# lnkloveating/MediQuery-RAG

Hardware: AMD Instinct MI355X
Metric: queries/s (embed+top-k, k=5, b=256) over 1M×768 corpus; p50 single-query ms (higher is better)
Workload: dtype f32 (exact 3-way bf16 split, fp32 accumulate; exact fp32 top-k)

## Files before the change

### include/mq.h

```cpp
#ifndef MQ_H
#define MQ_H

#include <stdint.h>

#ifdef __cplusplus
extern "C" {
#endif

#define MQ_OK 0
#define MQ_EINVAL -1
#define MQ_ENOMEM -2
#define MQ_EHIP -3
#define MQ_EIO -4
#define MQ_ESTATE -5

#define MQ_DTYPE_F32 0
#define MQ_DTYPE_BF16 1
#define MQ_DTYPE_F32X6 2
#define MQ_DTYPE_F32_SCREEN 3

#define MQ_GELU_ERF 0
#define MQ_GELU_TANH 1
#define MQ_POOL_CLS 0
#define MQ_POOL_MEAN 1

#define MQ_MAX_K 64

typedef struct mq_index mq_index;
typedef struct mq_encoder mq_encoder;

const char* mq_last_error(void);
const char* mq_version(void);
const char* mq_build_source_hash(void);
int mq_device_count(void);

int mq_index_create(int device, int dim, int64_t capacity, int dtype, mq_index** out);
int mq_index_destroy(mq_index* ix);
int mq_index_size(const mq_index* ix, int64_t* n_rows);
int mq_index_dim(const mq_index* ix, int* dim);
int mq_index_add(mq_index* ix, const float* rows, int64_t n, int rows_on_device, void* stream);
int mq_index_reset(mq_index* ix);
int mq_index_search(mq_index* ix, const float* queries, int64_t nq, int k,
                    float* out_scores, int64_t* out_ids, int io_on_device, void* stream);
int mq_index_select(mq_index* src, const int64_t* rows, int64_t n, mq_index* dst);
int mq_index_get(mq_index* ix, int64_t row0, int64_t n, float* out, int out_on_device, void* stream);
int mq_index_set_precision(mq_index* ix, int dtype);
int mq_index_set_stream_threshold(mq_index* ix, int max_queries);
int mq_index_set_threshold_scan(mq_index* ix, int enabled);
int mq_index_set_int8_screen(mq_index* ix, int enabled);
int mq_index_set_async_screen(mq_index* ix, int enabled);
int mq_index_rescans(const mq_index* ix, int64_t* rescans, int64_t* remerges);
int mq_index_screen_fallbacks(const mq_index* ix, int64_t* to_direct, int64_t* to_split);
int mq_index_screen_skips(const mq_index* ix, int64_t* bf16_skips, int64_t* int8_skips);
int mq_index_data(mq_index* ix, void** device_rows);
int mq_index_set_timing(mq_index* ix, int enabled);
int mq_index_read_timing(mq_index* ix, float* ms, int n);
#define MQ_MASK_SET 0
#define MQ_MASK_AND 1
#define MQ_MASK_OR 2
#define MQ_MASK_CLEAR 3
int mq_mask_eval(const int32_t* codes, int64_t n, const uint8_t* lut, int n_lut, uint32_t* bits, int mode,
                 void* stream);
int mq_mask_eval_bits(const int32_t* codes, int64_t n, const uint64_t* lut_words, int n_lut, uint32_t* bits,
                      int mode, void* stream);
int mq_mask_combine(uint32_t* dst, const uint32_t* src, int64_t n_words, int mode, void* stream);
int mq_index_search_masked(mq_index* ix, const float* query, int k, const uint32_t* bits, float* out_scores,
                           int64_t* out_ids, int io_on_device, void* stream);
int mq_index_search_masked_batch(mq_index* ix, const float* queries, int64_t nq, int k, const uint32_t* bits,
                                 float* out_scores, int64_t* out_ids, int io_on_device, void* stream);
int mq_index_masked_gathers(const mq_index* ix, int64_t* count);
#define MQ_CONTAINS_MAX_BYTES 256
#define MQ_CONTAINS_SPAN_BYTES 16384
int mq_mask_contains(const uint8_t* text, int64_t text_bytes, const int64_t* offsets, int64_t n,
                     const uint8_t* pattern, int pattern_len, int negate, uint32_t* bits, int mode,
                     uint32_t* scratch, void* stream);

#define MQ_MMR_SCORE(fmul, fsub, lambda, s, red) \
  fsub(fmul((lambda), (s)), fmul(fsub(1.0f, (lambda)), (red)))
int mq_index_mmr_select(mq_index* ix, const float* cand_scores, const int64_t* cand_ids, int64_t nq,
                        int fetch_k, int k, float lambda, float* out_scores, int64_t* out_ids,
                        int io_on_device, void* stream);
int mq_index_search_mmr(mq_index* ix, const float* queries, int64_t nq, int k, int fetch_k,
                        float lambda, const uint32_t* bits, float* out_scores, int64_t* out_ids,
                        int io_on_device, void* stream);

int mq_index_save(mq_index* ix, const char* path);
int mq_index_load(mq_index* ix, const char* path);
int mq_index_save_rows(mq_index* ix, const char* path, int64_t row0, int64_t n);
int mq_index_load_append(mq_index* ix, const char* path);

int mq_topk_merge_host(const float* scores, const int64_t* ids, int n_lists, int64_t nq,
                       int k_in, int k_out, float* out_scores, int64_t* out_ids);
int mq_topk_merge_device(const float* scores, const int64_t* ids, int n_lists, int64_t nq,
                         int k_in, int k_out, float* out_scores, int64_t* out_ids, void* stream);

typedef struct mq_bert_config {
  int vocab_size;
  int hidden;
  int layers;
  int heads;
  int ffn;
  int max_positions;
  int type_vocab;
  float ln_eps;
  int gelu;
  int pooling;
} mq_bert_config;

int mq_encoder_create(int device, const mq_bert_config* cfg, mq_encoder** out);
int mq_encoder_destroy(mq_encoder* enc);
int64_t mq_encoder_weight_count(const mq_bert_config* cfg);
int mq_encoder_load_weights(mq_encoder* enc, const float* blob, int64_t n_floats);
int mq_encoder_set_precision(mq_encoder* enc, int dtype);
#define MQ_ENC_STAGES 8
int mq_encoder_set_graphs(mq_encoder* enc, int enabled);
#define MQ_ENC_OPT_ROWS_MAX 0
#define MQ_ENC_OPT_ROWS_SPLITS 1
#define MQ_ENC_OPT_SPLITK_MAX 2
#define MQ_ENC_OPT_LN_ROWS_PER_WAVE 3
#define MQ_ENC_OPT_FUSE_ATTN_OPROJ 4
#define MQ_ENC_OPT_FUSED_LN 5
#define MQ_ENC_OPT_SPLITK_TILES 6
#define MQ_ENC_OPT_LN_ON_LOAD 7
#define MQ_ENC_OPT_RESIDENT_LAYERS 8
#define MQ_ENC_OPT_X6_PRESPLIT 9
#define MQ_ENC_OPT_ROWS_PLANES 10
#define MQ_ENC_OPT_LN_FOLD 11
#define MQ_ENC_OPT_CLS_KFREE 12
int mq_encoder_set_option(mq_encoder* enc, int option, int value);
int mq_encoder_get_option(const mq_encoder* enc, int option, int* value);
int mq_encoder_set_timing(mq_encoder* enc, int enabled);
int mq_encoder_read_timing(mq_encoder* enc, float* ms, int n);
int mq_encoder_embed(mq_encoder* enc, const int32_t* ids, const int32_t* mask, int B, int L,
                     float* out, int io_on_device, void* stream);

#define MQ_HEAD_MAX_LABELS 8
int mq_encoder_load_head(mq_encoder* enc, const float* pooler_w, const float* pooler_b, const float* cls_w,
                         const float* cls_b, int n_labels);
int mq_encoder_score(mq_encoder* enc, const int32_t* ids, const int32_t* types, const int32_t* mask, int B,
                     int L, float* logits, int io_on_device, void* stream);

typedef struct mq_tokenizer mq_tokenizer;
int mq_tokenizer_create_wordpiece(const char* vocab_path, int lower_case, int max_length,
                                  mq_tokenizer** out);
int mq_tokenizer_create_wordpiece_tokens(const char* const* tokens, int n_tokens, int lower_case,
                                         int max_length, mq_tokenizer** out);
int mq_tokenizer_create_char(int vocab_size, int max_length, mq_tokenizer** out);
int mq_tokenizer_destroy(mq_tokenizer* tok);
int mq_tokenizer_encode_batch(mq_tokenizer* tok, const char* const* texts, int n, int pad_to,
                              int32_t* ids, int32_t* mask, int* out_len);

int mq_tokenizer_encode_pairs(mq_tokenizer* tok, const char* const* first, const char* const* second, int n,
                              int pad_to, int32_t* ids, int32_t* types, int32_t* mask, int* out_len);

int mq_debug_gemm_f32(const float* A, const float* W, const float* bias, const float* resid,
                      float* out, int M, int N, int K, int epi, int tile, void* stream);
int64_t mq_debug_w3_bytes(int N, int K);
int mq_debug_split_w3(const float* W, int N, int K, void* w3, void* stream);
int mq_debug_gemm_x6p(const float* A, const void* W3, const float* bias, const float* resid,
                      float* out, int M, int N, int K, int epi, int tile, void* stream);
int mq_debug_gemm_x6p_ln(const float* A, const void* W3, const float* bias, const float* resid,
                         float* out, int M, int N, int K, int epi, int tile, const float* stats_in,
                         float* stats_out, const float* g, const float* b, const float* s_fold,
                         float eps, void* stream);
int mq_debug_ln_fold_weight(const float* W, const float* bias, const float* g, const float* b, int N,
                            int K, float* Wg, float* s_out, float* c_out, void* stream);
int mq_debug_attention(const float* qkv, const int* mask, int B, int L, int H, int heads, float scale,
                       int variant, float* ctx, void* stream);
int mq_debug_cls_attention(const float* q, const float* x, const float* stats, const float* ln_g,
                           const float* ln_b, float eps, const int* mask, int B, int L, int H, int heads,
                           float scale, const float* Wk, const float* Wv, const float* bv, float* ctx,
                           void* stream);
int mq_debug_attn_oproj(const float* qkv, const int* mask, int B, int L, int H, int heads, float scale,
                        const float* Wo, const float* bo, const float* resid, int cls_only, int hg, int qf,
                        int acc, float* out, void* stream);

int mq_debug_cls_head(const float* cls, int B, int H, const float* pooler_w, const float* pooler_b,
                      const float* cls_w, const float* cls_b, int n_labels, float* logits, void* stream);

int mq_debug_int8_screen(mq_index* ix, const float* query, int kc, float* out_scores, int64_t* out_ids,
                         float* stats);

#ifdef __cplusplus
}
#endif
#endif
```

### mediquery-rag_amd/csrc/encoder.hip

```cpp
#include <algorithm>
#include <cmath>
#include <cstdlib>
#include <cstring>
#include <memory>
#include <vector>

#include "cls_head.hpp"
#include "common.hpp"
#include "gemm_epi.hpp"
#include "gemm_f32.hpp"
#include "gemm_x6p.hpp"

namespace mq {


struct LnArgs {
  float* stats_out;
  const float* stats_in;
  const float* g;
  const float* b;
  float* xout;
  int ldx;
  int nt;
  float eps;
// ... 1572 lines not shown
      float mu, rho;
      ln_merge(sr, eps, mu, rho);
#pragma unroll
      for (int j = 0; j < 4; ++j) xr[j] = (xr[j] - mu) * rho;
    }
#pragma unroll
    for (int j = 0; j < 4; ++j) *reinterpret_cast<floatx4*>(xs + lrow * H + (lc4 + TPR * j) * 4) = xr[j];
    const int live_key = mk;
    __syncthreads();
    if (k0 + CH < L) fetch(k0 + CH);
    float d[CH];
#pragma unroll
    for (int k = 0; k < CH; ++k) {
      float a = 0.f;
#pragma unroll
      for (int i = 0; i < VPL; ++i) {
        const floatx4 v = *reinterpret_cast<const floatx4*>(xs + k * H + (i * 64 + lane) * 4);
        a = fmaf(v.x, ur[i].x, fmaf(v.y, ur[i].y, fmaf(v.z, ur[i].z, fmaf(v.w, ur[i].w, a))));
      }
      d[k] = a;
    }
#pragma unroll
    for (int k = 0; k < CH; ++k) d[k] = wave_sum_fast(d[k]);
    float sc = -INFINITY;
#pragma unroll
    for (int k = 0; k < CH; ++k) sc = lane == k ? d[k] : sc;
    sc = live_key != 0 ? sc * scale : -INFINITY;
    float tmax = sc;
#pragma unroll
    for (int off = 8; off > 0; off >>= 1) tmax = fmaxf(tmax, __shfl_xor(tmax, off));
    tmax = __shfl(tmax, 0);
    const float m_new = fmaxf(m_run, tmax);
    const float alpha = m_new == -INFINITY ? 1.f : expf(m_run - m_new);
    const float p = sc == -INFINITY ? 0.f : expf(sc - m_new);
    float psum = p;
#pragma unroll
    for (int off = 8; off > 0; off >>= 1) psum += __shfl_xor(psum, off);
    psum = __shfl(psum, 0);
    l_run = l_run * alpha + psum;
    m_run = m_new;
    if (lane < CH) ps[lane * HEADS + h] = p;
    if (lane == 0) alpha_s[h] = alpha;
    __syncthreads();
#pragma unroll
    for (int q4 = 0; q4 < HEADS / 4; ++q4) {
      const floatx4 a = *reinterpret_cast<const floatx4*>(alpha_s + 4 * q4);
#pragma unroll
      for (int e = 0; e < 4; ++e) zacc[4 * q4 + e] *= a[e];
    }
#pragma unroll
    for (int k = 0; k < CH; ++k) {
      const float xv = xs[k * H + t];
#pragma unroll
      for (int q4 = 0; q4 < HEADS / 4; ++q4) {
        const floatx4 pp = *reinterpret_cast<const floatx4*>(ps + k * HEADS + 4 * q4);
#pragma unroll
        for (int e = 0; e < 4; ++e) zacc[4 * q4 + e] = fmaf(pp[e], xv, zacc[4 * q4 + e]);
      }
    }
    __syncthreads();
  }
  if (lane == 0) l_s[h] = l_run;
  __syncthreads();
#pragma unroll
  for (int hh = 0; hh < HEADS; ++hh) {
    const float l = l_s[hh];
    float v = l > 0.f ? zacc[hh] * (1.0f / l) : 0.f;
    if constexpr (FOLD) v = l > 0.f ? fmaf(v, g[t], be[t]) : 0.f;
    z[((int64_t)b * HEADS + hh) * H + t] = v;
  }
  if (t == 0) live[b] = l_s[0] > 0.f ? 1.f : 0.f;
}

}

using namespace mq;

namespace {

struct Buf {
  float* p = nullptr;
  size_t n = 0;
  int ensure(size_t need) {
    if (need <= n) return MQ_OK;
    if (p) (void)hipFree(p);
    p = nullptr;
    n = 0;
    if (hipMalloc((void**)&p, need * sizeof(float)) != hipSuccess)
      MQ_FAIL(MQ_ENOMEM, "hipMalloc(%zu floats) failed", need);
    n = need;
    return MQ_OK;
  }
  void release() {
    if (p) (void)hipFree(p);
    p = nullptr;
    n = 0;
  }
};

struct LayerW {
  const float *wqkv, *bqkv, *wo, *bo, *ln1g, *ln1b, *w1, *b1, *w2, *b2, *ln2g, *ln2b;
  const unsigned char *wqkv3 = nullptr, *wo3 = nullptr, *w13 = nullptr, *w23 = nullptr;
  const float *wqkvf = nullptr, *wof = nullptr, *w1f = nullptr, *w2f = nullptr;
  const unsigned char *w1g3 = nullptr, *wqkvg3 = nullptr;
  const float *w1gf = nullptr, *wqkvgf = nullptr;
  const float *w1s = nullptr, *w1c = nullptr, *wqkvs = nullptr, *wqkvc = nullptr;
};

int64_t weight_count(const mq_bert_config& c) {
  const int64_t H = c.hidden, F = c.ffn;
  const int64_t per_layer = 3 * H * H + 3 * H + H * H + H + 2 * H + F * H + F + H * F + H + 2 * H;
  return ((int64_t)c.vocab_size + c.max_positions + c.type_vocab) * H + 2 * H + c.layers * per_layer;
}

}


namespace {

struct GemmArgs {
  float* slab;
  size_t slab_floats;
  const float* A;
  int lda;
  const float* W;
  const float* bias;
  const float* resid;
  int ldr;
  float* out;
  int ldo;
  int M, N, K;
  int nt = 0;
  const void* W3 = nullptr;
  LnFold lf{};
};

template <class T, int EPI, bool LN_IN = false>
void launch_gemm_t(const GemmArgs& g, int num_cus, hipStream_t s, const LnArgs& ln = LnArgs{}) {
  const int tiles = ((g.M + T::BM - 1) / T::BM) * ((g.N + T::BN - 1) / T::BN);
  const int grid = (std::min(tiles, T::WG_PER_CU * num_cus) + 7) / 8 * 8;
  const int tiles_m = (g.M + T::BM - 1) / T::BM, tiles_n = (g.N + T::BN - 1) / T::BN;
  const int rx = region_pick_rx(tiles_m, tiles_n, (double)T::BM * g.K * 4, (double)T::BN * g.K * 4, grid);
  hipLaunchKernelGGL((gemm_nt_kernel<T, EPI, LN_IN>), dim3(grid), dim3(T::THREADS), 0, s, g.A, g.lda, g.W,
                     g.bias, g.resid, g.ldr, g.out, g.ldo, g.M, g.N, g.K, ln, rx, g.lf);
}

using GemmBig = F32Tile<2, 2, 2, 2>;
using GemmT96 = F32Tile<4, 1, 1, 3>;
using GemmMid = F32Tile<2, 2, 2, 1>;
using GemmSmall = F32Tile<1, 4, 1, 1>;

using X6Big = F32Tile<2, 2, 2, 2, true, 2, false, 0, false, true>;
using X6T96 = F32Tile<4, 1, 1, 3, true, 2, false, 0, false, true>;
using X6Mid = F32Tile<2, 2, 2, 1, true, 2, false, 0, false, true>;
using X6W192 = F32Tile<4, 2, 1, 3, true, 2, false, 0, false, true>;

template <int EPI>
void launch_gemm_tile(const GemmArgs& g, int tile, int num_cus, hipStream_t s) {
  switch (tile) {
    case 0: launch_gemm_t<GemmBig, EPI>(g, num_cus, s); return;
    case 1: launch_gemm_t<GemmT96, EPI>(g, num_cus, s); return;
    case 2: launch_gemm_t<GemmMid, EPI>(g, num_cus, s); return;
    case 5: launch_gemm_t<X6Big, EPI>(g, num_cus, s); return;
    case 6: launch_gemm_t<X6T96, EPI>(g, num_cus, s); return;
    case 7: launch_gemm_t<X6Mid, EPI>(g, num_cus, s); return;
    case 8: launch_gemm_t<F32Tile<4, 2, 1, 3>, EPI>(g, num_cus, s); return;
    case 9: launch_gemm_t<X6W192, EPI>(g, num_cus, s); return;
    default: launch_gemm_t<GemmSmall, EPI>(g, num_cus, s); return;
  }
}

int splitk_factor(const GemmArgs& g, int num_cus, int cap = 16, int tiles_max = 0) {
  if (!g.slab || g.N % 4 != 0) return 0;
  const int64_t tiles = (int64_t)((g.M + 31) / 32) * ((g.N + 127) / 128);
  const int64_t slots = 2 * (int64_t)num_cus;
  if (tiles > (tiles_max > 0 ? tiles_max : num_cus) || g.M > 256) return 0;
  const int slices = g.K / kBK;
  int best = 1;
  for (int s = 1; s <= slices && s <= cap; ++s)
    if (slices % s == 0 && tiles * s <= slots && (size_t)s * g.M * g.N <= g.slab_floats) best = s;
  return best >= 2 ? best : 0;
}

void launch_splitk_gemm(const GemmArgs& g, int S, hipStream_t s) {
  auto go = [&](auto tile) {
    using T = decltype(tile);
    const int tiles = ((g.M + T::BM - 1) / T::BM) * ((g.N + T::BN - 1) / T::BN);
    hipLaunchKernelGGL((gemm_splitk_kernel<T>), dim3(tiles * S), dim3(256), 0, s, g.A, g.lda, g.W, g.M, g.N, g.K,
                       S, g.slab);
  };
  if (g.nt)
    go(F32Tile<1, 4, 1, 1, false, 2, false, 0, true>{});
  else
    go(F32Tile<1, 4, 1, 1>{});
}

template <int EPI>
void launch_splitk(const GemmArgs& g, int S, hipStream_t s) {
  launch_splitk_gemm(g, S, s);
  const int64_t n4 = (int64_t)g.M * g.N / 4;
  hipLaunchKernelGGL((splitk_reduce_kernel<EPI>), dim3((unsigned)((n4 + 255) / 256)), dim3(256), 0,
                     s, g.slab, S, g.M, g.N, g.bias, g.resid, g.ldr, g.out, g.ldo);
}

int x6_tile_pick(const GemmArgs& g, int num_cus) {
  const int bns[3] = {128, 96, 64};
  const double effs[3] = {1.0, 0.96, 0.9};
  const int64_t slots = 2 * (int64_t)num_cus;
  int best = 0;
  double best_cost = 1e300;
  for (int i = 0; i < 3; ++i) {
    const int64_t tiles = (int64_t)((g.M + 127) / 128) * ((g.N + bns[i] - 1) / bns[i]);
    const double cost = (double)((tiles + slots - 1) / slots) * 128 * bns[i] / effs[i];
    if (cost < best_cost) {
      best_cost = cost;
      best = i;
    }
  }
  return best;
}

template <int EPI>
void launch_gemm_fold(const GemmArgs& g, int num_cus, hipStream_t s) {
  if (g.W3) {
    X6pArgs a{g.A, g.lda, g.W3, g.bias, g.resid, g.ldr, g.out, g.ldo, g.M, g.N, g.K};
    a.lf = g.lf;
    launch_gemm_x6p(a, EPI, -1, num_cus, s);
    return;
  }
  if constexpr (EPI == EPI_RESID_LN_STATS) {
    launch_gemm_t<X6T96, EPI>(g, num_cus, s);
  } else {
    switch (x6_tile_pick(g, num_cus)) {
      case 0: launch_gemm_t<X6Big, EPI>(g, num_cus, s); return;
      case 1: launch_gemm_t<X6T96, EPI>(g, num_cus, s); return;
      default: launch_gemm_t<X6Mid, EPI>(g, num_cus, s); return;
    }
  }
}

template <int EPI>
void launch_gemm(const GemmArgs& g, int num_cus, hipStream_t s, bool x6 = false, int splitk_cap = 16,
                 int splitk_tiles = 0) {
  const int S = splitk_factor(g, num_cus, splitk_cap, splitk_tiles);
  if (S) {
    launch_splitk<EPI>(g, S, s);
    return;
  }
  if (x6 && (int64_t)((g.M + 127) / 128) * ((g.N + 191) / 192) < num_cus) x6 = false;
  if (x6 && g.W3) {
    launch_gemm_x6p(X6pArgs{g.A, g.lda, g.W3, g.bias, g.resid, g.ldr, g.out, g.ldo, g.M, g.N, g.K}, EPI, -1, num_cus,
                    s);
    return;
  }
  if (x6) {
    launch_gemm_tile<EPI>(g, 5 + x6_tile_pick(g, num_cus), num_cus, s);
    return;
  }
  struct Cand {
    int bm, bn;
    double eff;
  };
  const Cand cands[4] = {{128, 128, 1.0}, {128, 96, 0.96}, {128, 64, 0.9}, {32, 128, 0.55}};
  const int64_t slots = 2 * (int64_t)num_cus;
  int best = 0;
  double best_cost = 1e300;
  for (int i = 0; i < 4; ++i) {
    const int64_t tiles = (int64_t)((g.M + cands[i].bm - 1) / cands[i].bm) * ((g.N + cands[i].bn - 1) / cands[i].bn);
    const int64_t rounds = (tiles + slots - 1) / slots;
    const double cost = (double)rounds * cands[i].bm * cands[i].bn / cands[i].eff;
    if (cost < best_cost) {
      best_cost = cost;
      best = i;
    }
  }
  launch_gemm_tile<EPI>(g, best, num_cus, s);
}

void launch_gemm_stats(const GemmArgs& g, const LnArgs& ln, int num_cus, hipStream_t s) {
  launch_gemm_t<GemmT96, EPI_RESID_STATS>(g, num_cus, s, ln);
}

template <int EPI>
void launch_gemm_ln_in(const GemmArgs& g, const LnArgs& ln, int num_cus, hipStream_t s) {
  const int64_t slots = 2 * (int64_t)num_cus;
  auto cost = [&](int bn, double eff) {
    const int64_t tiles = (int64_t)((g.M + 127) / 128) * ((g.N + bn - 1) / bn);
    return (double)((tiles + slots - 1) / slots) * 128 * bn / eff;
  };
  if (cost(128, 1.0) <= cost(96, 0.96))
    launch_gemm_t<GemmBig, EPI, true>(g, num_cus, s, ln);
  else
    launch_gemm_t<GemmT96, EPI, true>(g, num_cus, s, ln);
}

#ifndef MQ_LN_FOLD_DEFAULT
#define MQ_LN_FOLD_DEFAULT 1
#endif
constexpr bool kLnFoldDefault = MQ_LN_FOLD_DEFAULT != 0;
#ifndef MQ_CLS_KFREE_DEFAULT
#define MQ_CLS_KFREE_DEFAULT 1
#endif
constexpr bool kClsKfreeDefault = MQ_CLS_KFREE_DEFAULT != 0;

enum Stage { ST_EMBED = 0, ST_QKV, ST_ATTN, ST_OPROJ, ST_LN, ST_FFN_UP, ST_FFN_DOWN, ST_POOL, ST_N };


}

struct mq_encoder {
  int device = 0;
  PinBuf pin;
  mq_bert_config cfg{};
  int precision = MQ_DTYPE_F32;
  bool loaded = false;
  Buf weights;
  const float *word = nullptr, *pos = nullptr, *typ = nullptr, *eg = nullptr, *eb = nullptr;
  std::vector<LayerW> layers;
  Buf x, y, qkv, ctx, ffn, io_out, slab;
  Buf w3;
  Buf wfrag;
  int* io_ids = nullptr;
  int* io_mask = nullptr;
  size_t io_tokens = 0;
  Timeline tl;
  int num_cus = 256;
  struct Graph {
    int B = 0, L = 0, precision = 0;
    std::vector<const void*> bufs;
    hipGraphExec_t exec = nullptr;
    uint64_t last_use = 0;
  };
  std::vector<Graph> graphs;
  bool fuse_attn_oproj = true;
  int rows_max = kRowsDefault;
  int rows_splits = 0;
  int splitk_max = 16;
  int splitk_tiles = 0;
  int ln_rows_per_wave = 4;
  bool fused_ln = false;
  int resident_layers = 8;
  bool ln_on_load = false;
  Buf lnst;
  bool x6_presplit = true;
  bool ln_fold = kLnFoldDefault;
  Buf wfold3, wfoldf, sfold;
  bool rows_planes = false;
  bool cls_kfree = kClsKfreeDefault;
  Buf wkt;
  Buf cls;
  Buf head;
  int n_labels = 0;
  Buf cls_state;
  int* io_types = nullptr;
  size_t io_type_tokens = 0;
  bool use_graphs = false;
  uint64_t graph_clock = 0;
  hipStream_t cap_stream = nullptr;
  std::mutex mu;
};

namespace {

int build_w3(mq_encoder* e) {
  if (e->precision != MQ_DTYPE_F32X6 || !e->loaded || e->layers.empty() || e->layers[0].wqkv3) return MQ_OK;
  const mq_bert_config& c = e->cfg;
  const int H = c.hidden, F = c.ffn;
  const size_t per = w3_bytes(3 * H, H) + w3_bytes(H, H) + w3_bytes(F, H) + w3_bytes(H, F);
  DeviceGuard dg(e->device);
  int rc = e->w3.ensure((per * e->layers.size() + 3) / 4);
  if (rc) return rc;
  unsigned char* p = reinterpret_cast<unsigned char*>(e->w3.p);
  for (LayerW& w : e->layers) {
    auto one = [&](const float* W, int n, int k, const unsigned char*& dst) {
      launch_split_w3(W, n, k, p, nullptr);
      dst = p;
      p += w3_bytes(n, k);
    };
    one(w.wqkv, 3 * H, H, w.wqkv3);
    one(w.wo, H, H, w.wo3);
    one(w.w1, F, H, w.w13);
    one(w.w2, H, F, w.w23);
  }
  MQ_HIP(hipGetLastError());
  MQ_HIP(hipStreamSynchronize(nullptr));
  return MQ_OK;
}

int build_fold(mq_encoder* e) {
  const mq_bert_config& c = e->cfg;
  const int H = c.hidden, F = c.ffn;
  if (!e->ln_fold || e->precision != MQ_DTYPE_F32X6 || !e->loaded || e->layers.empty() ||
      H != kLnPartW * kLnMaxParts || F % 32 != 0)
    return MQ_OK;
  const bool img = e->x6_presplit;
  if (img ? e->layers[0].w1g3 != nullptr : e->layers[0].w1gf != nullptr) return MQ_OK;
  const size_t nl = e->layers.size();
  DeviceGuard dg(e->device);
  int rc = e->sfold.ensure(nl * 2 * ((size_t)F + 3 * H));
  if (rc) return rc;
  Buf tmp;
  if (img) {
    rc = e->wfold3.ensure((nl * w3_bytes(F, H) + (nl - 1) * w3_bytes(3 * H, H) + 3) / 4);
    if (!rc) rc = tmp.ensure((size_t)std::max(F, 3 * H) * H);
  } else {
    rc = e->wfoldf.ensure((nl * (size_t)F + (nl - 1) * (size_t)3 * H) * H);
  }
  if (rc) return rc;
  unsigned char* p3 = reinterpret_cast<unsigned char*>(e->wfold3.p);
  float* pf = e->wfoldf.p;
  float* ps = e->sfold.p;
  const LayerW* prev = nullptr;
  for (LayerW& w : e->layers) {
    auto one = [&](const float* W, const float* bias, const float* g, const float* b, int n, const unsigned char*& d3,
                   const float*& df, const float*& ds, const float*& dc) {
      float* wg = img ? tmp.p : pf;
      launch_ln_fold_weight(W, bias, g, b, n, H, wg, ps, ps + n, nullptr);
      ds = ps;
      dc = ps + n;
      ps += 2 * n;
      if (img) {
        launch_split_w3(wg, n, H, p3, nullptr);
        d3 = p3;
        p3 += w3_bytes(n, H);
      } else {
        df = pf;
        pf += (size_t)n * H;
      }
    };
    one(w.w1, w.b1, w.ln1g, w.ln1b, F, w.w1g3, w.w1gf, w.w1s, w.w1c);
    if (prev) one(w.wqkv, w.bqkv, prev->ln2g, prev->ln2b, 3 * H, w.wqkvg3, w.wqkvgf, w.wqkvs, w.wqkvc);
    prev = &w;
  }
  const hipError_t e1 = hipGetLastError(), e2 = hipStreamSynchronize(nullptr);
  tmp.release();
  MQ_HIP(e1);
  MQ_HIP(e2);
  return MQ_OK;
}

int build_frag16(mq_encoder* e) {
  const mq_bert_config& c = e->cfg;
  const int64_t H = c.hidden, F = c.ffn;
  const int64_t per = 3 * H * H + H * H + F * H + H * F;
  DeviceGuard dg(e->device);
  int rc = e->wfrag.ensure((size_t)(per * (int64_t)e->layers.size()));
  if (rc) return rc;
  float* p = e->wfrag.p;
  for (LayerW& w : e->layers) {
    auto one = [&](const float* W, int64_t r, int64_t k, const float*& dst) {
      const int64_t n4 = r * k / 4;
      hipLaunchKernelGGL(frag16_image_kernel, dim3((unsigned)((n4 + 255) / 256)), dim3(256), 0, nullptr, W, (int)r,
                         (int)k, reinterpret_cast<floatx4*>(p));
      dst = p;
      p += r * k;
    };
    one(w.wqkv, 3 * H, H, w.wqkvf);
    one(w.wo, H, H, w.wof);
    one(w.w1, F, H, w.w1f);
    one(w.w2, H, F, w.w2f);
  }
  MQ_HIP(hipGetLastError());
  MQ_HIP(hipStreamSynchronize(nullptr));
  return MQ_OK;
}

int build_wkt(mq_encoder* e) {
  const int H = e->cfg.hidden;
  if (e->cfg.pooling != MQ_POOL_CLS || e->layers.empty()) return MQ_OK;
  DeviceGuard dg(e->device);
  int rc = e->wkt.ensure((size_t)H * H);
  if (rc) return rc;
  hipLaunchKernelGGL(transpose_kernel, dim3(H / 32, H / 32), dim3(256), 0, nullptr,
                     e->layers.back().wqkv + (int64_t)H * H, H, H, e->wkt.p);
  MQ_HIP(hipGetLastError());
  MQ_HIP(hipStreamSynchronize(nullptr));
  return MQ_OK;
}

template <int EPI>
void gemm(mq_encoder* e, const GemmArgs& g, int stage, hipStream_t s) {
  e->tl.mark(s, stage);
  GemmArgs a = g;
  if (!e->x6_presplit) a.W3 = nullptr;
  launch_gemm<EPI>(a, e->num_cus, s, e->precision == MQ_DTYPE_F32X6, e->splitk_max, e->splitk_tiles);
}

template <int VPL>
void gemm_resid_ln(mq_encoder* e, const GemmArgs& g, const float* lng, const float* lnb, float* x,
                   int stage, hipStream_t s) {
  const int H = VPL * 256;
  const unsigned rb = (unsigned)((g.M + 3) / 4);
  const int S = splitk_factor(g, e->num_cus, e->splitk_max, e->splitk_tiles);
  if constexpr (VPL <= 3) {
    if (!S && e->fused_ln && e->precision == MQ_DTYPE_F32 && g.ldr == H && g.N == H && g.resid == x) {
      using T = F32Tile<1, 8, 1, VPL, false, 2, false, 16>;
      e->tl.mark(s, stage);
      const int tiles = (g.M + 31) / 32;
      hipLaunchKernelGGL((gemm_resid_ln_kernel<T>), dim3(std::min(tiles, e->num_cus)), dim3(T::THREADS), 0, s,
                         g.A, g.lda, g.W, g.bias, g.resid, lng, lnb, e->cfg.ln_eps, x, g.M, g.K);
      return;
    }
  }
  if (S && g.ldr == H && g.N == H) {
    e->tl.mark(s, stage);
    launch_splitk_gemm(g, S, s);
    e->tl.mark(s, ST_LN);
    hipLaunchKernelGGL((splitk_reduce_ln_kernel<VPL>), dim3((unsigned)g.M), dim3(256), 0, s, g.slab, S,
                       g.M, g.bias, g.resid, g.ldr, lng, lnb, e->cfg.ln_eps, x, 0);
    return;
  }
  gemm<EPI_RESID>(e, g, stage, s);
  e->tl.mark(s, ST_LN);
  const int rpw = e->ln_rows_per_wave;
  if (rpw == 4)
    hipLaunchKernelGGL((ln_kernel<VPL, 4>), dim3((unsigned)((g.M + 15) / 16)), dim3(256), 0, s, g.out, g.M, lng,
                       lnb, e->cfg.ln_eps, x);
  else if (rpw == 1)
    hipLaunchKernelGGL((ln_kernel<VPL, 1>), dim3(rb), dim3(256), 0, s, g.out, g.M, lng, lnb, e->cfg.ln_eps, x);
  else
    hipLaunchKernelGGL((ln_kernel<VPL, 2>), dim3((unsigned)((g.M + 7) / 8)), dim3(256), 0, s, g.out, g.M, lng,
                       lnb, e->cfg.ln_eps, x);
}

struct ClsBufs {
  float *xc, *q, *u, *z, *part, *live;
  static size_t floats(int B, int H, int heads) {
    return (size_t)B * ((2 + kClsCtxSplits) * H + 2 * (size_t)heads * H + 1);
  }
  ClsBufs(float* p, int B, int H, int heads)
      : xc(p), q(xc + (size_t)B * H), u(q + (size_t)B * H), z(u + (size_t)B * heads * H),
        part(z + (size_t)B * heads * H), live(part + (size_t)kClsCtxSplits * B * H) {}
};

void launch_cls_u(int B, int H, int heads, const float* q, const float* wkt, float* u, hipStream_t s) {
  using T = F32Tile<1, 4, 1, 1>;
  const int tiles = ((B + T::BM - 1) / T::BM) * ((H + T::BN - 1) / T::BN);
  hipLaunchKernelGGL((gemm_heads_kernel<T>), dim3(tiles * heads), dim3(256), 0, s, q, H, kDh, wkt, H, kDh, nullptr,
                     nullptr, B, H, kDh, u, heads * H, H, 1, (int64_t)0);
}

void launch_cls_ctx(int B, int L, int H, int heads, float scale, const float* x, const float* stats,
                    const float* g, const float* be, float eps, const float* u, const int* mask, const float* wv,
                    const float* bv, float* z, float* part, float* live, float* ctx, hipStream_t s) {
  auto pass = [&](auto vpl) {
    constexpr int VPL = decltype(vpl)::value;
    if (stats)
      hipLaunchKernelGGL((cls_pass_kernel<VPL, true>), dim3(B), dim3(256 * VPL), 0, s, x, stats, g, be, eps, u, mask, L,
                         scale, z, live);
    else
      hipLaunchKernelGGL((cls_pass_kernel<VPL, false>), dim3(B), dim3(256 * VPL), 0, s, x, stats, g, be, eps, u, mask, L,
                         scale, z, live);
  };
  if (H == 256)
    pass(IC<1>{});
  else if (H == 512)
    pass(IC<2>{});
  else
    pass(IC<3>{});
  using T = F32Tile<2, 2, 1, 1>;
  const int tiles = (B + T::BM - 1) / T::BM;
  hipLaunchKernelGGL((gemm_heads_kernel<T>), dim3(tiles * heads * kClsCtxSplits), dim3(256), 0, s, z, heads * H, H, wv, H,
                     kDh * H, nullptr, nullptr, B, kDh, H, part, H, kDh, kClsCtxSplits, (int64_t)B * H);
  hipLaunchKernelGGL(cls_ctx_reduce_kernel, dim3((unsigned)(((int64_t)B * H / 4 + 255) / 256)), dim3(256), 0, s, part, B,
                     H, bv, live, ctx);
}

template <int VPL>
void gemm_resid_ln_pool(mq_encoder* e, const GemmArgs& g, const float* lng, const float* lnb, const int* mask,
                        float* out, int raw, int stage, hipStream_t s) {
  const int H = VPL * 256;
  const int S = splitk_factor(g, e->num_cus, e->splitk_max, e->splitk_tiles);
  if (S && g.ldr == H && g.N == H) {
    e->tl.mark(s, stage);
    launch_splitk_gemm(g, S, s);
    e->tl.mark(s, ST_POOL);
    hipLaunchKernelGGL((splitk_reduce_ln_kernel<VPL, true>), dim3((unsigned)g.M), dim3(256), 0, s, g.slab, S, g.M,
                       g.bias, g.resid, g.ldr, lng, lnb, e->cfg.ln_eps, out, raw);
    return;
  }
  gemm<EPI_RESID>(e, g, stage, s);
  e->tl.mark(s, ST_POOL);
  hipLaunchKernelGGL((ln_pool_kernel<VPL>), dim3((unsigned)((g.M + 3) / 4)), dim3(256), 0, s, g.out, 1, (int64_t)0, mask,
                     g.M, 1, 1, MQ_POOL_CLS, lng, lnb, e->cfg.ln_eps, out, raw);
}

template <int VPL>
int forward_vpl(mq_encoder* e, const int* ids, const int* types, const int* mask, int B, int L, float* out,
                int raw_cls, hipStream_t s) {
  const mq_bert_config& c = e->cfg;
  const int M = B * L, H = c.hidden, F = c.ffn;
  const unsigned row_blocks = (unsigned)((M + 3) / 4);
  const float scale = 1.0f / sqrtf((float)(H / c.heads));
  const int q_tiles = (L + 31) / 32;
  e->tl.mark(s, ST_EMBED);
  hipLaunchKernelGGL((embed_ln_kernel<VPL>), dim3(row_blocks), dim3(256), 0, s, ids, M, L,
                     c.vocab_size, e->word, e->pos, e->typ, types, c.type_vocab, e->eg, e->eb, c.ln_eps, e->x.p);
  const int nt = H / kLnPartW;
  const bool lnl = e->ln_on_load && !e->fused_ln && e->precision == MQ_DTYPE_F32 && M > 256 &&
                   H == kLnPartW * kLnMaxParts && e->lnst.n >= (size_t)4 * M * nt;
  float* st1 = e->lnst.p;
  float* st2 = lnl ? e->lnst.p + (size_t)2 * M * nt : nullptr;
  bool y_pending = false;
  const LayerW* prev = nullptr;
  const LayerW w0 = e->layers.empty() ? LayerW{} : e->layers[0];
  const bool fold = e->ln_fold && e->precision == MQ_DTYPE_F32X6 && M > 256 && H == kLnPartW * kLnMaxParts &&
                    F % 32 == 0 && (int64_t)((M + 127) / 128) * ((H + 191) / 192) >= e->num_cus &&
                    e->lnst.n >= (size_t)4 * M * nt && (e->x6_presplit ? w0.w1g3 != nullptr : w0.w1gf != nullptr);
  float* fst1 = e->lnst.p;
  float* fst2 = e->lnst.p + (size_t)2 * M * nt;
  bool raw = false;
  bool pooled = false;
  auto fold_gemm = [&](auto epi, GemmArgs g, int stage) {
    e->tl.mark(s, stage);
    if (!e->x6_presplit) g.W3 = nullptr;
    g.lf.eps = c.ln_eps;
    launch_gemm_fold<decltype(epi)::value>(g, e->num_cus, s);
  };
  auto ln_args = [&](const float* stats, const float* g, const float* b) {
    LnArgs a{};
    a.stats_in = stats;
    a.g = g;
    a.b = b;
    a.xout = e->x.p;
    a.ldx = H;
    a.nt = nt;
    a.eps = c.ln_eps;
    return a;
  };
  auto stats_out = [&](float* stats) {
    LnArgs a{};
    a.stats_out = stats;
    a.nt = nt;
    return a;
  };
  for (size_t li = 0; li < e->layers.size(); ++li) {
    const LayerW& w = e->layers[li];
    const bool cls_only = c.pooling == MQ_POOL_CLS && li + 1 == e->layers.size();
    const int rows = cls_only ? B : M;
    int stride = cls_only ? L * H : H;
    const float* resid = e->x.p;
    int ldr = stride;
    const bool kfree = cls_only && L > 1 && e->cls_kfree && VPL <= 3 && e->wkt.p != nullptr &&
                       e->cls.n >= ClsBufs::floats(B, H, c.heads);
    const float* qkv_in = y_pending ? e->y.p : e->x.p;
    const int lnt = M <= 256 && (int)li >= e->resident_layers ? 1 : 0;
    const bool fold_layer = fold && !(cls_only && L > 1);
    auto qkv_fold = [&](GemmArgs g, int row0) {
      g.W = w.wqkvgf ? w.wqkvgf + (int64_t)row0 * H : nullptr;
      g.W3 = w.wqkvg3 ? w.wqkvg3 + w3_row_offset(row0, H) : nullptr;
      g.bias = w.wqkvc + row0;
      g.lf.s = w.wqkvs + row0;
      g.lf.stats_in = fst2;
      fold_gemm(IC<EPI_BIAS_LNFOLD>{}, g, ST_QKV);
    };
    auto qkv_gemm = [&](GemmArgs g) {
      g.nt = lnt;
      if (raw) {
        qkv_fold(g, (int)(g.W - w.wqkv) / H);
      } else if (y_pending) {
        e->tl.mark(s, ST_QKV);
        launch_gemm_ln_in<EPI_BIAS>(g, ln_args(st2, prev->ln2g, prev->ln2b), e->num_cus, s);
      } else {
        gemm<EPI_BIAS>(e, g, ST_QKV, s);
      }
    };
    if (kfree) {
      const ClsBufs cb(e->cls.p, B, H, c.heads);
      const float* xin = raw ? e->x.p : y_pending ? e->y.p : e->x.p;
      const float* xst = raw ? fst2 : y_pending ? st2 : nullptr;
      if (xst) {
        e->tl.mark(s, ST_LN);
        hipLaunchKernelGGL((ln_rows_kernel<VPL>), dim3((unsigned)((B + 3) / 4)), dim3(256), 0, s, xin, B, (int64_t)L * H,
                           prev->ln2g, prev->ln2b, c.ln_eps, cb.xc);
        resid = cb.xc;
        ldr = H;
      }
      GemmArgs q{e->slab.p, e->slab.n, resid, ldr, w.wqkv, w.bqkv, nullptr, 0, cb.q, H, B, H, H, lnt};
      q.W3 = w.wqkv3;
      gemm<EPI_BIAS>(e, q, ST_QKV, s);
      launch_cls_u(B, H, c.heads, cb.q, e->wkt.p, cb.u, s);
      e->tl.mark(s, ST_ATTN);
      launch_cls_ctx(B, L, H, c.heads, scale, xin, xst, xst ? prev->ln2g : nullptr, xst ? prev->ln2b : nullptr,
                     c.ln_eps, cb.u, mask, w.wqkv + (int64_t)2 * H * H, w.bqkv + 2 * H, cb.z, cb.part, cb.live, e->ctx.p, s);
      stride = H;
    } else if (cls_only && L > 1) {
      GemmArgs kv{e->slab.p, e->slab.n, qkv_in, H, w.wqkv + (int64_t)H * H, w.bqkv + H, nullptr, 0, e->qkv.p + H,
                  3 * H, M, 2 * H, H};
      if (w.wqkv3) kv.W3 = w.wqkv3 + w3_row_offset(H, H);
      qkv_gemm(kv);
      if (raw) {
        e->tl.mark(s, ST_LN);
        hipLaunchKernelGGL((ln_rows_inplace_kernel<VPL>), dim3((unsigned)((B + 3) / 4)), dim3(256), 0, s, e->x.p, B,
                           (int64_t)L * H, prev->ln2g, prev->ln2b, c.ln_eps);
      }
      GemmArgs q{e->slab.p, e->slab.n, e->x.p, L * H, w.wqkv, w.bqkv, nullptr, 0, e->qkv.p, L * 3 * H, B, H, H, lnt};
      q.W3 = w.wqkv3;
      gemm<EPI_BIAS>(e, q, ST_QKV, s);
    } else {
      GemmArgs qkv{e->slab.p, e->slab.n, qkv_in, H, w.wqkv, w.bqkv, nullptr, 0, e->qkv.p, 3 * H, M, 3 * H, H};
      qkv.W3 = w.wqkv3;
      qkv_gemm(qkv);
    }
    y_pending = false;
    const bool resid_raw = raw && fold_layer;
    raw = false;
    if (!kfree) {
      e->tl.mark(s, ST_ATTN);
      const int qt = cls_only ? 1 : q_tiles;
      launch_attention(B, L, c.heads, qt, H, scale, e->qkv.p, mask, e->ctx.p, s);
    }
    const bool lnl_layer = lnl && !cls_only;
    GemmArgs oproj{e->slab.p, e->slab.n, e->ctx.p, stride, w.wo, w.bo, resid, ldr, e->y.p, H, rows, H, H, lnt};
    oproj.W3 = w.wo3;
    if (fold_layer) {
      oproj.lf.stats_out = fst1;
      if (resid_raw) {
        oproj.lf.stats_in = fst2;
        oproj.lf.g = prev->ln2g;
        oproj.lf.b = prev->ln2b;
      }
      fold_gemm(IC<EPI_RESID_LN_STATS>{}, oproj, ST_OPROJ);
    } else if (lnl_layer) {
      e->tl.mark(s, ST_OPROJ);
      launch_gemm_stats(oproj, stats_out(st1), e->num_cus, s);
    } else {
      gemm_resid_ln<VPL>(e, oproj, w.ln1g, w.ln1b, e->x.p, ST_OPROJ, s);
    }
    GemmArgs up{e->slab.p, e->slab.n, lnl_layer ? e->y.p : e->x.p, H, w.w1, w.b1, nullptr, 0, e->ffn.p, F,
                rows, F, H, lnt};
    up.W3 = w.w13;
    if (fold_layer) {
      up.A = e->y.p;
      up.W = w.w1gf;
      up.W3 = w.w1g3;
      up.bias = w.w1c;
      up.lf.s = w.w1s;
      up.lf.stats_in = fst1;
      if (c.gelu == MQ_GELU_TANH)
        fold_gemm(IC<EPI_GELU_TANH_LNFOLD>{}, up, ST_FFN_UP);
      else
        fold_gemm(IC<EPI_GELU_ERF_LNFOLD>{}, up, ST_FFN_UP);
    } else if (lnl_layer) {
      e->tl.mark(s, ST_FFN_UP);
      if (c.gelu == MQ_GELU_TANH)
        launch_gemm_ln_in<EPI_GELU_TANH>(up, ln_args(st1, w.ln1g, w.ln1b), e->num_cus, s);
      else
        launch_gemm_ln_in<EPI_GELU_ERF>(up, ln_args(st1, w.ln1g, w.ln1b), e->num_cus, s);
    } else if (c.gelu == MQ_GELU_TANH) {
      gemm<EPI_GELU_TANH>(e, up, ST_FFN_UP, s);
    } else {
      gemm<EPI_GELU_ERF>(e, up, ST_FFN_UP, s);
    }
    GemmArgs down{e->slab.p, e->slab.n, e->ffn.p, F, w.w2, w.b2, e->x.p, H, e->y.p, H, rows, H, F, lnt};
    down.W3 = w.w23;
    if (fold_layer) {
      const bool last = li + 1 == e->layers.size();
      down.resid = e->y.p;
      down.lf.stats_in = fst1;
      down.lf.g = w.ln1g;
      down.lf.b = w.ln1b;
      down.lf.stats_out = fst2;
      down.out = last ? e->ctx.p : e->x.p;
      fold_gemm(IC<EPI_RESID_LN_STATS>{}, down, ST_FFN_DOWN);
      if (last) {
        e->tl.mark(s, ST_LN);
        hipLaunchKernelGGL((ln_kernel<VPL, 4>), dim3((unsigned)((M + 15) / 16)), dim3(256), 0, s, e->ctx.p, M, w.ln2g,
                           w.ln2b, c.ln_eps, e->x.p);
      } else {
        raw = true;
      }
    } else if (lnl_layer && li + 1 < e->layers.size()) {
      e->tl.mark(s, ST_FFN_DOWN);
      launch_gemm_stats(down, stats_out(st2), e->num_cus, s);
      y_pending = true;
    } else if (kfree) {
      gemm_resid_ln_pool<VPL>(e, down, w.ln2g, w.ln2b, mask, out, raw_cls, ST_FFN_DOWN, s);
      pooled = true;
    } else {
      gemm_resid_ln<VPL>(e, down, w.ln2g, w.ln2b, e->x.p, ST_FFN_DOWN, s);
    }
    prev = &w;
  }
  if (!pooled) {
    e->tl.mark(s, ST_POOL);
    const bool pruned = c.pooling == MQ_POOL_CLS;
    hipLaunchKernelGGL((pool_kernel<VPL>), dim3((B + 3) / 4), dim3(256), 0, s, e->x.p, mask, B,
                       pruned ? 1 : L, c.pooling, out, raw_cls);
  }
  e->tl.close(s);
  MQ_HIP(hipGetLastError());
  return MQ_OK;
}

struct RowsArgs {
  const float* A;
  int lda;
  int64_t a_plane;
  const float* W;
  int ldw;
  const float* bias;
  const float* resid;
  int ldr;
  float* out;
  int ldo;
  int64_t o_plane;
  int M, N, K;
  int splits;
  const int* ids = nullptr;
  int L = 1, vocab = 0;
  const float* pos = nullptr;
  const float* typ = nullptr;
  const int* types = nullptr;
  int type_vocab = 1;
  int nt_w = 0;
  float* zbuf = nullptr;
  int64_t zn = 0;
};

template <int EPI, bool LN_IN, int VPL, int NB, int S_IN, int RT, int FL>
void launch_rows_rt(const RowsArgs& g, const float* lng, const float* lnb, float eps, float* ln_out,
                    hipStream_t s) {
  hipLaunchKernelGGL((rows_gemm_kernel<EPI, LN_IN, VPL, NB, S_IN, RT, FL>),
                     dim3(g.N / kRT, (g.M + kRT * RT - 1) / (kRT * RT), g.splits), dim3(64 * kRWaves), 0, s,
                     g.A, g.lda, g.a_plane, g.M, lng, lnb, eps, ln_out, g.W, g.ldw, g.bias, g.resid, g.ldr,
                     g.out, g.ldo, g.o_plane, g.ids, g.L, g.vocab, g.pos, g.typ, g.types, g.type_vocab, g.nt_w, g.zbuf,
                     g.zn);
}

template <int EPI, bool LN_IN, int VPL, int NB, int S_IN, int FL = 0>
void launch_rows_nb(const RowsArgs& g, const float* lng, const float* lnb, float eps, float* ln_out,
                    hipStream_t s) {
  constexpr bool two_fit = LN_IN && (size_t)(2 * kRT * (NB * 256 + 4) + kRWaves * 2 * kRT * kRT) * 4 <= 160 * 1024;
  if constexpr (two_fit) {
    if (g.M > kRT) {
      launch_rows_rt<EPI, LN_IN, VPL, NB, S_IN, 2, FL>(g, lng, lnb, eps, ln_out, s);
      return;
    }
  }
  launch_rows_rt<EPI, LN_IN, VPL, NB, S_IN, 1, FL>(g, lng, lnb, eps, ln_out, s);
}

bool rows_nb_ok(int nb) { return nb >= 1 && (nb <= 4 || nb == 6 || nb == 8 || nb == 12 || nb == 16); }

int rows_splits(int K, int forced = 0) {
  const int nb = K / 256;
  if (forced >= 1 && forced <= 4 && nb % forced == 0 && rows_nb_ok(nb / forced)) return forced;
  for (int sp = 1; sp <= 4; ++sp)
    if (nb % sp == 0 && nb / sp <= 6 && rows_nb_ok(nb / sp)) return sp;
  return 1;
}

template <int EPI, int NB, int FL>
void launch_rows_plain(const RowsArgs& g, hipStream_t s) {
  launch_rows_nb<EPI, false, 1, NB, 1, FL>(g, nullptr, nullptr, 0.f, nullptr, s);
}

template <int EPI, int FL = 0>
void launch_rows(const RowsArgs& g, hipStream_t s) {
  switch (g.K / g.splits / 256) {
    case 1: launch_rows_plain<EPI, 1, FL>(g, s); return;
    case 2: launch_rows_plain<EPI, 2, FL>(g, s); return;
    case 3: launch_rows_plain<EPI, 3, FL>(g, s); return;
    case 4: launch_rows_plain<EPI, 4, FL>(g, s); return;
    case 6: launch_rows_plain<EPI, 6, FL>(g, s); return;
    case 8: launch_rows_plain<EPI, 8, FL>(g, s); return;
    case 12: launch_rows_plain<EPI, 12, FL>(g, s); return;
    default: launch_rows_plain<EPI, 16, FL>(g, s); return;
  }
}

template <int EPI, int VPL, int FL = 0>
void launch_rows_ln(const RowsArgs& g, int s_in, const float* lng, const float* lnb, float eps,
                    float* ln_out, hipStream_t s) {
  switch (s_in) {
    case 0: launch_rows_nb<EPI, true, VPL, VPL, 0, FL>(g, lng, lnb, eps, ln_out, s); return;
    case 1: launch_rows_nb<EPI, true, VPL, VPL, 1, FL>(g, lng, lnb, eps, ln_out, s); return;
    case 2: launch_rows_nb<EPI, true, VPL, VPL, 2, FL>(g, lng, lnb, eps, ln_out, s); return;
    case 3: launch_rows_nb<EPI, true, VPL, VPL, 3, FL>(g, lng, lnb, eps, ln_out, s); return;
    default: launch_rows_nb<EPI, true, VPL, VPL, 4, FL>(g, lng, lnb, eps, ln_out, s); return;
  }
}

template <int HG, bool QF, bool ACC>
void launch_attn_oproj_hg(int nkb, dim3 grid, hipStream_t s, const float* qkv, const int* mask, int L, int H,
                          int rps, int qtiles, float scale, const float* wo, const float* bo, const float* resid,
                          int ldr, float* out, int64_t o_plane, int nt_w) {
  auto go = [&](auto kern) {
    hipLaunchKernelGGL(kern, grid, dim3(512), 0, s, qkv, mask, L, H, rps, qtiles, scale, wo, bo, resid, ldr, out,
                       o_plane, nt_w);
  };
  switch (nkb) {
    case 1: go(attn_oproj_rows_kernel<HG, 1, QF, ACC>); break;
    case 2: go(attn_oproj_rows_kernel<HG, 2, QF, ACC>); break;
    case 3: go(attn_oproj_rows_kernel<HG, 3, QF, ACC>); break;
    default: go(attn_oproj_rows_kernel<HG, 4, QF, ACC>); break;
  }
}

void launch_attn_oproj(int hg, bool qf, bool acc, int nkb, dim3 grid, hipStream_t s, const float* qkv,
                       const int* mask, int L, int H, int rps, int qtiles, float scale, const float* wo,
                       const float* bo, const float* resid, int ldr, float* out, int64_t o_plane, int nt_w) {
  auto go = [&](auto hgc, auto qfc, auto accc) {
    launch_attn_oproj_hg<decltype(hgc)::value, decltype(qfc)::value, decltype(accc)::value>(
        nkb, grid, s, qkv, mask, L, H, rps, qtiles, scale, wo, bo, resid, ldr, out, o_plane, nt_w);
  };
  if (hg == 6) {
    if (qf && acc) go(IC<6>{}, std::true_type{}, std::true_type{});
    else if (qf) go(IC<6>{}, std::true_type{}, std::false_type{});
    else if (acc) go(IC<6>{}, std::false_type{}, std::true_type{});
    else go(IC<6>{}, std::false_type{}, std::false_type{});
  } else {
    if (qf && acc) go(IC<4>{}, std::true_type{}, std::true_type{});
    else if (qf) go(IC<4>{}, std::true_type{}, std::false_type{});
    else if (acc) go(IC<4>{}, std::false_type{}, std::true_type{});
    else go(IC<4>{}, std::false_type{}, std::false_type{});
  }
}

int oproj_heads_per_plane(const mq_encoder* e, int L) {
  const mq_bert_config& c = e->cfg;
  if (!e->fuse_attn_oproj || L > 64 || c.hidden != c.heads * kDh || c.hidden % kOpCols) return 0;
  return c.heads % 6 == 0 ? 6 : c.heads % 4 == 0 ? 4 : 0;
}

template <int VPL>
int forward_rows(mq_encoder* e, const int* ids, const int* types, const int* mask, int B, int L, float* out,
                 int raw, hipStream_t s) {
  const mq_bert_config& c = e->cfg;
  const int M = B * L, H = c.hidden, F = c.ffn;
  const float eps = c.ln_eps;
  const float scale = 1.0f / sqrtf((float)(H / c.heads));
  const int q_tiles = (L + 31) / 32;
  const int dsplit = rows_splits(F, e->rows_splits);
  const int hg = oproj_heads_per_plane(e, L);
  const bool qf = hg != 0 && L % 16 == 0 && (3 * H) % 48 == 0;
  const bool dacc = dsplit == 2 && !e->rows_planes;
  const bool yacc = hg != 0 && c.heads / hg == 2 && !e->rows_planes;
  int prev_rows = M;
  for (size_t li = 0; li < e->layers.size(); ++li) {
    const LayerW& w = e->layers[li];
    const bool cls_only = c.pooling == MQ_POOL_CLS && li + 1 == e->layers.size();
    const int rows = cls_only ? B : M;
    const int stride = cls_only ? L * H : H;
    const int nt = (int)li >= e->resident_layers ? 1 : 0;
    e->tl.mark(s, ST_QKV);
    RowsArgs qkv{e->slab.p, H, (int64_t)prev_rows * H, w.wqkvf, H, w.bqkv, nullptr, 0, e->qkv.p, 3 * H, 0, M, 3 * H, H, 1};
    qkv.nt_w = nt;
    if (li == 0) {
      qkv.A = e->word;
      qkv.a_plane = 0;
      qkv.ids = ids;
      qkv.L = L;
      qkv.vocab = c.vocab_size;
      qkv.pos = e->pos;
      qkv.typ = e->typ;
      qkv.types = types;
      qkv.type_vocab = c.type_vocab;
    }
    const LayerW* pl = li ? &e->layers[li - 1] : nullptr;
    const float* lg = pl ? pl->ln2g : e->eg;
    const float* lb = pl ? pl->ln2b : e->eb;
    const int s_in = pl ? (dacc ? 1 : dsplit) : 0;
    if (yacc) {
      qkv.zbuf = e->y.p;
      qkv.zn = (int64_t)rows * H;
    }
    if (qf)
      ROWS_REP launch_rows_ln<EPI_BIAS, VPL, FL_O | FL_OT>(qkv, s_in, lg, lb, eps, e->x.p, s);
    else
      ROWS_REP launch_rows_ln<EPI_BIAS, VPL>(qkv, s_in, lg, lb, eps, e->x.p, s);
    const int qt = cls_only ? 1 : q_tiles;
    int y_planes = 1;
    if (hg) {
      e->tl.mark(s, ST_OPROJ);
      const int rps = cls_only ? 1 : L, qtiles = (rps + 15) / 16;
      y_planes = c.heads / hg;
      const dim3 grid(H / kOpCols, B * qtiles, y_planes);
      if (yacc) y_planes = 1;
      ROWS_REP launch_attn_oproj(hg, qf, yacc, (L + 15) / 16, grid, s, e->qkv.p, mask, L, H, rps, qtiles, scale, w.wof, w.bo, e->x.p,
                                 stride, e->y.p, (int64_t)rows * H, nt);
    } else {
      e->tl.mark(s, ST_ATTN);
      if (L <= 64)
        hipLaunchKernelGGL(attention_rows_kernel, dim3(B * c.heads * qt), dim3(512), 0, s, e->qkv.p, mask, L,
                           H, c.heads, qt, scale, e->ctx.p);
      else
        launch_attention(B, L, c.heads, qt, H, scale, e->qkv.p, mask, e->ctx.p, s);
      e->tl.mark(s, ST_OPROJ);
      RowsArgs oproj{e->ctx.p, stride, 0, w.wof, H, w.bo, e->x.p, stride, e->y.p, H, 0, rows, H, H, 1};
      oproj.nt_w = nt;
      launch_rows<EPI_RESID>(oproj, s);
    }
    e->tl.mark(s, ST_FFN_UP);
    RowsArgs up{e->y.p, H, (int64_t)rows * H, w.w1f, H, w.b1, nullptr, 0, e->ffn.p, F, 0, rows, F, H, 1};
    up.nt_w = nt;
    if (dacc) {
      up.zbuf = e->slab.p;
      up.zn = (int64_t)rows * H;
    }
    if (c.gelu == MQ_GELU_TANH)
      ROWS_REP launch_rows_ln<EPI_GELU_TANH, VPL, FL_O>(up, y_planes, w.ln1g, w.ln1b, eps, e->x.p, s);
    else
      ROWS_REP launch_rows_ln<EPI_GELU_ERF, VPL, FL_O>(up, y_planes, w.ln1g, w.ln1b, eps, e->x.p, s);
    e->tl.mark(s, ST_FFN_DOWN);
    RowsArgs down{e->ffn.p, F, 0, w.w2f, F, w.b2, e->x.p, H, e->slab.p, H, (int64_t)rows * H, rows, H, F, dsplit};
    down.nt_w = nt;
    if (dacc)
      ROWS_REP launch_rows<EPI_RESID, FL_A | FL_ACC>(down, s);
    else
      ROWS_REP launch_rows<EPI_RESID, FL_A>(down, s);
    prev_rows = rows;
  }
// ... 122 lines not shown
               "bad config");
  MQ_CHECK_ARG(c.gelu == MQ_GELU_ERF || c.gelu == MQ_GELU_TANH, "bad gelu variant");
  MQ_CHECK_ARG(c.pooling == MQ_POOL_CLS || c.pooling == MQ_POOL_MEAN, "bad pooling");
  DeviceGuard dg(device);
  if (!dg.ok) MQ_FAIL(MQ_EHIP, "hipSetDevice(%d) failed", device);
  auto e = std::make_unique<mq_encoder>();
  e->device = device;
  e->cfg = c;
  int cus = 0;
  if (hipDeviceGetAttribute(&cus, hipDeviceAttributeMultiprocessorCount, device) == hipSuccess &&
      cus > 0)
    e->num_cus = cus;
  *out = e.release();
  return MQ_OK;
}

int mq_encoder_destroy(mq_encoder* e) {
  clear_error();
  if (!e) return MQ_OK;
  {
    DeviceGuard dg(e->device);
    for (Buf* b : {&e->weights, &e->x, &e->y, &e->qkv, &e->ctx, &e->ffn, &e->io_out, &e->slab, &e->w3, &e->wfrag,
                   &e->lnst, &e->wkt, &e->cls, &e->head, &e->cls_state})
      b->release();
    if (e->io_types) (void)hipFree(e->io_types);
    if (e->io_ids) (void)hipFree(e->io_ids);
    if (e->io_mask) (void)hipFree(e->io_mask);
    e->pin.release();
    for (auto& g : e->graphs) (void)hipGraphExecDestroy(g.exec);
    if (e->cap_stream) (void)hipStreamDestroy(e->cap_stream);
  }
  delete e;
  return MQ_OK;
}

int mq_encoder_load_weights(mq_encoder* e, const float* blob, int64_t n_floats) {
  clear_error();
  MQ_CHECK_ARG(e && blob, "NULL argument");
  const mq_bert_config& c = e->cfg;
  const int64_t need = weight_count(c);
  MQ_CHECK_ARG(n_floats == need, "weight blob has %lld floats, config needs %lld",
               (long long)n_floats, (long long)need);
  std::lock_guard<std::mutex> lk(e->mu);
  DeviceGuard dg(e->device);
  int rc = e->weights.ensure((size_t)need);
  if (rc) return rc;
  MQ_HIP(hipMemcpy(e->weights.p, blob, (size_t)need * 4, hipMemcpyHostToDevice));
  const int64_t H = c.hidden, F = c.ffn;
  const float* p = e->weights.p;
  auto take = [&](int64_t n) {
    const float* r = p;
    p += n;
    return r;
  };
  e->word = take((int64_t)c.vocab_size * H);
  e->pos = take((int64_t)c.max_positions * H);
  e->typ = take((int64_t)c.type_vocab * H);
  e->eg = take(H);
  e->eb = take(H);
  e->layers.clear();
  for (int l = 0; l < c.layers; ++l) {
    LayerW w;
    w.wqkv = take(3 * H * H);
    w.bqkv = take(3 * H);
    w.wo = take(H * H);
    w.bo = take(H);
    w.ln1g = take(H);
    w.ln1b = take(H);
    w.w1 = take(F * H);
    w.b1 = take(F);
    w.w2 = take(H * F);
    w.b2 = take(H);
    w.ln2g = take(H);
    w.ln2b = take(H);
    e->layers.push_back(w);
  }
  e->loaded = true;
  if (H % 16 == 0 && F % 16 == 0) {
    rc = build_frag16(e);
    if (rc) return rc;
  }
  rc = build_wkt(e);
  if (rc) return rc;
  return build_w3(e);
}

int mq_encoder_set_precision(mq_encoder* e, int dtype) {
  clear_error();
  MQ_CHECK_ARG(e, "NULL encoder");
  MQ_CHECK_ARG(dtype == MQ_DTYPE_F32 || dtype == MQ_DTYPE_F32X6,
               "encoder precision must be MQ_DTYPE_F32 or MQ_DTYPE_F32X6 (got %d)", dtype);
  std::lock_guard<std::mutex> lk(e->mu);
  e->precision = dtype;
  return build_w3(e);
}

int mq_debug_gemm_f32(const float* A, const float* W, const float* bias, const float* resid,
                      float* out, int M, int N, int K, int epi, int tile, void* stream) {
  clear_error();
  MQ_CHECK_ARG(A && W && bias && out && (epi != EPI_RESID || resid), "NULL buffer");
  MQ_CHECK_ARG(M > 0 && N > 0 && K > 0 && K % kBK == 0, "bad shape M=%d N=%d K=%d", M, N, K);
  MQ_CHECK_ARG(epi >= 0 && epi <= 3 && tile >= 0 && tile <= 9, "bad epi/tile");
  int dev = 0, cus = 256;
  (void)hipGetDevice(&dev);
  (void)hipDeviceGetAttribute(&cus, hipDeviceAttributeMultiprocessorCount, dev);
  GemmArgs g{nullptr, 0, A, K, W, bias, resid, N, out, N, M, N, K};
  hipStream_t s = (hipStream_t)stream;
  if (tile == 4) {
    MQ_CHECK_ARG(N % 4 == 0, "split-K needs N %% 4 == 0");
    const int slices = K / kBK;
    int S = 1;
    for (int c = 2; c <= slices && c <= 64; ++c)
      if (slices % c == 0) S = c;
    float* slab = nullptr;
    if (hipMalloc((void**)&slab, (size_t)S * M * N * 4) != hipSuccess)
      MQ_FAIL(MQ_ENOMEM, "slab allocation failed");
    g.slab = slab;
    g.slab_floats = (size_t)S * M * N;
    switch (epi) {
      case EPI_BIAS: launch_splitk<EPI_BIAS>(g, S, s); break;
      case EPI_GELU_ERF: launch_splitk<EPI_GELU_ERF>(g, S, s); break;
      case EPI_GELU_TANH: launch_splitk<EPI_GELU_TANH>(g, S, s); break;
      default: launch_splitk<EPI_RESID>(g, S, s); break;
    }
    const hipError_t err = hipStreamSynchronize(s);
    (void)hipFree(slab);
    if (err != hipSuccess) MQ_FAIL(MQ_EHIP, "split-K GEMM failed: %s", hipGetErrorString(err));
    return MQ_OK;
  }
  switch (epi) {
    case EPI_BIAS: launch_gemm_tile<EPI_BIAS>(g, tile, cus, s); break;
    case EPI_GELU_ERF: launch_gemm_tile<EPI_GELU_ERF>(g, tile, cus, s); break;
    case EPI_GELU_TANH: launch_gemm_tile<EPI_GELU_TANH>(g, tile, cus, s); break;
    default: launch_gemm_tile<EPI_RESID>(g, tile, cus, s); break;
  }
  MQ_HIP(hipGetLastError());
  return MQ_OK;
}

int mq_debug_attention(const float* qkv, const int* mask, int B, int L, int H, int heads, float scale,
                       int variant, float* ctx, void* stream) {
  clear_error();
  MQ_CHECK_ARG(qkv && mask && ctx, "NULL buffer");
  MQ_CHECK_ARG(B > 0 && L > 0 && heads > 0 && H == heads * kDh, "bad shape B=%d L=%d H=%d heads=%d", B, L, H, heads);
  hipStream_t s = (hipStream_t)stream;
  const int qt = (L + 31) / 32;
  const dim3 grid(B * heads * qt);
  switch (variant) {
    case -1: launch_attention(B, L, heads, qt, H, scale, qkv, mask, ctx, s); break;
    case 1: hipLaunchKernelGGL(attention_kernel<1>, grid, dim3(64), 0, s, qkv, mask, L, H, heads, qt, scale, ctx); break;
    case 2: hipLaunchKernelGGL(attention_kernel<2>, grid, dim3(128), 0, s, qkv, mask, L, H, heads, qt, scale, ctx); break;
    case 4: hipLaunchKernelGGL(attention_kernel<4>, grid, dim3(256), 0, s, qkv, mask, L, H, heads, qt, scale, ctx); break;
    case 8: hipLaunchKernelGGL(attention_kernel<8>, grid, dim3(512), 0, s, qkv, mask, L, H, heads, qt, scale, ctx); break;
    case 12:
      MQ_CHECK_ARG(heads == 12 && L <= 32, "variant 12 needs heads == 12 and L <= 32 (heads %d, L %d)", heads, L);
      hipLaunchKernelGGL((attention_kernel<1, 12>), dim3(B * qt), dim3(768), 0, s, qkv, mask, L, H, heads, qt, scale,
                         ctx);
      break;
    case 16:
      MQ_CHECK_ARG(L <= 64, "variant 16 (attention_rows_kernel) needs L <= 64 (got %d)", L);
      hipLaunchKernelGGL(attention_rows_kernel, grid, dim3(512), 0, s, qkv, mask, L, H, heads, qt, scale, ctx);
      break;
    default: MQ_FAIL(MQ_EINVAL, "bad attention variant %d", variant);
  }
  MQ_HIP(hipGetLastError());
  return MQ_OK;
}

int mq_debug_attn_oproj(const float* qkv, const int* mask, int B, int L, int H, int heads, float scale,
                        const float* Wo, const float* bo, const float* resid, int cls_only, int hg, int qf,
                        int acc, float* out, void* stream) {
  clear_error();
  MQ_CHECK_ARG(qkv && mask && Wo && bo && resid && out, "NULL buffer");
  MQ_CHECK_ARG(B > 0 && L > 0 && heads > 0 && H == heads * kDh, "bad shape B=%d L=%d H=%d heads=%d", B, L, H, heads);
  MQ_CHECK_ARG((hg == 4 || hg == 6) && heads % hg == 0, "hg must be 4 or 6 and divide heads (hg %d, heads %d)", hg,
               heads);
  MQ_CHECK_ARG(L <= 64, "the fused kernel holds L <= 64 keys (got %d)", L);
  MQ_CHECK_ARG(!qf || L % 16 == 0, "qf needs L %% 16 == 0 (got %d)", L);
  const int planes = heads / hg;
  MQ_CHECK_ARG(!acc || planes == 2, "acc needs two head groups (got %d)", planes);
  hipStream_t s = (hipStream_t)stream;
  const int M = B * L, rows = cls_only ? B : M;
  float* scratch = nullptr;
  const size_t wo_floats = (size_t)H * H, qkv_floats = qf ? (size_t)M * 3 * H : 0;
  if (hipMalloc((void**)&scratch, (wo_floats + qkv_floats) * 4) != hipSuccess)
    MQ_FAIL(MQ_ENOMEM, "operand image allocation failed");
  hipLaunchKernelGGL(frag16_image_kernel, dim3((unsigned)((wo_floats / 4 + 255) / 256)), dim3(256), 0, s, Wo, H, H,
                     reinterpret_cast<floatx4*>(scratch));
  const float* qkv_in = qkv;
  if (qf) {
    float* img = scratch + wo_floats;
    hipLaunchKernelGGL(frag16_qkv_image_kernel, dim3((unsigned)((qkv_floats + 255) / 256)), dim3(256), 0, s, qkv, M,
                       H, img);
    qkv_in = img;
  }
  hipError_t err = hipSuccess;
  if (acc) err = hipMemsetAsync(out, 0, (size_t)rows * H * 4, s);
  if (err == hipSuccess) {
    const int rps = cls_only ? 1 : L, qtiles = (rps + 15) / 16;
    const dim3 grid(H / kOpCols, B * qtiles, planes);
    launch_attn_oproj(hg, qf != 0, acc != 0, (L + 15) / 16, grid, s, qkv_in, mask, L, H, rps, qtiles, scale, scratch,
                      bo, resid, cls_only ? L * H : H, out, (int64_t)rows * H, 0);
    err = hipGetLastError();
  }
  const hipError_t serr = hipStreamSynchronize(s);
  (void)hipFree(scratch);
  if (err == hipSuccess) err = serr;
  if (err != hipSuccess) MQ_FAIL(MQ_EHIP, "fused attention + output projection failed: %s", hipGetErrorString(err));
  return MQ_OK;
}

int mq_debug_cls_attention(const float* q, const float* x, const float* stats, const float* ln_g,
                           const float* ln_b, float eps, const int* mask, int B, int L, int H, int heads,
                           float scale, const float* Wk, const float* Wv, const float* bv, float* ctx,
                           void* stream) {
  clear_error();
  MQ_CHECK_ARG(q && x && mask && Wk && Wv && bv && ctx, "NULL buffer");
  MQ_CHECK_ARG(B > 0 && L > 0 && heads > 0 && H == heads * kDh, "bad shape B=%d L=%d H=%d heads=%d", B, L, H, heads);
  MQ_CHECK_ARG(H == 256 || H == 512 || H == 768, "hidden must be 256 / 512 / 768 (got %d)", H);
  MQ_CHECK_ARG(!stats || (ln_g && ln_b && H == kLnPartW * kLnMaxParts), "stats need ln_g, ln_b and H = %d",
               kLnPartW * kLnMaxParts);
  hipStream_t s = (hipStream_t)stream;
  float* scratch = nullptr;
  const size_t wkt_floats = (size_t)H * H;
  if (hipMalloc((void**)&scratch, (wkt_floats + ClsBufs::floats(B, H, heads)) * 4) != hipSuccess)
    MQ_FAIL(MQ_ENOMEM, "scratch allocation failed");
  const ClsBufs cb(scratch + wkt_floats, B, H, heads);
  hipLaunchKernelGGL(transpose_kernel, dim3(H / 32, H / 32), dim3(256), 0, s, Wk, H, H, scratch);
  launch_cls_u(B, H, heads, q, scratch, cb.u, s);
  launch_cls_ctx(B, L, H, heads, scale, x, stats, ln_g, ln_b, eps, cb.u, mask, Wv, bv, cb.z, cb.part, cb.live, ctx, s);
  hipError_t err = hipGetLastError();
  const hipError_t serr = hipStreamSynchronize(s);
  (void)hipFree(scratch);
  if (err == hipSuccess) err = serr;
  if (err != hipSuccess) MQ_FAIL(MQ_EHIP, "CLS attention failed: %s", hipGetErrorString(err));
  return MQ_OK;
}

int mq_encoder_set_graphs(mq_encoder* e, int enabled) {
  clear_error();
  MQ_CHECK_ARG(e, "NULL encoder");
  std::lock_guard<std::mutex> lk(e->mu);
  e->use_graphs = enabled != 0;
  return MQ_OK;
}

int mq_encoder_set_option(mq_encoder* e, int option, int value) {
  clear_error();
  MQ_CHECK_ARG(e, "NULL encoder");
  std::lock_guard<std::mutex> lk(e->mu);
  switch (option) {
    case MQ_ENC_OPT_ROWS_MAX:
      MQ_CHECK_ARG(value >= 0 && value <= kRowsMax, "rows_max must be in [0, %d] (got %d)", kRowsMax, value);
      e->rows_max = value;
      break;
    case MQ_ENC_OPT_ROWS_SPLITS:
      MQ_CHECK_ARG(value >= 0 && value <= 4, "rows_splits must be in [0, 4] (got %d)", value);
      e->rows_splits = value;
      break;
    case MQ_ENC_OPT_SPLITK_MAX:
      MQ_CHECK_ARG(value >= 2 && value <= 64, "splitk_max must be in [2, 64] (got %d)", value);
      e->splitk_max = value;
      break;
    case MQ_ENC_OPT_LN_ROWS_PER_WAVE:
      MQ_CHECK_ARG(value == 1 || value == 2 || value == 4, "ln_rows_per_wave must be 1, 2 or 4 (got %d)", value);
      e->ln_rows_per_wave = value;
      break;
    case MQ_ENC_OPT_FUSE_ATTN_OPROJ:
      MQ_CHECK_ARG(value == 0 || value == 1, "fuse_attn_oproj must be 0 or 1 (got %d)", value);
      e->fuse_attn_oproj = value != 0;
      break;
    case MQ_ENC_OPT_FUSED_LN:
      MQ_CHECK_ARG(value == 0 || value == 1, "fused_ln must be 0 or 1 (got %d)", value);
      e->fused_ln = value != 0;
      break;
    case MQ_ENC_OPT_RESIDENT_LAYERS:
      MQ_CHECK_ARG(value >= 0 && value <= 1024, "resident_layers must be in [0, 1024] (got %d)", value);
      e->resident_layers = value;
      break;
    case MQ_ENC_OPT_LN_ON_LOAD:
      MQ_CHECK_ARG(value == 0 || value == 1, "ln_on_load must be 0 or 1 (got %d)", value);
      e->ln_on_load = value != 0;
      break;
    case MQ_ENC_OPT_SPLITK_TILES:
      MQ_CHECK_ARG(value >= 0 && value <= 4096, "splitk_tiles must be in [0, 4096] (got %d)", value);
      e->splitk_tiles = value;
      break;
    case MQ_ENC_OPT_X6_PRESPLIT:
      MQ_CHECK_ARG(value == 0 || value == 1, "x6_presplit must be 0 or 1 (got %d)", value);
      e->x6_presplit = value != 0;
      break;
    case MQ_ENC_OPT_ROWS_PLANES:
      MQ_CHECK_ARG(value == 0 || value == 1, "rows_planes must be 0 or 1 (got %d)", value);
      e->rows_planes = value != 0;
      break;
    case MQ_ENC_OPT_LN_FOLD:
      MQ_CHECK_ARG(value == 0 || value == 1, "ln_fold must be 0 or 1 (got %d)", value);
      e->ln_fold = value != 0;
      break;
    case MQ_ENC_OPT_CLS_KFREE:
      MQ_CHECK_ARG(value == 0 || value == 1, "cls_kfree must be 0 or 1 (got %d)", value);
      e->cls_kfree = value != 0;
      break;
    default:
      MQ_FAIL(MQ_EINVAL, "unknown encoder option %d", option);
  }
  for (auto& g : e->graphs) (void)hipGraphExecDestroy(g.exec);
  e->graphs.clear();
  return MQ_OK;
}

int mq_encoder_get_option(const mq_encoder* e, int option, int* value) {
  clear_error();
  MQ_CHECK_ARG(e && value, "NULL argument");
  switch (option) {
    case MQ_ENC_OPT_ROWS_MAX: *value = e->rows_max; break;
    case MQ_ENC_OPT_ROWS_SPLITS: *value = e->rows_splits; break;
    case MQ_ENC_OPT_SPLITK_MAX: *value = e->splitk_max; break;
    case MQ_ENC_OPT_LN_ROWS_PER_WAVE: *value = e->ln_rows_per_wave; break;
    case MQ_ENC_OPT_FUSE_ATTN_OPROJ: *value = e->fuse_attn_oproj ? 1 : 0; break;
    case MQ_ENC_OPT_FUSED_LN: *value = e->fused_ln ? 1 : 0; break;
    case MQ_ENC_OPT_LN_ON_LOAD: *value = e->ln_on_load ? 1 : 0; break;
    case MQ_ENC_OPT_RESIDENT_LAYERS: *value = e->resident_layers; break;
    case MQ_ENC_OPT_SPLITK_TILES: *value = e->splitk_tiles; break;
    case MQ_ENC_OPT_X6_PRESPLIT: *value = e->x6_presplit ? 1 : 0; break;
    case MQ_ENC_OPT_ROWS_PLANES: *value = e->rows_planes ? 1 : 0; break;
    case MQ_ENC_OPT_LN_FOLD: *value = e->ln_fold ? 1 : 0; break;
    case MQ_ENC_OPT_CLS_KFREE: *value = e->cls_kfree ? 1 : 0; break;
    default: MQ_FAIL(MQ_EINVAL, "unknown encoder option %d", option);
  }
  return MQ_OK;
}

int mq_encoder_set_timing(mq_encoder* e, int enabled) {
  clear_error();
  MQ_CHECK_ARG(e, "NULL encoder");
  std::lock_guard<std::mutex> lk(e->mu);
  DeviceGuard dg(e->device);
  e->tl.drain();
  e->tl.on = enabled != 0;
  return MQ_OK;
}

int mq_encoder_read_timing(mq_encoder* e, float* ms, int n) {
  clear_error();
  MQ_CHECK_ARG(e && ms && n >= 0, "bad argument");
  std::lock_guard<std::mutex> lk(e->mu);
  DeviceGuard dg(e->device);
  e->tl.read(ms, n);
  return MQ_OK;
}

}

namespace {

int ensure_forward_bufs(mq_encoder* e, int B, int L) {
  const mq_bert_config& c = e->cfg;
  const size_t M = (size_t)B * L;
  if (e->tl.used > 4096) e->tl.drain();
  int rc = MQ_OK;
  rc = e->slab.ensure((size_t)2 * e->num_cus * 32 * 128);
  if (rc) return rc;
  rc = build_fold(e);
  if (rc) return rc;
  const size_t ln_parts = (e->ln_on_load || e->ln_fold) && M > 256 ? (size_t)4 * M * std::max(1, c.hidden / kLnPartW) : 0;
  const size_t cls_floats = e->cls_kfree && c.pooling == MQ_POOL_CLS && L > 1 ? ClsBufs::floats(B, c.hidden, c.heads) : 0;
  for (auto bn : {std::make_pair(&e->x, M * c.hidden), std::make_pair(&e->y, (M <= (size_t)kRowsMax ? 4 : 1) * M * c.hidden),
                  std::make_pair(&e->ctx, M * c.hidden), std::make_pair(&e->qkv, M * 3 * c.hidden),
                  std::make_pair(&e->ffn, (M + 15) / 16 * 16 * c.ffn), std::make_pair(&e->lnst, ln_parts),
                  std::make_pair(&e->cls, cls_floats)}) {
    rc = bn.first->ensure(bn.second);
    if (rc) return rc;
  }
  return MQ_OK;
}

int ensure_io(mq_encoder* e, size_t M, int B) {
  if (e->io_tokens < M) {
    if (e->io_ids) (void)hipFree(e->io_ids);
    if (e->io_mask) (void)hipFree(e->io_mask);
    e->io_ids = e->io_mask = nullptr;
    e->io_tokens = 0;
    if (hipMalloc((void**)&e->io_ids, M * 4) != hipSuccess ||
        hipMalloc((void**)&e->io_mask, M * 4) != hipSuccess)
      MQ_FAIL(MQ_ENOMEM, "hipMalloc(io) failed");
    e->io_tokens = M;
  }
  return e->io_out.ensure((size_t)B * e->cfg.hidden);
}

}

extern "C" {

int mq_encoder_embed(mq_encoder* e, const int32_t* ids, const int32_t* mask, int B, int L,
                     float* out, int io_on_device, void* stream) {
  clear_error();
  MQ_CHECK_ARG(e, "NULL encoder");
  MQ_CHECK_ARG(B >= 0 && L >= 1, "bad shape B=%d L=%d", B, L);
  MQ_CHECK_ARG(L <= e->cfg.max_positions, "L=%d exceeds max_positions %d", L, e->cfg.max_positions);
  if (B == 0) return MQ_OK;
  MQ_CHECK_ARG(ids && mask && out, "NULL buffer");
  MQ_CHECK_ARG((int64_t)B * L < (1ll << 31) / 4096, "batch too large");
  if (!e->loaded) MQ_FAIL(MQ_ESTATE, "encoder weights not loaded");
  std::lock_guard<std::mutex> lk(e->mu);
  DeviceGuard dg(e->device);
  hipStream_t s = (hipStream_t)stream;
  const mq_bert_config& c = e->cfg;
  const size_t M = (size_t)B * L;
  int rc = ensure_forward_bufs(e, B, L);
  if (rc) return rc;
  const bool graph = e->use_graphs && !e->tl.on;
  const int* dids = ids;
  const int* dmask = mask;
  float* dout = out;
  if (!io_on_device || graph) {
    rc = ensure_io(e, M, B);
    if (rc) return rc;
    const hipMemcpyKind kind = io_on_device ? hipMemcpyDeviceToDevice : hipMemcpyHostToDevice;
    if (!io_on_device && M * 8 + (size_t)B * c.hidden * 4 <= (1u << 20)) {
      rc = e->pin.ensure(M * 8 + (size_t)B * c.hidden * 4);
      if (rc) return rc;
      memcpy(e->pin.as<unsigned char>(), ids, M * 4);
      memcpy(e->pin.as<unsigned char>() + M * 4, mask, M * 4);
      MQ_HIP(hipMemcpyAsync(e->io_ids, e->pin.p, M * 4, kind, s));
      MQ_HIP(hipMemcpyAsync(e->io_mask, e->pin.as<unsigned char>() + M * 4, M * 4, kind, s));
    } else {
      MQ_HIP(hipMemcpyAsync(e->io_ids, ids, M * 4, kind, s));
      MQ_HIP(hipMemcpyAsync(e->io_mask, mask, M * 4, kind, s));
    }
    dids = e->io_ids;
    dmask = e->io_mask;
    dout = e->io_out.p;
  }
  if (graph) {
    rc = launch_graph(e, B, L, s);
  } else {
    rc = forward(e, dids, nullptr, dmask, B, L, dout, 0, s);
  }
  if (rc) return rc;
  if (io_on_device && dout != out)
    MQ_HIP(hipMemcpyAsync(out, dout, (size_t)B * c.hidden * 4, hipMemcpyDeviceToDevice, s));
  if (!io_on_device) {
    const size_t ob = (size_t)B * c.hidden * 4;
    if (M * 8 + ob <= (1u << 20)) {
      unsigned char* hp = e->pin.as<unsigned char>() + M * 8;
      MQ_HIP(hipMemcpyAsync(hp, dout, ob, hipMemcpyDeviceToHost, s));
      MQ_HIP(hipStreamSynchronize(s));
      memcpy(out, hp, ob);
    } else {
      MQ_HIP(hipMemcpyAsync(out, dout, ob, hipMemcpyDeviceToHost, s));
      MQ_HIP(hipStreamSynchronize(s));
    }
  }
  return MQ_OK;
}

int mq_encoder_load_head(mq_encoder* e, const float* pooler_w, const float* pooler_b, const float* cls_w,
                         const float* cls_b, int n_labels) {
  clear_error();
  MQ_CHECK_ARG(n_labels >= 1 && n_labels <= MQ_HEAD_MAX_LABELS, "n_labels must be in [1, %d] (got %d)",
               MQ_HEAD_MAX_LABELS, n_labels);
  MQ_CHECK_ARG(e, "NULL encoder");
  MQ_CHECK_ARG(pooler_w && pooler_b && cls_w && cls_b, "NULL argument");
  if (!e->loaded) MQ_FAIL(MQ_ESTATE, "encoder weights not loaded");
  std::lock_guard<std::mutex> lk(e->mu);
  DeviceGuard dg(e->device);
  const size_t H = (size_t)e->cfg.hidden;
  e->n_labels = 0;
  const int rc = e->head.ensure(H * H + H + (size_t)MQ_HEAD_MAX_LABELS * (H + 1));
  if (rc) return rc;
  float* p = e->head.p;
  MQ_HIP(hipMemcpy(p, pooler_w, H * H * 4, hipMemcpyHostToDevice));
  MQ_HIP(hipMemcpy(p + H * H, pooler_b, H * 4, hipMemcpyHostToDevice));
  MQ_HIP(hipMemcpy(p + H * H + H, cls_w, (size_t)n_labels * H * 4, hipMemcpyHostToDevice));
  MQ_HIP(hipMemcpy(p + H * H + H + (size_t)MQ_HEAD_MAX_LABELS * H, cls_b, (size_t)n_labels * 4, hipMemcpyHostToDevice));
  e->n_labels = n_labels;
  return MQ_OK;
}

int mq_encoder_score(mq_encoder* e, const int32_t* ids, const int32_t* types, const int32_t* mask, int B, int L,
                     float* logits, int io_on_device, void* stream) {
  clear_error();
  MQ_CHECK_ARG(e, "NULL encoder");
  MQ_CHECK_ARG(B >= 0 && L >= 1, "bad shape B=%d L=%d", B, L);
  MQ_CHECK_ARG(L <= e->cfg.max_positions, "L=%d exceeds max_positions %d", L, e->cfg.max_positions);
  if (!e->loaded) MQ_FAIL(MQ_ESTATE, "encoder weights not loaded");
  if (e->cfg.pooling != MQ_POOL_CLS) MQ_FAIL(MQ_ESTATE, "scoring needs CLS pooling (the head reads the CLS state)");
  if (B == 0) return MQ_OK;
  MQ_CHECK_ARG(ids && types && mask && logits, "NULL buffer");
  MQ_CHECK_ARG((int64_t)B * L < (1ll << 31) / 4096, "batch too large");
  std::lock_guard<std::mutex> lk(e->mu);
  if (e->n_labels < 1) MQ_FAIL(MQ_ESTATE, "no cross-encoder head loaded (mq_encoder_load_head)");
  DeviceGuard dg(e->device);
  hipStream_t s = (hipStream_t)stream;
  const mq_bert_config& c = e->cfg;
  const size_t M = (size_t)B * L, H = (size_t)c.hidden, nl = (size_t)e->n_labels;
  int rc = ensure_forward_bufs(e, B, L);
  if (!rc) rc = e->cls_state.ensure((size_t)B * H);
  if (rc) return rc;
  const int* dids = ids;
  const int* dtypes = types;
  const int* dmask = mask;
  float* dlogits = logits;
  const size_t ob = (size_t)B * nl * 4;
  if (!io_on_device) {
    rc = ensure_io(e, M, B);
    if (rc) return rc;
    if (e->io_type_tokens < M) {
      if (e->io_types) (void)hipFree(e->io_types);
      e->io_types = nullptr;
      e->io_type_tokens = 0;
      if (hipMalloc((void**)&e->io_types, M * 4) != hipSuccess) MQ_FAIL(MQ_ENOMEM, "hipMalloc(io) failed");
      e->io_type_tokens = M;
    }
    rc = e->pin.ensure(M * 12 + ob);
    if (rc) return rc;
    unsigned char* hp = e->pin.as<unsigned char>();
    memcpy(hp, ids, M * 4);
    memcpy(hp + M * 4, types, M * 4);
    memcpy(hp + M * 8, mask, M * 4);
    MQ_HIP(hipMemcpyAsync(e->io_ids, hp, M * 4, hipMemcpyHostToDevice, s));
    MQ_HIP(hipMemcpyAsync(e->io_types, hp + M * 4, M * 4, hipMemcpyHostToDevice, s));
    MQ_HIP(hipMemcpyAsync(e->io_mask, hp + M * 8, M * 4, hipMemcpyHostToDevice, s));
    dids = e->io_ids;
    dtypes = e->io_types;
    dmask = e->io_mask;
    dlogits = e->io_out.p;
  }
  rc = forward(e, dids, dtypes, dmask, B, L, e->cls_state.p, 1, s);
  if (rc) return rc;
  const float* hp = e->head.p;
  e->tl.mark(s, ST_POOL);
  launch_cls_head(e->cls_state.p, B, c.hidden, hp, hp + H * H, hp + H * H + H,
                  hp + H * H + H + (size_t)MQ_HEAD_MAX_LABELS * H, e->n_labels, dlogits, s);
  e->tl.close(s);
  MQ_HIP(hipGetLastError());
  if (!io_on_device) {
    unsigned char* out_pin = e->pin.as<unsigned char>() + M * 12;
    MQ_HIP(hipMemcpyAsync(out_pin, dlogits, ob, hipMemcpyDeviceToHost, s));
    MQ_HIP(hipStreamSynchronize(s));
    memcpy(logits, out_pin, ob);
  }
  return MQ_OK;
}

#ifdef MQ_KTRACE
int mq_debug_ktrace_read(long long* out, int n) {
  const int total = kTraceRegions * kTraceWgs * kTraceSlots;
  if (!out || n < total) return MQ_EINVAL;
  if (hipMemcpyFromSymbol(out, HIP_SYMBOL(mq_ktrace), total * sizeof(long long)) != hipSuccess) return MQ_EHIP;
  std::vector<long long> zero(total, 0);
  if (hipMemcpyToSymbol(HIP_SYMBOL(mq_ktrace), zero.data(), total * sizeof(long long)) != hipSuccess) return MQ_EHIP;
  return MQ_OK;
}
#endif

}
```

### mediquery-rag_amd/csrc/gemm_epi.hpp

```cpp
#pragma once

#include "gemm_f32.hpp"
#include "gemm_x6p.hpp"

namespace mq {

enum Epi {
  EPI_BIAS = 0,
  EPI_GELU_ERF = 1,
  EPI_GELU_TANH = 2,
  EPI_RESID = 3,
  EPI_RESID_STATS = 4,
  EPI_RESID_LN_STATS = 5,
  EPI_BIAS_LNFOLD = 6,
  EPI_GELU_ERF_LNFOLD = 7,
  EPI_GELU_TANH_LNFOLD = 8
};
constexpr bool epi_is_lnfold(int epi) { return epi >= EPI_BIAS_LNFOLD && epi <= EPI_GELU_TANH_LNFOLD; }

__device__ __forceinline__ float gelu_erf(float x) {
  const float z = fabsf(x) * 0.70710678118654752f;
  const float t = __builtin_amdgcn_rcpf(fmaf(0.5f, z, 1.0f));
  float p = 0.17087277f;
  p = fmaf(p, t, -0.82215223f);
  p = fmaf(p, t, 1.48851587f);
  p = fmaf(p, t, -1.13520398f);
  p = fmaf(p, t, 0.27886807f);
  p = fmaf(p, t, -0.18628806f);
  p = fmaf(p, t, 0.09678418f);
  p = fmaf(p, t, 0.37409196f);
  p = fmaf(p, t, 1.00002368f);
  p = fmaf(p, t, -1.26551223f);
  const float e = t * __builtin_amdgcn_exp2f(fmaf(-z, z, p) * 1.4426950408889634f);
  return x * (x >= 0.f ? fmaf(-0.5f, e, 1.0f) : 0.5f * e);
}
__device__ __forceinline__ float gelu_tanh(float x) {
  const float u = 0.7978845608028654f * fmaf(0.044715f * x, x * x, x);
  return x * __builtin_amdgcn_rcpf(1.0f + __builtin_amdgcn_exp2f(u * -2.8853900817779268f));
}

template <int EPI>
__device__ __forceinline__ float epi_apply(float v) {
  if constexpr (EPI == EPI_GELU_ERF || EPI == EPI_GELU_ERF_LNFOLD) return gelu_erf(v);
  if constexpr (EPI == EPI_GELU_TANH || EPI == EPI_GELU_TANH_LNFOLD) return gelu_tanh(v);
  return v;
}

__device__ __forceinline__ void ln_merge(const floatx4 (&p)[kLnMaxParts / 2], float eps, float& mean, float& rstd) {
  float sum = 0.f;
#pragma unroll
  for (int i = 0; i < kLnMaxParts / 2; ++i) {
    sum += p[i].x;
    sum += p[i].z;
  }
  mean = sum * (1.0f / (float)kLnMaxParts);
  float m2 = 0.f;
#pragma unroll
  for (int i = 0; i < kLnMaxParts / 2; ++i) {
    const float d0 = p[i].x - mean, d1 = p[i].z - mean;
    m2 = __fmaf_rn((float)kLnPartW * d0, d0, m2 + p[i].y);
    m2 = __fmaf_rn((float)kLnPartW * d1, d1, m2 + p[i].w);
  }
  rstd = 1.0f / sqrtf(__fmaf_rn(m2, 1.0f / (float)(kLnPartW * kLnMaxParts), eps));
}
template <int MB>
__device__ __forceinline__ void ln_row_own(const float* __restrict__ stats, int wr0, int M, float eps, int lane,
                                           float& mean, float& rstd) {
  const int c = lane & 15;
  const int row = min(wr0 + 16 * min(c >> 2, MB - 1) + 4 * (lane >> 4) + (c & 3), M - 1);
  const floatx4* src = reinterpret_cast<const floatx4*>(stats + (int64_t)row * (2 * kLnMaxParts));
  floatx4 p[kLnMaxParts / 2];
#pragma unroll
  for (int i = 0; i < kLnMaxParts / 2; ++i) p[i] = src[i];
  ln_merge(p, eps, mean, rstd);
}
__device__ __forceinline__ float ln_row_bcast(float v, int lane, int m, int e) {
  return __shfl(v, (lane & 48) + 4 * m + e);
}
__device__ __forceinline__ float row16_sum(float v) {
  v += __int_as_float(__builtin_amdgcn_update_dpp(0, __float_as_int(v), 0xB1, 0xF, 0xF, false));
  v += __int_as_float(__builtin_amdgcn_update_dpp(0, __float_as_int(v), 0x4E, 0xF, 0xF, false));
  v += __int_as_float(__builtin_amdgcn_update_dpp(0, __float_as_int(v), 0x141, 0xF, 0xF, false));
  v += __int_as_float(__builtin_amdgcn_update_dpp(0, __float_as_int(v), 0x140, 0xF, 0xF, false));
  return v;
}

template <int EPI, int TM, int TN>
__device__ __forceinline__ void store_wave_tile(floatx16 (&acc)[TM][TN], int wr0, int wc0, int M, int N,
                                                const float* __restrict__ bias, const float* __restrict__ resid,
                                                int ldr, float* __restrict__ out, int ldo, int lane) {
  if (wr0 + TM * 32 <= M && wc0 + TN * 32 <= N) {
    float bv[TN];
#pragma unroll
    for (int tn = 0; tn < TN; ++tn) bv[tn] = bias[wc0 + tn * 32 + (lane & 31)];
    float rv[TM][TN][16];
    if constexpr (EPI == EPI_RESID) {
      const __amdgpu_buffer_rsrc_t rr = __builtin_amdgcn_make_buffer_rsrc(
          (void*)(resid + (int64_t)wr0 * ldr + wc0), (short)0, 0x7fffffff, 0x00020000);
      const int rl = (4 * (lane >> 5) * ldr + (lane & 31)) * 4;
#pragma unroll
      for (int tm = 0; tm < TM; ++tm)
#pragma unroll
        for (int tn = 0; tn < TN; ++tn)
#pragma unroll
          for (int e = 0; e < 16; ++e)
            rv[tm][tn][e] = __uint_as_float(
                __builtin_amdgcn_raw_buffer_load_b32(rr, rl, (acc_row(tm, e, 0) * ldr + tn * 32) * 4, 0));
    }
    const __amdgpu_buffer_rsrc_t ro = __builtin_amdgcn_make_buffer_rsrc(
        (void*)(out + (int64_t)wr0 * ldo + wc0), (short)0, 0x7fffffff, 0x00020000);
    const int ol = (4 * (lane >> 5) * ldo + (lane & 31)) * 4;
#pragma unroll
    for (int tm = 0; tm < TM; ++tm)
#pragma unroll
      for (int tn = 0; tn < TN; ++tn)
#pragma unroll
        for (int e = 0; e < 16; ++e) {
          float v = epi_apply<EPI>(acc[tm][tn][e] + bv[tn]);
          if constexpr (EPI == EPI_RESID) v += rv[tm][tn][e];
          __builtin_amdgcn_raw_buffer_store_b32(__float_as_uint(v), ro, ol, (acc_row(tm, e, 0) * ldo + tn * 32) * 4, 0);
        }
    return;
  }
#pragma unroll
  for (int tn = 0; tn < TN; ++tn) {
    const int col = wc0 + tn * 32 + (lane & 31);
    if (col >= N) continue;
    const float b = bias[col];
#pragma unroll
    for (int tm = 0; tm < TM; ++tm)
#pragma unroll
      for (int e = 0; e < 16; ++e) {
        const int row = wr0 + acc_row(tm, e, lane);
        if (row >= M) continue;
        float v = epi_apply<EPI>(acc[tm][tn][e] + b);
        if constexpr (EPI == EPI_RESID) v += resid[(int64_t)row * ldr + col];
        out[(int64_t)row * ldo + col] = v;
      }
  }
}

typedef unsigned uint2v_t __attribute__((ext_vector_type(2)));
__device__ __forceinline__ unsigned ln_t_slot(int lane) { return 16u * (unsigned)(lane ^ (lane >> 4)); }
template <int ER, int MB, int NB, bool HAND = false>
__device__ __forceinline__ void store_wave_tile16_ln_stats(floatx4 (&acc)[MB][NB], int wr0, int wc0, int M,
                                                           const float* __restrict__ bias,
                                                           const float* __restrict__ resid, int ldr,
                                                           float* __restrict__ out, int ldo, int lane,
                                                           const LnFold& lf, const unsigned char* tl = nullptr) {
  static_assert(NB * 16 == kLnPartW && MB <= 4, "partials are per kLnPartW-column wave tile");
  static_assert(!HAND || ER == 1, "the hand-off form finishes a row at a time");
  const int c = lane & 15, g = lane >> 4;
  const bool ln_r = lf.stats_in != nullptr;
  float own_mu = 0.f, own_rho = 1.0f;
  if constexpr (!HAND) {
    if (ln_r) ln_row_own<MB>(lf.stats_in, wr0, M, lf.eps, lane, own_mu, own_rho);
  }
  float gv[NB];
#pragma unroll
  for (int n = 0; n < NB; ++n) {
    const int col = wc0 + n * 16 + c;
    const float bb = bias[col] + (ln_r ? lf.b[col] : 0.f);
    gv[n] = ln_r ? lf.g[col] : 1.0f;
#pragma unroll
    for (int m = 0; m < MB; ++m)
#pragma unroll
      for (int e = 0; e < 4; ++e) acc[m][n][e] += bb;
  }
  const __amdgpu_buffer_rsrc_t rr =
      __builtin_amdgcn_make_buffer_rsrc((void*)(resid + wc0), (short)0, 0x7fffffff, 0x00020000);
  const __amdgpu_buffer_rsrc_t ro =
      __builtin_amdgcn_make_buffer_rsrc((void*)(out + wc0), (short)0, 0x7fffffff, 0x00020000);
  const __amdgpu_buffer_rsrc_t rs = __builtin_amdgcn_make_buffer_rsrc(
      (void*)(lf.stats_out + 2 * (wc0 / kLnPartW)), (short)0, 0x7fffffff, 0x00020000);
#pragma unroll
  for (int m = 0; m < MB; ++m) {
    floatx4 tv[NB];
    if constexpr (HAND) {
#pragma unroll
      for (int n = 0; n < NB; ++n)
        tv[n] = *reinterpret_cast<const floatx4*>(tl + (m * NB + n) * 1024 + ln_t_slot(lane));
    }
#pragma unroll
    for (int eh = 0; eh < 4; eh += ER) {
      float v[ER][NB];
      if constexpr (!HAND) {
#pragma unroll
        for (int e2 = 0; e2 < ER; ++e2) {
          const int lo = (min(wr0 + m * 16 + 4 * g + eh + e2, M - 1) * ldr + c) * 4;
#pragma unroll
          for (int n = 0; n < NB; ++n)
            v[e2][n] = __uint_as_float(__builtin_amdgcn_raw_buffer_load_b32(rr, lo, n * 64, 0));
        }
      }
#pragma unroll
      for (int e2 = 0; e2 < ER; ++e2) {
        const int e = eh + e2, row = wr0 + m * 16 + 4 * g + e;
        float mu = 0.f, rho = 1.0f;
        if constexpr (!HAND) {
          mu = ln_row_bcast(own_mu, lane, m, e);
          rho = ln_row_bcast(own_rho, lane, m, e);
        }
        const int so = (row * ldo + c) * 4;
        float sum = 0.f;
#pragma unroll
        for (int n = 0; n < NB; ++n) {
          if constexpr (HAND)
            v[e2][n] = __fmaf_rn(tv[n][e], gv[n], acc[m][n][e]);
          else
            v[e2][n] = __fmaf_rn((v[e2][n] - mu) * rho, gv[n], acc[m][n][e]);
          sum += v[e2][n];
          if (row < M) __builtin_amdgcn_raw_buffer_store_b32(__float_as_uint(v[e2][n]), ro, so, n * 64, 0);
        }
        const float mean = row16_sum(sum) * (1.0f / (float)kLnPartW);
        float m2 = 0.f;
#pragma unroll
        for (int n = 0; n < NB; ++n) {
          const float d = v[e2][n] - mean;
          m2 = __fmaf_rn(d, d, m2);
        }
        m2 = row16_sum(m2);
        if (c == 0 && row < M) {
          uint2v_t pr;
          pr.x = __float_as_uint(mean);
          pr.y = __float_as_uint(m2);
          __builtin_amdgcn_raw_buffer_store_b64(pr, rs, row * (kLnMaxParts * 8), 0, 0);
        }
      }
    }
  }
}

template <int MB, int NB>
struct LnTileRegs {
  floatx4 r[MB][NB];
  floatx4 p[kLnMaxParts / 2];
};
template <int Q>
__device__ __forceinline__ float quad_bcast(float v) {
  return __int_as_float(__builtin_amdgcn_update_dpp(0, __float_as_int(v), Q * 0x55, 0xF, 0xF, false));
}
template <int MB, int NB>
__device__ __forceinline__ void ln_tile_load(LnTileRegs<MB, NB>& q, const float* __restrict__ resid, int ldr,
                                             int wr0, int wc0, int M, const LnFold& lf, int lane) {
  const __amdgpu_buffer_rsrc_t rr =
      __builtin_amdgcn_make_buffer_rsrc((void*)(resid + wc0), (short)0, 0x7fffffff, 0x00020000);
#pragma unroll
  for (int m = 0; m < MB; ++m) {
    const int row = min(wr0 + m * 16 + (lane >> 2), M - 1);
    const int lo = (row * ldr + 4 * (lane & 3)) * 4;
#pragma unroll
    for (int n = 0; n < NB; ++n)
      q.r[m][n] = __builtin_bit_cast(floatx4, __builtin_amdgcn_raw_buffer_load_b128(rr, lo, n * 64, 0));
  }
  if (lf.stats_in != nullptr) {
    const int row = min(wr0 + (lane & 3) * 16 + (lane >> 2), M - 1);
    const floatx4* src = reinterpret_cast<const floatx4*>(lf.stats_in + (int64_t)row * (2 * kLnMaxParts));
#pragma unroll
    for (int i = 0; i < kLnMaxParts / 2; ++i) q.p[i] = src[i];
  }
}
template <int MB, int NB>
__device__ __forceinline__ void ln_tile_write(const LnTileRegs<MB, NB>& q, unsigned char* tl, const LnFold& lf,
                                              int lane) {
  static_assert(MB == 4, "a quad's lanes share out the block rows");
  const int g = lane >> 4, e = (lane >> 2) & 3;
  unsigned off[4];
#pragma unroll
  for (int i = 0; i < 4; ++i) off[i] = (unsigned)(256 * g + 16 * ((4 * (lane & 3) + i) ^ g) + 4 * e);
  float own_mu = 0.f, own_rho = 1.0f;
  if (lf.stats_in != nullptr) ln_merge(q.p, lf.eps, own_mu, own_rho);
  const float mus[4] = {quad_bcast<0>(own_mu), quad_bcast<1>(own_mu), quad_bcast<2>(own_mu), quad_bcast<3>(own_mu)};
  const float rhos[4] = {quad_bcast<0>(own_rho), quad_bcast<1>(own_rho), quad_bcast<2>(own_rho),
                         quad_bcast<3>(own_rho)};
#pragma unroll
  for (int m = 0; m < MB; ++m) {
    const float mu = mus[m], rho = rhos[m];
#pragma unroll
    for (int n = 0; n < NB; ++n)
#pragma unroll
      for (int i = 0; i < 4; ++i)
        *reinterpret_cast<float*>(tl + (m * NB + n) * 1024 + off[i]) = (q.r[m][n][i] - mu) * rho;
  }
}

template <int EPI, int MB, int NB>
__device__ __forceinline__ void store_wave_tile16(floatx4 (&acc)[MB][NB], int wr0, int wc0, int M, int N,
                                                  const float* __restrict__ bias, const float* __restrict__ resid,
                                                  int ldr, float* __restrict__ out, int ldo, int lane,
                                                  const LnFold& lf = LnFold{}) {
  const int c = lane & 15, g = lane >> 4;
  if constexpr (EPI == EPI_RESID_LN_STATS) {
    store_wave_tile16_ln_stats<1>(acc, wr0, wc0, M, bias, resid, ldr, out, ldo, lane, lf);
    return;
  }
  constexpr bool FOLD = epi_is_lnfold(EPI);
  static_assert(!FOLD || MB <= 4, "one lane of a 16-lane row group per row of the wave tile");
  float own_mu = 0.f, own_rho = 0.f;
  if constexpr (FOLD) ln_row_own<MB>(lf.stats_in, wr0, M, lf.eps, lane, own_mu, own_rho);
  if (wr0 + MB * 16 <= M && wc0 + NB * 16 <= N) {
    float bv[NB], sv[NB];
#pragma unroll
    for (int n = 0; n < NB; ++n) bv[n] = bias[wc0 + n * 16 + c];
    if constexpr (FOLD) {
#pragma unroll
      for (int n = 0; n < NB; ++n) sv[n] = lf.s[wc0 + n * 16 + c];
    }
    const __amdgpu_buffer_rsrc_t rr = __builtin_amdgcn_make_buffer_rsrc(
        (void*)(resid + (EPI == EPI_RESID ? (int64_t)wr0 * ldr + wc0 : 0)), (short)0, 0x7fffffff, 0x00020000);
    const int rl = (4 * g * ldr + c) * 4;
    const __amdgpu_buffer_rsrc_t ro = __builtin_amdgcn_make_buffer_rsrc(
        (void*)(out + (int64_t)wr0 * ldo + wc0), (short)0, 0x7fffffff, 0x00020000);
    const int ol = (4 * g * ldo + c) * 4;
#pragma unroll
    for (int m = 0; m < MB; ++m) {
      float rv[NB][4];
      if constexpr (EPI == EPI_RESID) {
#pragma unroll
        for (int n = 0; n < NB; ++n)
#pragma unroll
          for (int e = 0; e < 4; ++e)
            rv[n][e] = __uint_as_float(
                __builtin_amdgcn_raw_buffer_load_b32(rr, rl, ((m * 16 + e) * ldr + n * 16) * 4, 0));
      }
      if constexpr (FOLD) {
#pragma unroll
        for (int e = 0; e < 4; ++e) {
          const float mu = ln_row_bcast(own_mu, lane, m, e), rho = ln_row_bcast(own_rho, lane, m, e);
#pragma unroll
          for (int n = 0; n < NB; ++n) {
            const float v = epi_apply<EPI>(__fmaf_rn(rho, __fmaf_rn(-mu, sv[n], acc[m][n][e]), bv[n]));
            __builtin_amdgcn_raw_buffer_store_b32(__float_as_uint(v), ro, ol, ((m * 16 + e) * ldo + n * 16) * 4, 0);
          }
        }
      } else {
#pragma unroll
        for (int n = 0; n < NB; ++n)
#pragma unroll
          for (int e = 0; e < 4; ++e) {
            float v = epi_apply<EPI>(acc[m][n][e] + bv[n]);
            if constexpr (EPI == EPI_RESID) v += rv[n][e];
            __builtin_amdgcn_raw_buffer_store_b32(__float_as_uint(v), ro, ol, ((m * 16 + e) * ldo + n * 16) * 4, 0);
          }
      }
    }
    return;
  }
  if constexpr (FOLD) {
#pragma unroll
    for (int m = 0; m < MB; ++m) {
      float mu[4], rho[4];
#pragma unroll
      for (int e = 0; e < 4; ++e) {
        mu[e] = ln_row_bcast(own_mu, lane, m, e);
        rho[e] = ln_row_bcast(own_rho, lane, m, e);
      }
#pragma unroll
      for (int n = 0; n < NB; ++n) {
        const int col = wc0 + n * 16 + c;
        if (col < N) {
          const float b = bias[col], sn = lf.s[col];
#pragma unroll
          for (int e = 0; e < 4; ++e) {
            const int row = wr0 + m * 16 + 4 * g + e;
            if (row < M)
              out[(int64_t)row * ldo + col] = epi_apply<EPI>(__fmaf_rn(rho[e], __fmaf_rn(-mu[e], sn, acc[m][n][e]), b));
          }
        }
      }
    }
    return;
  }
#pragma unroll
  for (int n = 0; n < NB; ++n) {
    const int col = wc0 + n * 16 + c;
    if (col >= N) continue;
    const float b = bias[col];
#pragma unroll
    for (int m = 0; m < MB; ++m)
#pragma unroll
      for (int e = 0; e < 4; ++e) {
        const int row = wr0 + m * 16 + 4 * g + e;
        if (row >= M) continue;
        float v = epi_apply<EPI>(acc[m][n][e] + b);
        if constexpr (EPI == EPI_RESID) v += resid[(int64_t)row * ldr + col];
        out[(int64_t)row * ldo + col] = v;
      }
  }
}

}
```

### mediquery-rag_amd/csrc/gemm_x6p.hip

```cpp
#include <algorithm>

#include "gemm_epi.hpp"
#include "gemm_x6p.hpp"

namespace mq {
namespace {

typedef __attribute__((address_space(3))) void x6p_lds_t;

__device__ __forceinline__ void x6p_glds(const void* base, unsigned voff, unsigned lds_dst) {
  const uint64_t b64 = (uint64_t)(uintptr_t)base;
  base = (const void*)(uintptr_t)(((uint64_t)__builtin_amdgcn_readfirstlane((unsigned)(b64 >> 32)) << 32) |
                                  (unsigned)__builtin_amdgcn_readfirstlane((unsigned)b64));
  unsigned keep;
  asm volatile("s_mov_b32 %0, m0\n\ts_mov_b32 m0, %3\n\ts_nop 0\n\tglobal_load_lds_dwordx4 %1, %2\n\ts_mov_b32 m0, %0"
               : "=&s"(keep)
               : "v"(voff), "s"(base), "s"(__builtin_amdgcn_readfirstlane(lds_dst))
               : "memory");
}

__device__ __forceinline__ int a_swz(int q) { return q ^ (q >> 1); }

typedef __bf16 bf16x2_t __attribute__((ext_vector_type(2)));
typedef float float2_t __attribute__((ext_vector_type(2)));
__device__ __forceinline__ unsigned cvt_pk_bf16(float lo, float hi) {
  float2_t v;
  v.x = lo;
  v.y = hi;
  return __builtin_bit_cast(unsigned, __builtin_convertvector(v, bf16x2_t));
}
__device__ __forceinline__ void split3v(floatx4 x, uint2 (&pl)[3]) {
#pragma unroll
  for (int p = 0; p < 3; ++p) {
    const unsigned a = cvt_pk_bf16(x.x, x.y), b = cvt_pk_bf16(x.z, x.w);
    pl[p] = make_uint2(a, b);
    if (p < 2) {
      x.x -= bf16_lo(a);
      x.y -= bf16_hi(a);
      x.z -= bf16_lo(b);
      x.w -= bf16_hi(b);
    }
  }
}

#if defined(MQ_X6P_DBG) && !defined(MQ_MEASUREMENT_BUILD)
#error "MQ_X6P_DBG computes wrong results: only a measurement build (-DMQ_MEASUREMENT_BUILD) may set it"
#endif

template <int WAVES_M_, int WAVES_N_, int TM_, int TN_, int NBUF_, int KS_ = 1, int DMAW_ = 8, bool SCHED_ = false,
          int DBG_ = 0, int DSTEP_ = 1, int BR0_ = 0, int PS_ = 4, bool LDR_ = false, bool M16_ = false,
          bool DEEP_ = false>
struct X6pTile {
  static constexpr int WAVES_M = WAVES_M_, WAVES_N = WAVES_N_, TM = TM_, TN = TN_, NBUF = NBUF_;
  static constexpr int KS = KS_;
  static constexpr int DMAW = DMAW_;
  static constexpr bool SCHED = SCHED_;
  static constexpr int DSTEP = DSTEP_, BR0 = BR0_, PS = PS_;
  static constexpr int DBG = DBG_;
  static constexpr bool LDR = LDR_;
  static constexpr bool M16 = M16_, DEEP = DEEP_;
  static constexpr int NW = WAVES_M * WAVES_N, THREADS = (LDR ? 2 * NW : NW) * 64;
  static constexpr int WM = TM * 32, WN = TN * 32, BM = WAVES_M * WM, BN = WAVES_N * WN;
  static constexpr int A_SUB = BM * 64;
  static constexpr int B_SUB = BN * 96;
  static constexpr int STAGE = KS * (A_SUB + B_SUB);
  static constexpr int NA = BM / 16, NB = BN / 32 * 3;
  static constexpr int NI = KS * (NA + NB);
  static constexpr int CNT_LO = NI / DMAW, REM = NI % DMAW, CNT_HI = CNT_LO + (REM ? 1 : 0);
  static_assert(DMAW == 8 || DMAW == 4, "DMA waves");
  static_assert(!LDR || DMAW == 4, "loader mode: the 4 loader waves issue every DMA");
  static constexpr int AHEAD = KS == 1 || (M16 && DEEP) ? NBUF : NBUF - 1;
  static_assert(!M16 || (KS == 2 && SCHED), "16x16x32 body: slot-scheduled 32-deep stages");
  static_assert(!DEEP || M16, "DEEP is a 16x16x32 option");
#ifndef MQ_X6P_GM
#define MQ_X6P_GM 4
#endif
  static constexpr int GM = MQ_X6P_GM;
  static_assert(LDR ? NW == 4 : NW == 8, "8-wave workgroups");
  static_assert(!SCHED || (CNT_HI - 1) * DSTEP < TM * TN * 6 * (M16 ? 4 : 1), "DMAs per k-step slots");
  static_assert(AHEAD >= 2 && NBUF * STAGE <= 160 * 1024, "LDS ring");
};

template <class T, int EPI, bool FORMER = false>
__global__ __launch_bounds__(T::THREADS, 1) void gemm_x6p_kernel(const float* __restrict__ A, int lda,
                                                             const unsigned char* __restrict__ W3,
                                                             const float* __restrict__ bias,
                                                             const float* __restrict__ resid, int ldr,
                                                             float* __restrict__ out, int ldo, int M, int N,
                                                             int K, int rx, LnFold lf) {
  __shared__ __attribute__((aligned(1024))) unsigned char lds[T::NBUF * T::STAGE];
  const unsigned lds0 = (unsigned)(uintptr_t)(x6p_lds_t*)lds;
  constexpr bool HAND = EPI == EPI_RESID_LN_STATS && T::LDR && T::M16 && !T::DEEP && T::NBUF == 3 && !FORMER;
  static_assert(!HAND || (T::NW == 4 && 2 * T::WM * T::WN * 4 <= T::STAGE && T::WN == kLnPartW && T::STAGE % 1024 == 0),
                "hand-off: two wave tiles of t per ring slot");
  const int lane = threadIdx.x & 63;
  const int wave = __builtin_amdgcn_readfirstlane(threadIdx.x >> 6);
  const int cw = T::LDR ? wave % T::NW : wave;
  const int wm = cw / T::WAVES_N, wn = cw % T::WAVES_N;
  const int tiles_m = (M + T::BM - 1) / T::BM, tiles_n = (N + T::BN - 1) / T::BN;
  const int total = tiles_m * tiles_n;
  const int G = gridDim.x, per_xcd = G >> 3;
  const int xslot = (blockIdx.x & 7) * per_xcd + (blockIdx.x >> 3);
  int m_lo = 0, rm = tiles_m, n_lo = 0, rn = tiles_n, loc = xslot, wstep = G, rtiles = total;
  if (rx > 0) {
    const Region rg = region_of(rx, blockIdx.x & 7, tiles_m, tiles_n);
    m_lo = rg.m_lo;
    rm = rg.rm;
    n_lo = rg.n_lo;
    rn = rg.rn;
    loc = blockIdx.x >> 3;
    wstep = per_xcd;
    rtiles = rm * rn;
  }
  const int n_tiles = loc < rtiles ? (rtiles - loc + wstep - 1) / wstep : 0;
  if (n_tiles == 0) return;
  const int nk = K >> 4;
  const int nst = nk / T::KS;
  const int S = n_tiles * nst;
  const int nbw = (N + 31) >> 5;
  const int band_tiles = T::GM * rn;
  auto coords = [&](int i, int& m0, int& n0) {
    const int t = i * wstep + loc;
    const int band = t / band_tiles;
    const int gm = min(T::GM, rm - band * T::GM);
    const int w = t - band * band_tiles;
    const int tc = w / gm;
    m0 = (m_lo + band * T::GM + (w - tc * gm)) * T::BM;
    n0 = (n_lo + tc) * T::BN;
  };

  int is_j = 0, is_i = 0, is_kt = 0, is_m0, is_n0;
  coords(0, is_m0, is_n0);
  const unsigned a_chunk = (unsigned)(((lane & 3) ^ a_swz((lane >> 4) & 3)) * 16);
  auto issue_one = [&](int buf, int t) __attribute__((always_inline)) {
    if constexpr (T::DBG & 1) return;
    if constexpr (T::DBG & 64) {
      if (is_j >= T::AHEAD) return;
    }
    const int dw = T::LDR ? wave - T::NW : wave;
    if (dw < 0 || dw >= T::DMAW || (T::REM && t == T::CNT_HI - 1 && dw >= T::REM)) return;
    const unsigned dst = lds0 + (unsigned)(buf * T::STAGE);
    const int ins = dw + t * T::DMAW;
    const int ks = ins / (T::NA + T::NB), in = ins - ks * (T::NA + T::NB);
    const int kt = is_kt + ks;
    if (in < T::NA) {
      if constexpr (T::DBG & 16) return;
      const float* abase = A + (int64_t)is_m0 * lda + kt * 16;
      const unsigned voff = (unsigned)min(16 * in + (lane >> 2), M - 1 - is_m0) * (unsigned)lda * 4u + a_chunk;
      x6p_glds(abase, voff, dst + ks * T::A_SUB + in * 1024);
    } else {
      if constexpr (T::DBG & 32) return;
      const int b = in - T::NA, nbl = b / 3, p = b - nbl * 3;
      const int nbg = min((is_n0 >> 5) + nbl, nbw - 1);
      const unsigned char* wbase = W3 + ((size_t)(nbg * nk + kt) * 3 + p) * 1024;
      x6p_glds(wbase, (unsigned)lane * 16u, dst + T::KS * T::A_SUB + ks * T::B_SUB + b * 1024);
    }
  };
  auto advance = [&]() __attribute__((always_inline)) {
    if (is_j + 1 < S) {
      ++is_j;
      is_kt += T::KS;
      if (is_kt == nk) {
        is_kt = 0;
        ++is_i;
        coords(is_i, is_m0, is_n0);
      }
    }
  };
  auto issue = [&](int buf) __attribute__((always_inline)) {
#pragma unroll
    for (int t = 0; t < T::CNT_HI; ++t) issue_one(buf, t);
    advance();
  };

  const int r = lane & 31, h = lane >> 5, sw = a_swz((r >> 2) & 3);
  const unsigned a_lo = (unsigned)((((2 * h) ^ sw) * 16)), a_hi = (unsigned)((((2 * h + 1) ^ sw) * 16));
  struct Frags {
    floatx4 raw[T::TM][2];
    bf16x8 a[T::TM][3], b[T::TN][3];
  };
  auto read_frags = [&](int buf, int ks, Frags& f) __attribute__((always_inline)) {
    if constexpr (T::DBG & 8) return;
    const unsigned char* st = lds + buf * T::STAGE;
#pragma unroll
    for (int tm = 0; tm < T::TM; ++tm) {
      const unsigned char* ar = st + ks * T::A_SUB + (wm * T::WM + tm * 32 + r) * 64;
      f.raw[tm][0] = *reinterpret_cast<const floatx4*>(ar + a_lo);
      f.raw[tm][1] = *reinterpret_cast<const floatx4*>(ar + a_hi);
    }
    const unsigned char* bs = st + T::KS * T::A_SUB + ks * T::B_SUB + lane * 16;
#pragma unroll
    for (int tn = 0; tn < T::TN; ++tn)
#pragma unroll
      for (int p = 0; p < 3; ++p)
        f.b[tn][p] = __builtin_bit_cast(bf16x8, *reinterpret_cast<const uintx4*>(bs + ((wn * T::TN + tn) * 3 + p) * 1024));
  };
  auto split_frags = [&](Frags& f) __attribute__((always_inline)) {
#pragma unroll
    for (int tm = 0; tm < T::TM; ++tm) {
      if constexpr (T::DBG & 2) {
        f.a[tm][0] = __builtin_bit_cast(bf16x8, f.raw[tm][0]);
        f.a[tm][1] = __builtin_bit_cast(bf16x8, f.raw[tm][1]);
        f.a[tm][2] = f.a[tm][0];
        continue;
      }
      uint2 pl[3], ph[3];
      split3v(f.raw[tm][0], pl);
      split3v(f.raw[tm][1], ph);
#pragma unroll
      for (int p = 0; p < 3; ++p) {
        uintx4 v;
        v.x = pl[p].x;
        v.y = pl[p].y;
        v.z = ph[p].x;
        v.w = ph[p].y;
        f.a[tm][p] = __builtin_bit_cast(bf16x8, v);
      }
    }
  };
  floatx16 acc[T::TM][T::TN];
  auto mma = [&](const Frags& f, auto&& hook) __attribute__((always_inline)) {
#pragma unroll
    for (int tm = 0; tm < T::TM; ++tm)
#pragma unroll
      for (int tn = 0; tn < T::TN; ++tn) {
        acc[tm][tn] = __builtin_amdgcn_mfma_f32_32x32x16_bf16(f.a[tm][2], f.b[tn][0], acc[tm][tn], 0, 0, 0);
        acc[tm][tn] = __builtin_amdgcn_mfma_f32_32x32x16_bf16(f.a[tm][1], f.b[tn][1], acc[tm][tn], 0, 0, 0);
        acc[tm][tn] = __builtin_amdgcn_mfma_f32_32x32x16_bf16(f.a[tm][0], f.b[tn][2], acc[tm][tn], 0, 0, 0);
        acc[tm][tn] = __builtin_amdgcn_mfma_f32_32x32x16_bf16(f.a[tm][1], f.b[tn][0], acc[tm][tn], 0, 0, 0);
        acc[tm][tn] = __builtin_amdgcn_mfma_f32_32x32x16_bf16(f.a[tm][0], f.b[tn][1], acc[tm][tn], 0, 0, 0);
        acc[tm][tn] = __builtin_amdgcn_mfma_f32_32x32x16_bf16(f.a[tm][0], f.b[tn][0], acc[tm][tn], 0, 0, 0);
        hook(tm * T::TN + tn);
      }
  };
  auto mma_one = [&](const Frags& f, int i) __attribute__((always_inline)) {
    const int g = i / 6, tm = g / T::TN, tn = g % T::TN, term = i % 6;
    const int pa = term == 0 ? 2 : term == 1 || term == 3 ? 1 : 0;
    const int pb = term == 0 || term >= 3 ? (term == 4 ? 1 : 0) : term == 1 ? 1 : 2;
    acc[tm][tn] = __builtin_amdgcn_mfma_f32_32x32x16_bf16(f.a[tm][pa], f.b[tn][pb], acc[tm][tn], 0, 0, 0);
  };
  auto read_a = [&](int buf, int ks, Frags& f) __attribute__((always_inline)) {
    if constexpr ((T::DBG & 8) || (T::DBG & 512)) {
#pragma unroll
      for (int tm = 0; tm < T::TM; ++tm) asm volatile("" : "+v"(f.raw[tm][0]), "+v"(f.raw[tm][1]));
      return;
    }
    const unsigned char* st = lds + buf * T::STAGE;
#pragma unroll
    for (int tm = 0; tm < T::TM; ++tm) {
      const unsigned char* ar = st + ks * T::A_SUB + (wm * T::WM + tm * 32 + r) * 64;
      f.raw[tm][0] = *reinterpret_cast<const floatx4*>(ar + a_lo);
      f.raw[tm][1] = *reinterpret_cast<const floatx4*>(ar + a_hi);
    }
  };
  auto read_b = [&](int buf, int ks, Frags& f, int q) __attribute__((always_inline)) {
    if constexpr ((T::DBG & 8) || (T::DBG & 256)) {
      asm volatile("" : "+v"(f.b[q / 3][q % 3]));
      return;
    }
    const unsigned char* bs = lds + buf * T::STAGE + T::KS * T::A_SUB + ks * T::B_SUB + lane * 16;
    f.b[q / 3][q % 3] = __builtin_bit_cast(bf16x8, *reinterpret_cast<const uintx4*>(bs + ((wn * T::TN) * 3 + q) * 1024));
  };
  unsigned pk[T::TM][2][3][2];
  auto piece = [&](Frags& f, int q) __attribute__((always_inline)) {
    const int tm = q / 12, half = (q / 6) % 2, p = (q % 6) / 2, part = q % 2;
    floatx4& x = f.raw[tm][half];
    unsigned u;
    if (part == 0) {
      u = cvt_pk_bf16(x.x, x.y);
      if (p < 2) {
        x.x -= bf16_lo(u);
        x.y -= bf16_hi(u);
      }
    } else {
      u = cvt_pk_bf16(x.z, x.w);
      if (p < 2) {
        x.z -= bf16_lo(u);
        x.w -= bf16_hi(u);
      }
    }
    asm volatile("" : "+v"(u), "+v"(x));
    pk[tm][half][p][part] = u;
  };
  auto assemble = [&](Frags& f) __attribute__((always_inline)) {
#pragma unroll
    for (int tm = 0; tm < T::TM; ++tm)
#pragma unroll
      for (int p = 0; p < 3; ++p) {
        uintx4 v;
        v.x = pk[tm][0][p][0];
        v.y = pk[tm][0][p][1];
        v.z = pk[tm][1][p][0];
        v.w = pk[tm][1][p][1];
        f.a[tm][p] = __builtin_bit_cast(bf16x8, v);
        asm volatile("" : "+v"(f.a[tm][p]));
      }
  };
  int c_i = 0, c_st = 0;
  auto tile_end = [&]() __attribute__((always_inline)) {
    if (++c_st == nst) {
      c_st = 0;
      int m0, n0;
      coords(c_i, m0, n0);
      if constexpr (!(T::DBG & 4))
        store_wave_tile<EPI, T::TM, T::TN>(acc, m0 + wm * T::WM, n0 + wn * T::WN, M, N, bias, resid, ldr, out, ldo,
                                           lane);
      zero_acc<T>(acc);
      ++c_i;
    }
  };
  auto wait_stages = [&](auto stages) __attribute__((always_inline)) {
    constexpr int n = decltype(stages)::value;
    const int dwi = T::LDR ? wave - T::NW : wave;
    if constexpr (T::DBG & 128) {
      if (T::REM && dwi >= 0 && dwi < T::REM)
        asm volatile("s_waitcnt vmcnt(%0)\n\ts_waitcnt lgkmcnt(0)" ::"n"(T::CNT_HI * n) : "memory");
      else
        asm volatile("s_waitcnt vmcnt(%0)\n\ts_waitcnt lgkmcnt(0)" ::"n"(T::CNT_LO * n) : "memory");
      return;
    }
    if (T::REM && dwi >= 0 && dwi < T::REM)
      asm volatile("s_waitcnt vmcnt(%0)" ::"n"(T::CNT_HI * n) : "memory");
    else
      asm volatile("s_waitcnt vmcnt(%0)" ::"n"(T::CNT_LO * n) : "memory");
    __builtin_amdgcn_s_waitcnt(0xC07F);
    asm volatile("s_barrier" ::: "memory");
  };
  zero_acc<T>(acc);

  if constexpr (T::LDR) {
    if (wave >= T::NW) {
#pragma unroll
      for (int d = 0; d < T::AHEAD; ++d) issue(d);
      wait_stages(IC<T::AHEAD - 1>{});
      if constexpr (HAND) {
        static_assert(T::AHEAD == 2, "hand-off: the ring two stages ahead");
        for (int j = 0; j + 2 < S; ++j) {
          wait_stages(IC<0>{});
          issue((j + 2) % T::NBUF);
        }
        if (S >= 2) wait_stages(IC<0>{});
        int m0, n0;
        coords(n_tiles - 1, m0, n0);
        LnTileRegs<2 * T::TM, 2 * T::TN> q;
        ln_tile_load(q, resid, ldr, m0 + wm * T::WM, n0 + wn * T::WN, M, lf, lane);
        wait_stages(IC<0>{});
        const int ts = (S + (cw >> 1)) % T::NBUF;
        ln_tile_write(q, lds + ts * T::STAGE + (cw & 1) * (T::WM * T::WN * 4), lf, lane);
        __builtin_amdgcn_s_waitcnt(0xC07F);
        asm volatile("s_barrier" ::: "memory");
        return;
      }
      for (int j = 0; j < S; ++j) {
        wait_stages(IC<T::AHEAD - 2>{});
        issue((j + T::AHEAD) % T::NBUF);
      }
      asm volatile("s_waitcnt vmcnt(0)" ::: "memory");
      return;
    }
  } else {
#pragma unroll
    for (int d = 0; d < T::AHEAD; ++d) issue(d);
  }
  if constexpr (T::M16) {
    constexpr int MB = 2 * T::TM, NB16 = 2 * T::TN, RS = NB16 * 6, NM16 = MB * RS, NSUB = 28;
    static_assert(RS >= NSUB + 4, "a region holds one block's split and its raw reads");
    const int c = lane & 15, kq = lane >> 4, hq = kq & 1, sw16 = a_swz((c >> 2) & 3);
    const unsigned a_base = (unsigned)((kq >> 1) * T::A_SUB + (wm * T::WM + c) * 64);
    const unsigned a_lo16 = a_base + (unsigned)(((2 * hq) ^ sw16) * 16);
    const unsigned a_hi16 = a_base + (unsigned)(((2 * hq + 1) ^ sw16) * 16);
    const unsigned b_base =
        (unsigned)(T::KS * T::A_SUB + (kq >> 1) * T::B_SUB + wn * T::TN * 3 * 1024 + hq * 512 + c * 16);
    floatx4 acc4[MB][NB16];
    uintx4 au[MB][3];
    bf16x8 bw[NB16][3];
    floatx4 raw[2];
    auto rd_raw = [&](const unsigned char* st, int m, int half) __attribute__((always_inline)) {
      raw[half] = *reinterpret_cast<const floatx4*>(st + m * 1024 + (half ? a_hi16 : a_lo16));
    };
    auto rd_b = [&](const unsigned char* st, int n, int p) __attribute__((always_inline)) {
      bw[n][p] = __builtin_bit_cast(
          bf16x8, *reinterpret_cast<const uintx4*>(st + b_base + ((n >> 1) * 3 + p) * 1024 + (n & 1) * 256));
    };
    auto sub = [&](int m, int q) __attribute__((always_inline)) {
      const int half = q / 14, rq = q % 14;
      const int p = rq < 12 ? rq / 6 : 2, part = rq < 12 ? (rq % 6) / 3 : rq - 12, op = rq < 12 ? rq % 3 : 0;
      floatx4& x = raw[half];
      if (op == 0) {
        unsigned u = cvt_pk_bf16(x[2 * part], x[2 * part + 1]);
        asm volatile("" : "+v"(u));
        au[m][p][2 * half + part] = u;
      } else {
        const unsigned u = au[m][p][2 * half + part];
        if (op == 1)
          x[2 * part] -= bf16_lo(u);
        else
          x[2 * part + 1] -= bf16_hi(u);
        asm volatile("" : "+v"(x));
      }
    };
    auto zero4 = [&]() __attribute__((always_inline)) {
#pragma unroll
      for (int m = 0; m < MB; ++m)
#pragma unroll
        for (int n = 0; n < NB16; ++n) acc4[m][n] = floatx4{0.f, 0.f, 0.f, 0.f};
    };
    zero4();
    wait_stages(IC<T::AHEAD - 1>{});
#pragma unroll
    for (int m = 0; m < MB; ++m) {
      rd_raw(lds, m, 0);
      rd_raw(lds, m, 1);
      if (m < MB - 1) {
#pragma unroll
        for (int q = 0; q < NSUB; ++q) sub(m, q);
      }
    }
#pragma unroll
    for (int n = 0; n < NB16; ++n)
#pragma unroll
      for (int p = 0; p < 3; ++p) rd_b(lds, n, p);
    int rb = 1 % T::NBUF;
    int ib = T::AHEAD % T::NBUF;
    for (int j = 0; j < S; ++j) {
      if constexpr (!T::LDR) {
        wait_stages(IC<T::AHEAD - 2>{});
      } else {
        if constexpr (T::DEEP) __builtin_amdgcn_s_waitcnt(0xC07F);
        asm volatile("s_barrier" ::: "memory");
      }
      const unsigned char* st = lds + rb * T::STAGE;
      static_for<NM16>([&](auto ic) {
        constexpr int i = decltype(ic)::value;
        constexpr int m = i / RS, w = i % RS, n = w / 6, term = w % 6;
        constexpr int pa = term == 0 ? 2 : term == 1 || term == 3 ? 1 : 0;
        constexpr int pb = term == 0 || term >= 3 ? (term == 4 ? 1 : 0) : term == 1 ? 1 : 2;
        acc4[m][n] = __builtin_amdgcn_mfma_f32_16x16x32_bf16(__builtin_bit_cast(bf16x8, au[m][pa]), bw[n][pb],
                                                             acc4[m][n], 0, 0, 0);
        if constexpr (w >= 2 && w < 2 + NSUB) sub((m + MB - 1) % MB, w - 2);
        if constexpr (w == 2 + NSUB || w == 3 + NSUB) rd_raw(st, m, w - 2 - NSUB);
        if constexpr (m == MB - 1 && term == 2) rd_b(st, n, 2);
        if constexpr (m == MB - 1 && term == 4) rd_b(st, n, 1);
        if constexpr (m == MB - 1 && term == 5) rd_b(st, n, 0);
        if constexpr (!T::LDR && i % T::DSTEP == 0 && i / T::DSTEP < T::CNT_HI) issue_one(ib, i / T::DSTEP);
        __builtin_amdgcn_sched_barrier(0);
      });
      if constexpr (!T::LDR) {
        advance();
        ib = ib + 1 == T::NBUF ? 0 : ib + 1;
      }
      rb = rb + 1 == T::NBUF ? 0 : rb + 1;
      if (++c_st == nst) {
        if constexpr (HAND) {
          if (j == S - 1) break;
        }
        c_st = 0;
        int m0, n0;
        coords(c_i, m0, n0);
        store_wave_tile16<EPI, MB, NB16>(acc4, m0 + wm * T::WM, n0 + wn * T::WN, M, N, bias, resid, ldr, out, ldo,
                                         lane, lf);
        zero4();
        ++c_i;
      }
    }
    if constexpr (HAND) {
      asm volatile("s_barrier" ::: "memory");
      int m0, n0;
      coords(n_tiles - 1, m0, n0);
      const int ts = (S + (cw >> 1)) % T::NBUF;
      store_wave_tile16_ln_stats<1, MB, NB16, true>(acc4, m0 + wm * T::WM, n0 + wn * T::WN, M, bias, resid, ldr, out,
                                                    ldo, lane, lf,
                                                    lds + ts * T::STAGE + (cw & 1) * (T::WM * T::WN * 4));
      return;
    }
    if constexpr (!T::LDR) asm volatile("s_waitcnt vmcnt(0)" ::: "memory");
    return;
  }
  wait_stages(IC<T::AHEAD - 1>{});
  Frags f0 = {}, f1 = {};
  read_frags(0, 0, f0);
  split_frags(f0);
  auto step = [&](int j, Frags& fa, Frags& fb) __attribute__((always_inline)) {
    wait_stages(IC<T::AHEAD - 2>{});
    const int buf = (j + T::AHEAD) % T::NBUF;
    if constexpr (!T::SCHED && !T::LDR) issue(buf);
    static_for<T::KS>([&](auto kc) {
      constexpr int ks = decltype(kc)::value;
      Frags& cur = ks % 2 == 0 ? fa : fb;
      Frags& nxt = ks % 2 == 0 ? fb : fa;
      if constexpr (T::SCHED) {
        constexpr int NM = T::TM * T::TN * 6, NBR = 3 * T::TN, PS = T::PS, NP = 12 * T::TM;
        constexpr int PER = (NP + (NM - PS) - 1) / (NM - PS);
        const int rbuf = ks + 1 < T::KS ? j % T::NBUF : (j + 1) % T::NBUF;
        constexpr int rks = ks + 1 < T::KS ? ks + 1 : 0;
        read_a(rbuf, rks, nxt);
        __builtin_amdgcn_sched_barrier(0);
        static_for<NM>([&](auto ic) {
          constexpr int i = decltype(ic)::value;
          mma_one(cur, i);
          constexpr bool dma_slot = !T::LDR && ks == 0 && i % T::DSTEP == 0 && i / T::DSTEP < T::CNT_HI;
          constexpr int bslot = [] {
            int n = 0;
            for (int k = T::BR0; k < i; ++k)
              if (!(!T::LDR && ks == 0 && k % T::DSTEP == 0 && k / T::DSTEP < T::CNT_HI) || T::DSTEP == 1) ++n;
            return n;
          }();
          if constexpr (i >= T::BR0 && (!dma_slot || T::DSTEP == 1)) {
            if constexpr (2 * bslot < NBR) read_b(rbuf, rks, nxt, 2 * bslot);
            if constexpr (2 * bslot + 1 < NBR) read_b(rbuf, rks, nxt, 2 * bslot + 1);
          }
          if constexpr (dma_slot) issue_one(buf, i / T::DSTEP);
          if constexpr (i >= PS) {
            static_for<PER>([&](auto pc) {
              constexpr int q = (i - PS) * PER + decltype(pc)::value;
              if constexpr (q < NP) piece(nxt, q);
            });
          }
          __builtin_amdgcn_sched_barrier(0);
        });
        assemble(nxt);
      } else {
        if constexpr (ks + 1 < T::KS)
          read_frags(j % T::NBUF, ks + 1, nxt);
        else
          read_frags((j + 1) % T::NBUF, 0, nxt);
        mma(cur, [](int) {});
        split_frags(nxt);
      }
    });
    if constexpr (T::SCHED && !T::LDR) advance();
    tile_end();
  };
  if constexpr (T::KS % 2 == 0) {
    for (int j = 0; j < S; ++j) step(j, f0, f1);
  } else {
    for (int j = 0; j < S; j += 2) {
      step(j, f0, f1);
      if (j + 1 >= S) break;
      step(j + 1, f1, f0);
    }
  }
  asm volatile("s_waitcnt vmcnt(0)" ::: "memory");
}

__global__ __launch_bounds__(256) void split_w3_kernel(const float* __restrict__ W, int N, int K,
                                                       uintx4* __restrict__ w3) {
  const int k8n = K >> 3, np = (N + 31) & ~31;
  const int64_t idx = (int64_t)blockIdx.x * 256 + threadIdx.x;
  if (idx >= (int64_t)np * k8n) return;
  const int n = (int)(idx / k8n), k8 = (int)(idx - (int64_t)n * k8n);
  floatx4 lo = {0.f, 0.f, 0.f, 0.f}, hi = lo;
  if (n < N) {
    lo = *reinterpret_cast<const floatx4*>(W + (int64_t)n * K + 8 * k8);
    hi = *reinterpret_cast<const floatx4*>(W + (int64_t)n * K + 8 * k8 + 4);
  }
  uint2 pl[3], ph[3];
  split3(lo, pl);
  split3(hi, ph);
  const int kb = k8 >> 1, hh = k8 & 1, nb = n >> 5, rr = n & 31;
#pragma unroll
  for (int p = 0; p < 3; ++p) {
    uintx4 v;
    v.x = pl[p].x;
    v.y = pl[p].y;
    v.z = ph[p].x;
    v.w = ph[p].y;
    w3[((int64_t)(nb * (K >> 4) + kb) * 3 + p) * 64 + hh * 32 + rr] = v;
  }
}

using X6p0 = X6pTile<2, 2, 2, 3, 3, 2, 4, true, 0, 1, 0, 6, true, true>;
using X6p1 = X6pTile<4, 1, 2, 3, 3, 2, 4, true, 0, 1, 0, 6, true, true>;
using X6p2 = X6pTile<4, 2, 1, 3, 3, 2, 4, true, 0, 2, 1, 6, false, true>;
using X6p3 = X6pTile<4, 2, 2, 3, 2, 2, 8, true, 0, 6, 1, 8, false, true, true>;
using X6p4 = X6pTile<2, 2, 2, 3, 3, 2, 4, true, 0, 1, 0, 6, true, true, true>;
using X6p5 = X6pTile<2, 2, 1, 3, 3, 2, 4, true, 0, 1, 0, 6, true, true, true>;
using X6p6 = X6pTile<4, 1, 2, 3, 3, 2, 4, true, 0, 1, 0, 6, true, true, true>;
using X6p7 = X6pTile<2, 2, 1, 3, 3, 2, 4, true, 0, 1, 0, 6, true, true>;
using X6p16 = X6pTile<2, 2, 2, 3, 4, 1, 4, true, 0, 1, 0, 6, true>;
using X6p17 = X6pTile<2, 2, 1, 3, 4, 1, 4, true, 0, 1, 0, 6, true>;

template <class T, int EPI, bool FORMER = false>
void launch_t(const X6pArgs& g, int num_cus, hipStream_t s) {
  if constexpr (EPI < EPI_RESID_LN_STATS) {
    if (g.K % (16 * T::KS) != 0) {
      launch_t<X6pTile<4, 2, 1, 3, 4>, EPI>(g, num_cus, s);
      return;
    }
  }
  const int tiles = ((g.M + T::BM - 1) / T::BM) * ((g.N + T::BN - 1) / T::BN);
  const int grid = (std::min(tiles, num_cus) + 7) / 8 * 8;
  const int tiles_m = (g.M + T::BM - 1) / T::BM, tiles_n = (g.N + T::BN - 1) / T::BN;
  int rx = g.rx;
  if (rx < 0) rx = region_pick_rx(tiles_m, tiles_n, (double)T::BM * g.K * 4, (double)T::BN * g.K * 6, grid);
  if (rx > 0 && (8 % rx != 0 || rx > tiles_n || 8 / rx > tiles_m || grid < 8)) rx = 0;
  hipLaunchKernelGGL((gemm_x6p_kernel<T, EPI, FORMER>), dim3(grid), dim3(T::THREADS), 0, s, g.A, g.lda,
                     static_cast<const unsigned char*>(g.W3), g.bias, g.resid, g.ldr, g.out, g.ldo, g.M, g.N, g.K, rx,
                     g.lf);
}

template <int EPI>
void launch_tile(const X6pArgs& g, int tile, int num_cus, hipStream_t s) {
#ifdef MQ_X6P_DBG
  if (tile >= 8) {
    switch (tile) {
      case 8: launch_t<X6pTile<2, 2, 2, 3, 4, 1, 4, true, 64, 1, 0, 6, true>, EPI>(g, num_cus, s); return;
      case 9: launch_t<X6pTile<2, 2, 2, 3, 4, 1, 4, true, 66, 1, 0, 6, true>, EPI>(g, num_cus, s); return;
      case 10: launch_t<X6pTile<2, 2, 2, 3, 4, 1, 4, true, 8, 1, 0, 6, true>, EPI>(g, num_cus, s); return;
      case 11: launch_t<X6pTile<2, 2, 2, 3, 4, 1, 4, true, 74, 1, 0, 6, true>, EPI>(g, num_cus, s); return;
      case 12: launch_t<X6pTile<2, 2, 2, 3, 4, 1, 4, true, 2, 1, 0, 6, true>, EPI>(g, num_cus, s); return;
      case 13: launch_t<X6pTile<2, 2, 2, 3, 4, 1, 4, true, 256, 1, 0, 6, true>, EPI>(g, num_cus, s); return;
      case 14: launch_t<X6pTile<2, 2, 2, 3, 4, 1, 4, true, 512, 1, 0, 6, true>, EPI>(g, num_cus, s); return;
      default: launch_t<X6pTile<2, 2, 2, 3, 4, 1, 4, true, 128, 1, 0, 6, true>, EPI>(g, num_cus, s); return;
    }
  }
#endif
  switch (tile) {
    case 1: launch_t<X6p1, EPI>(g, num_cus, s); return;
    case 2: launch_t<X6p2, EPI>(g, num_cus, s); return;
    case 3: launch_t<X6p3, EPI>(g, num_cus, s); return;
    case 4: launch_t<X6p4, EPI>(g, num_cus, s); return;
    case 5: launch_t<X6p5, EPI>(g, num_cus, s); return;
    case 6: launch_t<X6p6, EPI>(g, num_cus, s); return;
    case 7: launch_t<X6p7, EPI>(g, num_cus, s); return;
    case 16: launch_t<X6p16, EPI>(g, num_cus, s); return;
    case 17: launch_t<X6p17, EPI>(g, num_cus, s); return;
    default: launch_t<X6p0, EPI>(g, num_cus, s); return;
  }
}

template <int EPI>
void launch_tile_fold(const X6pArgs& g, int tile, int num_cus, hipStream_t s) {
  constexpr bool HAS_FORMER = EPI == EPI_RESID_LN_STATS;
  switch (tile) {
    case 1: launch_t<X6p1, EPI>(g, num_cus, s); return;
    case 20: launch_t<X6p0, EPI, HAS_FORMER>(g, num_cus, s); return;
    case 21: launch_t<X6p1, EPI, HAS_FORMER>(g, num_cus, s); return;
    default: launch_t<X6p0, EPI>(g, num_cus, s); return;
  }
}

__global__ __launch_bounds__(256) void ln_fold_weight_kernel(const float* __restrict__ W,
                                                             const float* __restrict__ bias,
                                                             const float* __restrict__ g,
                                                             const float* __restrict__ b, int N, int K,
                                                             float* __restrict__ Wg, float* __restrict__ s_out,
                                                             float* __restrict__ c_out) {
  const int lane = threadIdx.x & 63;
  const int n = blockIdx.x * 4 + (threadIdx.x >> 6);
  if (n >= N) return;
  double sg = 0.0, sb = 0.0;
  for (int k = lane; k < K; k += 64) {
    const float w = W[(int64_t)n * K + k];
    const float wg = g[k] * w;
    Wg[(int64_t)n * K + k] = wg;
    sg += (double)wg;
    sb += (double)b[k] * (double)w;
  }
#pragma unroll
  for (int off = 32; off > 0; off >>= 1) {
    sg += __shfl_xor(sg, off);
    sb += __shfl_xor(sb, off);
  }
  if (lane == 0) {
    s_out[n] = (float)sg;
    c_out[n] = (float)((double)bias[n] + sb);
  }
}

}

void launch_ln_fold_weight(const float* W, const float* bias, const float* g, const float* b, int N, int K, float* Wg,
                           float* s_out, float* c_out, hipStream_t s) {
  hipLaunchKernelGGL(ln_fold_weight_kernel, dim3((unsigned)((N + 3) / 4)), dim3(256), 0, s, W, bias, g, b, N, K, Wg,
                     s_out, c_out);
}

void launch_split_w3(const float* W, int N, int K, void* w3, hipStream_t s) {
  const int64_t n = (int64_t)((N + 31) & ~31) * (K >> 3);
  hipLaunchKernelGGL(split_w3_kernel, dim3((unsigned)((n + 255) / 256)), dim3(256), 0, s, W, N, K,
                     static_cast<uintx4*>(w3));
}

int x6p_pick_tile(int M, int N, int num_cus) {
  auto rounds = [&](int bm, int bn) {
    const int64_t tiles = (int64_t)((M + bm - 1) / bm) * ((N + bn - 1) / bn);
    return (tiles + num_cus - 1) / num_cus;
  };
  return rounds(256, 96) < rounds(128, 192) ? 1 : 0;
}

void launch_gemm_x6p(const X6pArgs& g, int epi, int tile, int num_cus, hipStream_t s) {
  if (tile < 0) {
    tile = x6p_pick_tile(g.M, g.N, num_cus);
  }
  switch (epi) {
    case EPI_GELU_ERF: launch_tile<EPI_GELU_ERF>(g, tile, num_cus, s); return;
    case EPI_GELU_TANH: launch_tile<EPI_GELU_TANH>(g, tile, num_cus, s); return;
    case EPI_RESID: launch_tile<EPI_RESID>(g, tile, num_cus, s); return;
    case EPI_RESID_LN_STATS: launch_tile_fold<EPI_RESID_LN_STATS>(g, tile, num_cus, s); return;
    case EPI_BIAS_LNFOLD: launch_tile_fold<EPI_BIAS_LNFOLD>(g, tile, num_cus, s); return;
    case EPI_GELU_ERF_LNFOLD: launch_tile_fold<EPI_GELU_ERF_LNFOLD>(g, tile, num_cus, s); return;
    case EPI_GELU_TANH_LNFOLD: launch_tile_fold<EPI_GELU_TANH_LNFOLD>(g, tile, num_cus, s); return;
    default: launch_tile<EPI_BIAS>(g, tile, num_cus, s); return;
  }
}

}

extern "C" {

int64_t mq_debug_w3_bytes(int N, int K) { return N > 0 && K > 0 && K % 16 == 0 ? (int64_t)mq::w3_bytes(N, K) : -1; }

int mq_debug_split_w3(const float* W, int N, int K, void* w3, void* stream) {
  using namespace mq;
  clear_error();
  MQ_CHECK_ARG(W && w3, "NULL buffer");
  MQ_CHECK_ARG(N > 0 && K > 0 && K % 16 == 0, "bad shape N=%d K=%d", N, K);
  launch_split_w3(W, N, K, w3, (hipStream_t)stream);
  MQ_HIP(hipGetLastError());
  return MQ_OK;
}

int mq_debug_gemm_x6p(const float* A, const void* W3, const float* bias, const float* resid, float* out, int M,
                      int N, int K, int epi, int tile, void* stream) {
  using namespace mq;
  clear_error();
  MQ_CHECK_ARG(A && W3 && bias && out && (epi != EPI_RESID || resid), "NULL buffer");
  MQ_CHECK_ARG(M > 0 && N > 0 && K > 0 && K % 32 == 0, "bad shape M=%d N=%d K=%d", M, N, K);
  const int rx = tile >= 100 ? tile / 100 - 1 : -1;
  if (tile >= 100) tile %= 100;
  MQ_CHECK_ARG(epi >= 0 && epi <= 3 && tile >= -1 && tile <= 17 && rx <= 8, "bad epi/tile");
  int dev = 0, cus = 256;
  (void)hipGetDevice(&dev);
  (void)hipDeviceGetAttribute(&cus, hipDeviceAttributeMultiprocessorCount, dev);
  X6pArgs g{A, K, W3, bias, resid, N, out, N, M, N, K};
  g.rx = rx;
  launch_gemm_x6p(g, epi, tile, cus, (hipStream_t)stream);
  MQ_HIP(hipGetLastError());
  return MQ_OK;
}

int mq_debug_ln_fold_weight(const float* W, const float* bias, const float* g, const float* b, int N, int K,
                            float* Wg, float* s_out, float* c_out, void* stream) {
  using namespace mq;
  clear_error();
  MQ_CHECK_ARG(W && bias && g && b && Wg && s_out && c_out, "NULL buffer");
  MQ_CHECK_ARG(N > 0 && K > 0, "bad shape N=%d K=%d", N, K);
  launch_ln_fold_weight(W, bias, g, b, N, K, Wg, s_out, c_out, (hipStream_t)stream);
  MQ_HIP(hipGetLastError());
  return MQ_OK;
}

int mq_debug_gemm_x6p_ln(const float* A, const void* W3, const float* bias, const float* resid, float* out, int M,
                         int N, int K, int epi, int tile, const float* stats_in, float* stats_out, const float* g,
                         const float* b, const float* s_fold, float eps, void* stream) {
  using namespace mq;
  clear_error();
  MQ_CHECK_ARG(A && W3 && bias && out, "NULL buffer");
  MQ_CHECK_ARG(M > 0 && N > 0 && K > 0 && K % 32 == 0, "bad shape M=%d N=%d K=%d", M, N, K);
  MQ_CHECK_ARG((tile >= -1 && tile <= 1) || tile == 20 || tile == 21,
               "the LayerNorm-fold epilogues run on tiles 0 and 1 (20 / 21: their former epilogues; got %d)", tile);
  if (epi == EPI_RESID_LN_STATS) {
    MQ_CHECK_ARG(resid && stats_out && (!stats_in || (g && b)), "producer: NULL buffer");
    MQ_CHECK_ARG(N == kLnPartW * kLnMaxParts, "producer: N must be %d (got %d)", kLnPartW * kLnMaxParts, N);
    MQ_CHECK_ARG((int64_t)M * N < (1ll << 29), "producer: M * N must stay below 2^29 (32-bit byte offsets)");
  } else {
    MQ_CHECK_ARG(epi_is_lnfold(epi), "epi must be a LayerNorm-fold kind (got %d)", epi);
    MQ_CHECK_ARG(stats_in && s_fold, "consumer: NULL buffer");
    MQ_CHECK_ARG(K == kLnPartW * kLnMaxParts, "consumer: K must be %d (got %d)", kLnPartW * kLnMaxParts, K);
  }
  int dev = 0, cus = 256;
  (void)hipGetDevice(&dev);
  (void)hipDeviceGetAttribute(&cus, hipDeviceAttributeMultiprocessorCount, dev);
  X6pArgs a{A, K, W3, bias, resid, N, out, N, M, N, K};
  a.lf.stats_in = stats_in;
  a.lf.stats_out = stats_out;
  a.lf.g = g;
  a.lf.b = b;
  a.lf.s = s_fold;
  a.lf.eps = eps;
  launch_gemm_x6p(a, epi, tile, cus, (hipStream_t)stream);
  MQ_HIP(hipGetLastError());
  return MQ_OK;
}

}
```

### mediquery-rag_amd/csrc/gemm_x6p.hpp

```cpp
#pragma once

#include <hip/hip_runtime.h>

#include <cstddef>
#include <cstdint>

namespace mq {

inline size_t w3_bytes(int64_t N, int64_t K) { return (size_t)((N + 31) / 32) * (size_t)(K / 16) * 3 * 1024; }
inline size_t w3_row_offset(int64_t row0, int64_t K) { return (size_t)(row0 / 32) * (size_t)(K / 16) * 3 * 1024; }

inline int region_pick_rx(int64_t tiles_m, int64_t tiles_n, double a_bytes_per_row_tile,
                          double w_bytes_per_col_tile, int64_t grid) {
  if (tiles_m * tiles_n <= grid || grid < 8) return 0;
  const double l2 = 4.0 * 1024 * 1024;
  const int64_t per_xcd = grid / 8;
  int best = 0;
  double best_b = 0;
  for (int rx = 1; rx <= 8; rx *= 2) {
    const int ry = 8 / rx;
    if (rx > tiles_n || ry > tiles_m) continue;
    const int64_t rm = (tiles_m + ry - 1) / ry, rn = (tiles_n + rx - 1) / rx;
    const int64_t rounds = (rm * rn + per_xcd - 1) / per_xcd;
    const double w = (double)rn * w_bytes_per_col_tile;
    const double b = (double)rm * a_bytes_per_row_tile + (w <= l2 ? w : w * (double)rounds);
    if (best == 0 || b < best_b) {
      best = rx;
      best_b = b;
    }
  }
  return best;
}
struct Region {
  int m_lo, rm, n_lo, rn;
};
__host__ __device__ inline Region region_of(int rx, int xc, int tiles_m, int tiles_n) {
  const int ry = 8 / rx, ri = xc / rx, rj = xc - ri * rx;
  Region r;
  r.m_lo = ri * tiles_m / ry;
  r.rm = (ri + 1) * tiles_m / ry - r.m_lo;
  r.n_lo = rj * tiles_n / rx;
  r.rn = (rj + 1) * tiles_n / rx - r.n_lo;
  return r;
}

void launch_split_w3(const float* W, int N, int K, void* w3, hipStream_t s);

constexpr int kLnPartW = 96;
constexpr int kLnMaxParts = 8;
struct LnFold {
  const float* stats_in = nullptr;
  float* stats_out = nullptr;
  const float* g = nullptr;
  const float* b = nullptr;
  const float* s = nullptr;
  float eps = 0.f;
};
void launch_ln_fold_weight(const float* W, const float* bias, const float* g, const float* b, int N, int K, float* Wg,
                           float* s_out, float* c_out, hipStream_t s);

struct X6pArgs {
  const float* A;
  int lda;
  const void* W3;
  const float* bias;
  const float* resid;
  int ldr;
  float* out;
  int ldo;
  int M, N, K;
  int rx = -1;
  LnFold lf{};
};

int x6p_pick_tile(int M, int N, int num_cus);
void launch_gemm_x6p(const X6pArgs& g, int epi, int tile, int num_cus, hipStream_t s);

}
```

### mediquery-rag_amd/mediquery_hip/_lib.py

```python
import ctypes
import hashlib
import os

try:
    import torch
except Exception:
    torch = None

LIB_PATH = os.environ.get("MQ_LIB_PATH") or os.path.join(os.path.dirname(os.path.abspath(__file__)),
                                                          "libmqhip.so")

MQ_OK = 0
MQ_DTYPE_F32, MQ_DTYPE_BF16, MQ_DTYPE_F32X6, MQ_DTYPE_F32_SCREEN = 0, 1, 2, 3
MQ_GELU_ERF, MQ_GELU_TANH = 0, 1
MQ_POOL_CLS, MQ_POOL_MEAN = 0, 1
MQ_MAX_K = 64
MQ_HEAD_MAX_LABELS = 8
MQ_MASK_SET, MQ_MASK_AND, MQ_MASK_OR, MQ_MASK_CLEAR = 0, 1, 2, 3
MQ_CONTAINS_MAX_BYTES = 256
MQ_CONTAINS_SPAN_BYTES = 16384
MQ_ENC_OPT_ROWS_MAX, MQ_ENC_OPT_ROWS_SPLITS, MQ_ENC_OPT_SPLITK_MAX = 0, 1, 2
MQ_ENC_OPT_LN_ROWS_PER_WAVE, MQ_ENC_OPT_FUSE_ATTN_OPROJ, MQ_ENC_OPT_FUSED_LN = 3, 4, 5
MQ_ENC_OPT_SPLITK_TILES, MQ_ENC_OPT_LN_ON_LOAD, MQ_ENC_OPT_RESIDENT_LAYERS = 6, 7, 8
MQ_ENC_OPT_X6_PRESPLIT = 9
MQ_ENC_OPT_ROWS_PLANES = 10
MQ_ENC_OPT_LN_FOLD = 11
MQ_ENC_OPT_CLS_KFREE = 12


class MQError(RuntimeError):

    def __init__(self, fn, code, msg):
        super().__init__("%s failed (status %d): %s" % (fn, code, msg))
        self.code = code


class BertConfigC(ctypes.Structure):
    _fields_ = [("vocab_size", ctypes.c_int), ("hidden", ctypes.c_int), ("layers", ctypes.c_int),
                ("heads", ctypes.c_int), ("ffn", ctypes.c_int), ("max_positions", ctypes.c_int),
                ("type_vocab", ctypes.c_int), ("ln_eps", ctypes.c_float), ("gelu", ctypes.c_int),
                ("pooling", ctypes.c_int)]

    @classmethod
    def from_config(cls, cfg):
        return cls(cfg.vocab_size, cfg.hidden, cfg.layers, cfg.heads, cfg.ffn, cfg.max_positions,
                   cfg.type_vocab, cfg.ln_eps, cfg.gelu, cfg.pooling)


_P = ctypes.c_void_p
_I = ctypes.c_int
_I64 = ctypes.c_int64
_PP = ctypes.POINTER(ctypes.c_void_p)

SIGNATURES = {
    "mq_last_error": (ctypes.c_char_p, []),
    "mq_version": (ctypes.c_char_p, []),
    "mq_build_source_hash": (ctypes.c_char_p, []),
    "mq_device_count": (_I, []),
    "mq_index_create": (_I, [_I, _I, _I64, _I, _PP]),
    "mq_index_destroy": (_I, [_P]),
    "mq_index_size": (_I, [_P, ctypes.POINTER(_I64)]),
    "mq_index_dim": (_I, [_P, ctypes.POINTER(_I)]),
    "mq_index_add": (_I, [_P, _P, _I64, _I, _P]),
    "mq_index_reset": (_I, [_P]),
    "mq_index_search": (_I, [_P, _P, _I64, _I, _P, _P, _I, _P]),
    "mq_index_get": (_I, [_P, _I64, _I64, _P, _I, _P]),
    "mq_index_select": (_I, [_P, _P, _I64, _P]),
    "mq_index_data": (_I, [_P, _PP]),
    "mq_index_set_precision": (_I, [_P, _I]),
    "mq_index_set_stream_threshold": (_I, [_P, _I]),
    "mq_index_set_threshold_scan": (_I, [_P, _I]),
    "mq_index_set_int8_screen": (_I, [_P, _I]),
    "mq_index_set_async_screen": (_I, [_P, _I]),
    "mq_index_rescans": (_I, [_P, _P, _P]),
    "mq_index_screen_fallbacks": (_I, [_P, _P, _P]),
    "mq_index_screen_skips": (_I, [_P, _P, _P]),
    "mq_index_set_timing": (_I, [_P, _I]),
    "mq_index_read_timing": (_I, [_P, _P, _I]),
    "mq_index_save": (_I, [_P, ctypes.c_char_p]),
    "mq_index_load": (_I, [_P, ctypes.c_char_p]),
    "mq_index_save_rows": (_I, [_P, ctypes.c_char_p, ctypes.c_int64, ctypes.c_int64]),
    "mq_index_load_append": (_I, [_P, ctypes.c_char_p]),
    "mq_mask_eval": (_I, [_P, _I64, _P, _I, _P, _I, _P]),
    "mq_mask_eval_bits": (_I, [_P, _I64, _P, _I, _P, _I, _P]),
    "mq_mask_combine": (_I, [_P, _P, _I64, _I, _P]),
    "mq_mask_contains": (_I, [_P, _I64, _P, _I64, _P, _I, _I, _P, _I, _P, _P]),
    "mq_index_search_masked": (_I, [_P, _P, _I, _P, _P, _P, _I, _P]),
    "mq_index_search_masked_batch": (_I, [_P, _P, _I64, _I, _P, _P, _P, _I, _P]),
    "mq_index_masked_gathers": (_I, [_P, ctypes.POINTER(_I64)]),
    "mq_index_mmr_select": (_I, [_P, _P, _P, _I64, _I, _I, ctypes.c_float, _P, _P, _I, _P]),
    "mq_index_search_mmr": (_I, [_P, _P, _I64, _I, _I, ctypes.c_float, _P, _P, _P, _I, _P]),
    "mq_topk_merge_host": (_I, [_P, _P, _I, _I64, _I, _I, _P, _P]),
    "mq_topk_merge_device": (_I, [_P, _P, _I, _I64, _I, _I, _P, _P, _P]),
    "mq_encoder_create": (_I, [_I, ctypes.POINTER(BertConfigC), _PP]),
    "mq_encoder_destroy": (_I, [_P]),
    "mq_encoder_weight_count": (_I64, [ctypes.POINTER(BertConfigC)]),
    "mq_encoder_load_weights": (_I, [_P, _P, _I64]),
    "mq_encoder_set_precision": (_I, [_P, _I]),
    "mq_encoder_set_graphs": (_I, [_P, _I]),
    "mq_encoder_set_option": (_I, [_P, _I, _I]),
    "mq_encoder_get_option": (_I, [_P, _I, ctypes.POINTER(ctypes.c_int)]),
    "mq_encoder_set_timing": (_I, [_P, _I]),
    "mq_encoder_read_timing": (_I, [_P, _P, _I]),
    "mq_encoder_embed": (_I, [_P, _P, _P, _I, _I, _P, _I, _P]),
    "mq_encoder_load_head": (_I, [_P, _P, _P, _P, _P, _I]),
    "mq_encoder_score": (_I, [_P, _P, _P, _P, _I, _I, _P, _I, _P]),
    "mq_tokenizer_create_wordpiece": (_I, [ctypes.c_char_p, _I, _I, _PP]),
    "mq_tokenizer_create_wordpiece_tokens": (_I, [ctypes.POINTER(ctypes.c_char_p), _I, _I, _I, _PP]),
    "mq_tokenizer_create_char": (_I, [_I, _I, _PP]),
    "mq_tokenizer_destroy": (_I, [_P]),
    "mq_tokenizer_encode_batch": (_I, [_P, ctypes.POINTER(ctypes.c_char_p), _I, _I, _P, _P,
                                       ctypes.POINTER(_I)]),
    "mq_tokenizer_encode_pairs": (_I, [_P, ctypes.POINTER(ctypes.c_char_p), ctypes.POINTER(ctypes.c_char_p), _I, _I,
                                       _P, _P, _P, ctypes.POINTER(_I)]),
    "mq_debug_cls_head": (_I, [_P, _I, _I, _P, _P, _P, _P, _I, _P, _P]),
    "mq_debug_gemm_f32": (_I, [_P, _P, _P, _P, _P, _I, _I, _I, _I, _I, _P]),
    "mq_debug_w3_bytes": (_I64, [_I, _I]),
    "mq_debug_split_w3": (_I, [_P, _I, _I, _P, _P]),
    "mq_debug_gemm_x6p": (_I, [_P, _P, _P, _P, _P, _I, _I, _I, _I, _I, _P]),
    "mq_debug_gemm_x6p_ln": (_I, [_P, _P, _P, _P, _P, _I, _I, _I, _I, _I, _P, _P, _P, _P, _P, ctypes.c_float, _P]),
    "mq_debug_ln_fold_weight": (_I, [_P, _P, _P, _P, _I, _I, _P, _P, _P, _P]),
    "mq_debug_attention": (_I, [_P, _P, _I, _I, _I, _I, ctypes.c_float, _I, _P, _P]),
    "mq_debug_cls_attention": (_I, [_P, _P, _P, _P, _P, ctypes.c_float, _P, _I, _I, _I, _I, ctypes.c_float, _P, _P, _P,
                                    _P, _P]),
    "mq_debug_attn_oproj": (_I, [_P, _P, _I, _I, _I, _I, ctypes.c_float, _P, _P, _P, _I, _I, _I, _I, _P, _P]),
    "mq_debug_int8_screen":(_I, [_P, _P, _I, _P, _P, _P]),
}

_lib = None


def lib():
    global _lib
    if _lib is None:
        if not os.path.exists(LIB_PATH):
            raise ImportError("libmqhip.so not found at %s - build it with "
                              "`make -C mediquery-rag_amd/csrc` or __graft_entry__.build()" % LIB_PATH)
        h = ctypes.CDLL(LIB_PATH)
        allow_missing = os.environ.get("MQ_LIB_ALLOW_MISSING") == "1"
        for name, (res, args) in SIGNATURES.items():
            if allow_missing and not hasattr(h, name):
                continue
            fn = getattr(h, name)
            fn.restype = res
            fn.argtypes = args
        _lib = h
    return _lib


def check(fn_name, rc):
    if rc != MQ_OK:
        raise MQError(fn_name, rc, lib().mq_last_error().decode("utf-8", "replace"))
    return rc


def call(fn_name, *args):
    return check(fn_name, getattr(lib(), fn_name)(*args))


CSRC = os.path.join(os.path.dirname(os.path.dirname(os.path.abspath(__file__))), "csrc")
_STAMPED_EXT = (".hip", ".cpp", ".hpp", ".inc")


def tree_source_hash(csrc=CSRC):
    names = sorted(f for f in os.listdir(csrc) if f.endswith(_STAMPED_EXT))
    paths = [os.path.join(csrc, f) for f in names]
    paths += [os.path.join(csrc, "Makefile"), os.path.join(csrc, "..", "..", "include", "mq.h")]
    h = hashlib.sha256()
    for p in paths:
        with open(p, "rb") as f:
            h.update(f.read())
    return h.hexdigest()[:16]


def built_source_hash():
    return lib().mq_build_source_hash().decode()


def check_build_fresh():
    if not os.path.isdir(CSRC):
        return
    built, tree = built_source_hash(), tree_source_hash()
    if built != tree:
        raise ImportError("libmqhip.so at %s was built from sources %s, the tree holds %s: "
                          "rebuild with `make -C mediquery-rag_amd/csrc`" % (LIB_PATH, built, tree))


def device_count():
    return lib().mq_device_count()


def ptr(a):
    if a is None:
        return None
    if isinstance(a, int):
        return ctypes.c_void_p(a)
    if hasattr(a, "data_ptr"):
        return ctypes.c_void_p(a.data_ptr())
    return ctypes.c_void_p(a.ctypes.data)


class device_scope:

    def __init__(self, device):
        self._ctx = None
        if device is not None and torch is not None and torch.cuda.is_available():
            self._ctx = torch.cuda.device(int(device))

    def __enter__(self):
        if self._ctx is not None:
            self._ctx.__enter__()
        return self

    def __exit__(self, *exc):
        if self._ctx is not None:
            return self._ctx.__exit__(*exc)
        return False


def stream_handle(stream=None):
    if stream is None:
        if torch is None or not torch.cuda.is_available():
            return None
        stream = torch.cuda.current_stream()
    if isinstance(stream, int):
        return ctypes.c_void_p(stream)
    return ctypes.c_void_p(stream.cuda_stream)
```

### mediquery-rag_amd/mediquery_hip/native.py

```python
import ctypes

import numpy as np

from . import _lib
from .config import BertConfig
from .weights import head_from_state_dict, state_dict_to_blob, synthetic_state_dict


class FlatIndex:

    def __init__(self, dim=768, capacity=0, device=0, dtype=_lib.MQ_DTYPE_F32):
        h = ctypes.c_void_p()
        _lib.call("mq_index_create", device, dim, capacity, dtype, ctypes.byref(h))
        self._h = h
        self.dim = dim
        self.device = device

    def close(self):
        h, self._h = getattr(self, "_h", None), None
        if h:
            try:
                _lib.lib().mq_index_destroy(h)
            except Exception:
                pass

    __del__ = close

    def __len__(self):
        n = ctypes.c_int64()
        _lib.call("mq_index_size", self._h, ctypes.byref(n))
        return n.value

    def add(self, rows):
        rows = np.ascontiguousarray(rows, dtype=np.float32).reshape(-1, self.dim)
        _lib.call("mq_index_add", self._h, _lib.ptr(rows), rows.shape[0], 0, None)

    def add_device(self, rows, stream=None):
        assert rows.is_cuda and rows.dtype.is_floating_point and rows.is_contiguous()
        _lib.call("mq_index_add", self._h, _lib.ptr(rows), rows.shape[0], 1,
                  _lib.stream_handle(stream))

    def reset(self):
        _lib.call("mq_index_reset", self._h)

    def search(self, queries, k):
        q = np.ascontiguousarray(queries, dtype=np.float32).reshape(-1, self.dim)
        scores = np.empty((q.shape[0], k), dtype=np.float32)
        ids = np.empty((q.shape[0], k), dtype=np.int64)
        _lib.call("mq_index_search", self._h, _lib.ptr(q), q.shape[0], k, _lib.ptr(scores),
                  _lib.ptr(ids), 0, None)
        return scores, ids

    def search_device(self, queries, k, out_scores, out_ids, stream=None):
        _lib.call("mq_index_search", self._h, _lib.ptr(queries), queries.shape[0], k,
                  _lib.ptr(out_scores), _lib.ptr(out_ids), 1, _lib.stream_handle(stream))

    def get(self, row0=0, n=None):
        n = len(self) - row0 if n is None else n
        out = np.empty((n, self.dim), dtype=np.float32)
        _lib.call("mq_index_get", self._h, row0, n, _lib.ptr(out), 0, None)
        return out

    def select(self, rows, out=None):
        rows = np.ascontiguousarray(rows, dtype=np.int64).reshape(-1)
        out = FlatIndex(dim=self.dim, device=self.device) if out is None else out
        _lib.call("mq_index_select", self._h, _lib.ptr(rows), rows.size, out._h)
        return out

    def data_ptr(self):
        p = ctypes.c_void_p()
        _lib.call("mq_index_data", self._h, ctypes.byref(p))
        return p.value

    STAGES = ("flat_search_kernel", "merge_kernel")

    def set_precision(self, dtype):
        _lib.call("mq_index_set_precision", self._h, dtype)

    def set_stream_threshold(self, max_queries):
        _lib.call("mq_index_set_stream_threshold", self._h, int(max_queries))

    def set_threshold_scan(self, enabled=True):
        _lib.call("mq_index_set_threshold_scan", self._h, int(bool(enabled)))

    def set_int8_screen(self, enabled=True):
        _lib.call("mq_index_set_int8_screen", self._h, int(bool(enabled)))

    def set_async_screen(self, enabled=True):
        _lib.call("mq_index_set_async_screen", self._h, int(bool(enabled)))

    @property
    def rescans(self):
        n = ctypes.c_int64()
        _lib.call("mq_index_rescans", self._h, ctypes.byref(n), None)
        return n.value

    @property
    def remerges(self):
        n = ctypes.c_int64()
        _lib.call("mq_index_rescans", self._h, None, ctypes.byref(n))
        return n.value

    @property
    def screen_fallbacks(self):
        n = ctypes.c_int64()
        _lib.call("mq_index_screen_fallbacks", self._h, ctypes.byref(n), None)
        return n.value

    @property
    def screen_passdowns(self):
        n = ctypes.c_int64()
        _lib.call("mq_index_screen_fallbacks", self._h, None, ctypes.byref(n))
        return n.value

    @property
    def screen_skips(self):
        n = ctypes.c_int64()
        _lib.call("mq_index_screen_skips", self._h, ctypes.byref(n), None)
        return n.value

    @property
    def int8_skips(self):
        n = ctypes.c_int64()
        _lib.call("mq_index_screen_skips", self._h, None, ctypes.byref(n))
        return n.value

    def set_timing(self, enabled=True):
        _lib.call("mq_index_set_timing", self._h, int(bool(enabled)))

    def read_timing(self):
        ms = np.zeros(len(self.STAGES), dtype=np.float32)
        _lib.call("mq_index_read_timing", self._h, _lib.ptr(ms), len(ms))
        return dict(zip(self.STAGES, ms.tolist()))

    def save(self, path):
        _lib.call("mq_index_save", self._h, str(path).encode())

    def load(self, path):
        _lib.call("mq_index_load", self._h, str(path).encode())

    def _check_bits(self, bits):
        check_mask_words(bits, len(self), self.device)

    def search_masked(self, queries, k, bits):
        q = np.ascontiguousarray(queries, dtype=np.float32).reshape(-1, self.dim)
        self._check_bits(bits)
        scores = np.empty((q.shape[0], k), dtype=np.float32)
        ids = np.empty((q.shape[0], k), dtype=np.int64)
        with _lib.device_scope(self.device):
            _lib.call("mq_index_search_masked_batch", self._h, _lib.ptr(q), q.shape[0], k, _lib.ptr(bits),
                      _lib.ptr(scores), _lib.ptr(ids), 0, _lib.stream_handle(None))
        return scores, ids

    def mmr_select(self, cand_scores, cand_ids, k, lambda_mult=0.5):
        s = np.ascontiguousarray(cand_scores, dtype=np.float32)
        i = np.ascontiguousarray(cand_ids, dtype=np.int64)
        s = s.reshape(1, -1) if s.ndim == 1 else s
        i = i.reshape(s.shape)
        scores = np.empty((s.shape[0], k), dtype=np.float32)
        ids = np.empty((s.shape[0], k), dtype=np.int64)
        with _lib.device_scope(self.device):
            _lib.call("mq_index_mmr_select", self._h, _lib.ptr(s), _lib.ptr(i), s.shape[0], s.shape[1], k,
                      float(lambda_mult), _lib.ptr(scores), _lib.ptr(ids), 0, _lib.stream_handle(None))
        return scores, ids

    def mmr_select_device(self, cand_scores, cand_ids, k, lambda_mult, out_scores, out_ids, stream=None):
        _lib.call("mq_index_mmr_select", self._h, _lib.ptr(cand_scores), _lib.ptr(cand_ids),
                  cand_scores.shape[0], cand_scores.shape[1], k, float(lambda_mult), _lib.ptr(out_scores),
                  _lib.ptr(out_ids), 1, _lib.stream_handle(stream))

    def search_mmr(self, queries, k, fetch_k, lambda_mult=0.5, bits=None):
        q = np.ascontiguousarray(queries, dtype=np.float32).reshape(-1, self.dim)
        if bits is not None:
            self._check_bits(bits)
        scores = np.empty((q.shape[0], k), dtype=np.float32)
        ids = np.empty((q.shape[0], k), dtype=np.int64)
        with _lib.device_scope(self.device):
            _lib.call("mq_index_search_mmr", self._h, _lib.ptr(q), q.shape[0], k, fetch_k, float(lambda_mult),
                      _lib.ptr(bits), _lib.ptr(scores), _lib.ptr(ids), 0, _lib.stream_handle(None))
        return scores, ids

    @property
    def masked_gathers(self):
        n = ctypes.c_int64()
        _lib.call("mq_index_masked_gathers", self._h, ctypes.byref(n))
        return n.value

    def save_rows(self, path, row0, n):
        _lib.call("mq_index_save_rows", self._h, str(path).encode(), int(row0), int(n))

    def load_append(self, path):
        _lib.call("mq_index_load_append", self._h, str(path).encode())


def merge_topk_host(scores, ids, k_out):
    scores = np.ascontiguousarray(scores, dtype=np.float32)
    ids = np.ascontiguousarray(ids, dtype=np.int64)
    n_lists, nq, k_in = scores.shape
    os_ = np.empty((nq, k_out), dtype=np.float32)
    oi = np.empty((nq, k_out), dtype=np.int64)
    _lib.call("mq_topk_merge_host", _lib.ptr(scores), _lib.ptr(ids), n_lists, nq, k_in, k_out,
              _lib.ptr(os_), _lib.ptr(oi))
    return os_, oi


def merge_topk_device(scores, ids, k_out, out_scores, out_ids, stream=None):
    n_lists, nq, k_in = scores.shape
    _lib.call("mq_topk_merge_device", _lib.ptr(scores), _lib.ptr(ids), n_lists, nq, k_in, k_out,
              _lib.ptr(out_scores), _lib.ptr(out_ids), _lib.stream_handle(stream))


class Encoder:

    def __init__(self, cfg: BertConfig, weights=None, seed=0, device=0):
        self.cfg = cfg
        self.device = device
        self._ccfg = _lib.BertConfigC.from_config(cfg)
        h = ctypes.c_void_p()
        _lib.call("mq_encoder_create", device, ctypes.byref(self._ccfg), ctypes.byref(h))
        self._h = h
        sd = weights if weights is not None else synthetic_state_dict(cfg, seed)
        blob = state_dict_to_blob(cfg, sd)
        n = _lib.lib().mq_encoder_weight_count(ctypes.byref(self._ccfg))
        if n != blob.size:
            raise ValueError("weight blob %d floats, library expects %d" % (blob.size, n))
        _lib.call("mq_encoder_load_weights", self._h, _lib.ptr(blob), blob.size)
        self.n_labels = 0

    def close(self):
        h, self._h = getattr(self, "_h", None), None
        if h:
            try:
                _lib.lib().mq_encoder_destroy(h)
            except Exception:
                pass

    __del__ = close

    STAGES = ("embed_ln", "qkv_gemm", "attention", "out_proj_gemm", "layernorm", "ffn_up_gemm",
              "ffn_down_gemm", "pool")

    def set_timing(self, enabled=True):
        _lib.call("mq_encoder_set_timing", self._h, int(bool(enabled)))

    def read_timing(self):
        ms = np.zeros(len(self.STAGES), dtype=np.float32)
        _lib.call("mq_encoder_read_timing", self._h, _lib.ptr(ms), len(ms))
        return dict(zip(self.STAGES, ms.tolist()))

    def set_precision(self, dtype):
        _lib.call("mq_encoder_set_precision", self._h, dtype)

    def set_graphs(self, enabled=True):
        _lib.call("mq_encoder_set_graphs", self._h, int(bool(enabled)))

    OPTIONS = {"rows_max": _lib.MQ_ENC_OPT_ROWS_MAX, "rows_splits": _lib.MQ_ENC_OPT_ROWS_SPLITS,
               "splitk_max": _lib.MQ_ENC_OPT_SPLITK_MAX, "ln_rows_per_wave": _lib.MQ_ENC_OPT_LN_ROWS_PER_WAVE,
               "fuse_attn_oproj": _lib.MQ_ENC_OPT_FUSE_ATTN_OPROJ, "fused_ln": _lib.MQ_ENC_OPT_FUSED_LN,
               "splitk_tiles": _lib.MQ_ENC_OPT_SPLITK_TILES, "ln_on_load": _lib.MQ_ENC_OPT_LN_ON_LOAD,
               "resident_layers": _lib.MQ_ENC_OPT_RESIDENT_LAYERS, "x6_presplit": _lib.MQ_ENC_OPT_X6_PRESPLIT,
               "rows_planes": _lib.MQ_ENC_OPT_ROWS_PLANES, "ln_fold": _lib.MQ_ENC_OPT_LN_FOLD,
               "cls_kfree": _lib.MQ_ENC_OPT_CLS_KFREE}

    def set_option(self, name, value):
        _lib.call("mq_encoder_set_option", self._h, self.OPTIONS[name], int(value))

    def get_option(self, name):
        v = ctypes.c_int()
        _lib.call("mq_encoder_get_option", self._h, self.OPTIONS[name], ctypes.byref(v))
        return v.value

    def embed(self, ids, mask):
        ids = np.ascontiguousarray(ids, dtype=np.int32)
        mask = np.ascontiguousarray(mask, dtype=np.int32)
        B, L = ids.shape
        out = np.empty((B, self.cfg.hidden), dtype=np.float32)
        _lib.call("mq_encoder_embed", self._h, _lib.ptr(ids), _lib.ptr(mask), B, L, _lib.ptr(out),
                  0, None)
        return out

    def embed_device(self, ids, mask, out, stream=None):
        B, L = ids.shape
        _lib.call("mq_encoder_embed", self._h, _lib.ptr(ids), _lib.ptr(mask), B, L, _lib.ptr(out),
                  1, _lib.stream_handle(stream))

    def load_head(self, sd):
        pw, pb, cw, cb = head_from_state_dict(sd, self.cfg)
        n_labels = int(cw.shape[0])
        if not 1 <= n_labels <= _lib.MQ_HEAD_MAX_LABELS:
            raise ValueError("n_labels must be in [1, %d] (got %d)" % (_lib.MQ_HEAD_MAX_LABELS, n_labels))
        _lib.call("mq_encoder_load_head", self._h, _lib.ptr(pw), _lib.ptr(pb), _lib.ptr(cw), _lib.ptr(cb), n_labels)
        self.n_labels = n_labels

    def score(self, ids, types, mask):
        ids = np.ascontiguousarray(ids, dtype=np.int32)
        types = np.ascontiguousarray(types, dtype=np.int32)
        mask = np.ascontiguousarray(mask, dtype=np.int32)
        if types.shape != ids.shape or mask.shape != ids.shape or ids.ndim != 2:
            raise ValueError("ids, types and mask must share one [B, L] shape")
        B, L = ids.shape
        out = np.empty((B, max(1, self.n_labels)), dtype=np.float32)
        _lib.call("mq_encoder_score", self._h, _lib.ptr(ids), _lib.ptr(types), _lib.ptr(mask), B, L,
                  _lib.ptr(out), 0, None)
        return out

    def score_device(self, ids, types, mask, out, stream=None):
        if tuple(types.shape) != tuple(ids.shape) or tuple(mask.shape) != tuple(ids.shape):
            raise ValueError("ids, types and mask must share one [B, L] shape")
        B, L = ids.shape
        if out.numel() < B * max(1, self.n_labels):
            raise ValueError("out holds %d floats, needs B * n_labels = %d" % (out.numel(), B * self.n_labels))
        _lib.call("mq_encoder_score", self._h, _lib.ptr(ids), _lib.ptr(types), _lib.ptr(mask), B, L,
                  _lib.ptr(out), 1, _lib.stream_handle(stream))


def check_mask_words(bits, n, device=None):
    if not (getattr(bits, "is_cuda", False) and bits.element_size() == 4 and bits.is_contiguous()
            and bits.numel() >= (int(n) + 31) // 32):
        raise ValueError("bits must be a contiguous 32-bit device tensor of >= ceil(n / 32) = %d words"
                         % ((int(n) + 31) // 32))
    if device is not None and bits.device.index != int(device):
        raise ValueError("bits lives on cuda:%s, the index on cuda:%d" % (bits.device.index, int(device)))


def _check_codes(codes, bits):
    import torch
    if not (getattr(codes, "is_cuda", False) and codes.dtype == torch.int32 and codes.is_contiguous()):
        raise ValueError("codes must be a contiguous int32 device tensor")
    check_mask_words(bits, codes.numel(), codes.device.index)


def mask_eval(codes, lut, bits, mode, stream=None):
    import torch
    _check_codes(codes, bits)
    if not (getattr(lut, "is_cuda", False) and lut.dtype == torch.uint8 and lut.is_contiguous()
            and lut.device == codes.device and lut.numel() >= 1):
        raise ValueError("lut must be a non-empty contiguous uint8 tensor on the codes' device")
    with _lib.device_scope(codes.device.index):
        _lib.call("mq_mask_eval", _lib.ptr(codes), codes.numel(), _lib.ptr(lut), lut.numel(), _lib.ptr(bits),
                  mode, _lib.stream_handle(stream))


def mask_eval_bits(codes, lut, bits, mode, stream=None):
    _check_codes(codes, bits)
    lut = np.asarray(lut).astype(bool)
    if not 1 <= lut.size <= 256:
        raise ValueError("a by-value table holds 1..256 entries (got %d)" % lut.size)
    words = np.zeros(4, dtype=np.uint64)
    for i in np.flatnonzero(lut).tolist():
        words[i >> 6] |= np.uint64(1 << (i & 63))
    with _lib.device_scope(codes.device.index):
        _lib.call("mq_mask_eval_bits", _lib.ptr(codes), codes.numel(), _lib.ptr(words), len(lut), _lib.ptr(bits),
                  mode, _lib.stream_handle(stream))


def mask_contains(text, offsets, pattern, bits, mode, negate=False, stream=None, scratch=None):
    import torch
    if not (getattr(text, "is_cuda", False) and text.dtype == torch.uint8 and text.is_contiguous()
            and text.dim() == 1):
        raise ValueError("text must be a contiguous 1-d uint8 device tensor")
    if text.numel() and text.data_ptr() % 16:
        raise ValueError("text must start at a 16-byte aligned address")
    if not (getattr(offsets, "is_cuda", False) and offsets.dtype == torch.int64 and offsets.is_contiguous()
            and offsets.numel() >= 1 and offsets.device == text.device):
        raise ValueError("offsets must be a contiguous int64 tensor of n + 1 elements on the text's device")
    n = offsets.numel() - 1
    check_mask_words(bits, n, text.device.index)
    if not isinstance(pattern, (bytes, bytearray)) or not 1 <= len(pattern) <= _lib.MQ_CONTAINS_MAX_BYTES:
        raise ValueError("pattern must be 1..%d bytes" % _lib.MQ_CONTAINS_MAX_BYTES)
    with _lib.device_scope(text.device.index):
        if scratch is None:
            scratch = torch.empty(max(1, (n + 31) // 32), dtype=torch.int32, device=text.device)
        check_mask_words(scratch, n, text.device.index)
        if scratch.data_ptr() == bits.data_ptr():
            raise ValueError("scratch must not be bits")
        _lib.call("mq_mask_contains", _lib.ptr(text), text.numel(), _lib.ptr(offsets), n, bytes(pattern),
                  len(pattern), int(bool(negate)), _lib.ptr(bits), mode, _lib.ptr(scratch),
                  _lib.stream_handle(stream))


def mask_combine(dst, src, mode, stream=None):
    check_mask_words(dst, 0)
    if src is not None:
        check_mask_words(src, 32 * dst.numel(), dst.device.index)
    with _lib.device_scope(dst.device.index):
        _lib.call("mq_mask_combine", _lib.ptr(dst), _lib.ptr(src), dst.numel(), mode, _lib.stream_handle(stream))
```

Measured before the change: 38060.

## Fuse L=32 attention into the x6p QKV GEMM epilogue

Adds an attention epilogue to the 3-way bf16-split QKV GEMM. When sequence length is 32 and the shape fits, each 128x192 tile holds Q, K and V for one head, so scores, masked softmax and P·V are computed in-register with MFMA and only the context is written. This removes the round trip of the QKV activation through global memory and a separate attention launch. It also adds a standalone attn32 kernel used when the fused path is not taken, plus synchronisation between the loader and partner waves. Risks are a longer epilogue that stalls the GEMM pipeline, extra barriers, and a narrow shape gate.

Result: faster. 39350, median of 6 (+3.4%).

```diff
diff --git a/include/mq.h b/include/mq.h
--- a/include/mq.h
+++ b/include/mq.h
@@ -127,6 +127,7 @@
 #define MQ_ENC_OPT_ROWS_PLANES 10
 #define MQ_ENC_OPT_LN_FOLD 11
 #define MQ_ENC_OPT_CLS_KFREE 12
+#define MQ_ENC_OPT_QKV_ATTN 13
 int mq_encoder_set_option(mq_encoder* enc, int option, int value);
 int mq_encoder_get_option(const mq_encoder* enc, int option, int* value);
 int mq_encoder_set_timing(mq_encoder* enc, int enabled);
@@ -165,6 +166,10 @@
                          float eps, void* stream);
 int mq_debug_ln_fold_weight(const float* W, const float* bias, const float* g, const float* b, int N,
                             int K, float* Wg, float* s_out, float* c_out, void* stream);
+int mq_debug_gemm_x6p_attn(const float* A, const void* W3, const float* bias, const int* mask,
+                           float* ctx, int M, int K, int heads, float scale, int epi,
+                           const float* stats_in, const float* s_fold, float eps, int max_workgroups,
+                           void* stream);
 int mq_debug_attention(const float* qkv, const int* mask, int B, int L, int H, int heads, float scale,
                        int variant, float* ctx, void* stream);
 int mq_debug_cls_attention(const float* q, const float* x, const float* stats, const float* ln_g,
diff --git a/mediquery-rag_amd/csrc/encoder.hip b/mediquery-rag_amd/csrc/encoder.hip
--- a/mediquery-rag_amd/csrc/encoder.hip
+++ b/mediquery-rag_amd/csrc/encoder.hip
@@ -1898,6 +1898,10 @@
 #define MQ_CLS_KFREE_DEFAULT 1
 #endif
 constexpr bool kClsKfreeDefault = MQ_CLS_KFREE_DEFAULT != 0;
+#ifndef MQ_QKV_ATTN_DEFAULT
+#define MQ_QKV_ATTN_DEFAULT 1
+#endif
+constexpr bool kQkvAttnDefault = MQ_QKV_ATTN_DEFAULT != 0;
 
 enum Stage { ST_EMBED = 0, ST_QKV, ST_ATTN, ST_OPROJ, ST_LN, ST_FFN_UP, ST_FFN_DOWN, ST_POOL, ST_N };
 
@@ -1943,6 +1947,7 @@
   Buf wfold3, wfoldf, sfold;
   bool rows_planes = false;
   bool cls_kfree = kClsKfreeDefault;
+  bool qkv_attn = kQkvAttnDefault;
   Buf wkt;
   Buf cls;
   Buf head;
@@ -2207,6 +2212,11 @@
   float* fst2 = e->lnst.p + (size_t)2 * M * nt;
   bool raw = false;
   bool pooled = false;
+  const bool attn_shape = e->qkv_attn && e->precision == MQ_DTYPE_F32X6 && L == 32 && H == 64 * c.heads &&
+                          H % 192 == 0 && H % 32 == 0 && M > 256 && !lnl &&
+                          (int64_t)((M + 127) / 128) * ((3 * H + 191) / 192) >= e->num_cus &&
+                          x6p_pick_tile(M, 3 * H, e->num_cus) == 0 && (int64_t)M * H < (1ll << 29);
+  const bool qkv_attn = attn_shape && e->x6_presplit;
   auto fold_gemm = [&](auto epi, GemmArgs g, int stage) {
     e->tl.mark(s, stage);
     if (!e->x6_presplit) g.W3 = nullptr;
@@ -2242,6 +2252,8 @@
     const float* qkv_in = y_pending ? e->y.p : e->x.p;
     const int lnt = M <= 256 && (int)li >= e->resident_layers ? 1 : 0;
     const bool fold_layer = fold && !(cls_only && L > 1);
+    bool attn_done = false;
+    bool attn_after = false;
     auto qkv_fold = [&](GemmArgs g, int row0) {
       g.W = w.wqkvgf ? w.wqkvgf + (int64_t)row0 * H : nullptr;
       g.W3 = w.wqkvg3 ? w.wqkvg3 + w3_row_offset(row0, H) : nullptr;
@@ -2293,18 +2305,34 @@
       GemmArgs q{e->slab.p, e->slab.n, e->x.p, L * H, w.wqkv, w.bqkv, nullptr, 0, e->qkv.p, L * 3 * H, B, H, H, lnt};
       q.W3 = w.wqkv3;
       gemm<EPI_BIAS>(e, q, ST_QKV, s);
+    } else if (qkv_attn && (raw ? w.wqkvg3 != nullptr : w.wqkv3 != nullptr)) {
+      X6pArgs a{qkv_in, H, raw ? w.wqkvg3 : w.wqkv3, raw ? w.wqkvc : w.bqkv, nullptr, 0, e->ctx.p, H, M, 3 * H, H};
+      if (raw) {
+        a.lf.s = w.wqkvs;
+        a.lf.stats_in = fst2;
+        a.lf.eps = c.ln_eps;
+      }
+      a.at.mask = mask;
+      a.at.scale = scale;
+      e->tl.mark(s, ST_QKV);
+      launch_gemm_x6p(a, raw ? EPI_ATTN_LNFOLD : EPI_ATTN_BIAS, 0, e->num_cus, s);
+      attn_done = true;
     } else {
       GemmArgs qkv{e->slab.p, e->slab.n, qkv_in, H, w.wqkv, w.bqkv, nullptr, 0, e->qkv.p, 3 * H, M, 3 * H, H};
       qkv.W3 = w.wqkv3;
       qkv_gemm(qkv);
+      attn_after = attn_shape;
     }
     y_pending = false;
     const bool resid_raw = raw && fold_layer;
     raw = false;
-    if (!kfree) {
+    if (!kfree && !attn_done) {
       e->tl.mark(s, ST_ATTN);
       const int qt = cls_only ? 1 : q_tiles;
-      launch_attention(B, L, c.heads, qt, H, scale, e->qkv.p, mask, e->ctx.p, s);
+      if (attn_after)
+        launch_attn32(e->qkv.p, mask, e->ctx.p, M, H, scale, s);
+      else
+        launch_attention(B, L, c.heads, qt, H, scale, e->qkv.p, mask, e->ctx.p, s);
     }
     const bool lnl_layer = lnl && !cls_only;
     GemmArgs oproj{e->slab.p, e->slab.n, e->ctx.p, stride, w.wo, w.bo, resid, ldr, e->y.p, H, rows, H, H, lnt};
@@ -3033,6 +3061,10 @@
       MQ_CHECK_ARG(value == 0 || value == 1, "cls_kfree must be 0 or 1 (got %d)", value);
       e->cls_kfree = value != 0;
       break;
+    case MQ_ENC_OPT_QKV_ATTN:
+      MQ_CHECK_ARG(value == 0 || value == 1, "qkv_attn must be 0 or 1 (got %d)", value);
+      e->qkv_attn = value != 0;
+      break;
     default:
       MQ_FAIL(MQ_EINVAL, "unknown encoder option %d", option);
   }
@@ -3058,6 +3090,7 @@
     case MQ_ENC_OPT_ROWS_PLANES: *value = e->rows_planes ? 1 : 0; break;
     case MQ_ENC_OPT_LN_FOLD: *value = e->ln_fold ? 1 : 0; break;
     case MQ_ENC_OPT_CLS_KFREE: *value = e->cls_kfree ? 1 : 0; break;
+    case MQ_ENC_OPT_QKV_ATTN: *value = e->qkv_attn ? 1 : 0; break;
     default: MQ_FAIL(MQ_EINVAL, "unknown encoder option %d", option);
   }
   return MQ_OK;
diff --git a/mediquery-rag_amd/csrc/gemm_epi.hpp b/mediquery-rag_amd/csrc/gemm_epi.hpp
--- a/mediquery-rag_amd/csrc/gemm_epi.hpp
+++ b/mediquery-rag_amd/csrc/gemm_epi.hpp
@@ -14,9 +14,12 @@
   EPI_RESID_LN_STATS = 5,
   EPI_BIAS_LNFOLD = 6,
   EPI_GELU_ERF_LNFOLD = 7,
-  EPI_GELU_TANH_LNFOLD = 8
+  EPI_GELU_TANH_LNFOLD = 8,
+  EPI_ATTN_BIAS = 9,
+  EPI_ATTN_LNFOLD = 10
 };
 constexpr bool epi_is_lnfold(int epi) { return epi >= EPI_BIAS_LNFOLD && epi <= EPI_GELU_TANH_LNFOLD; }
+constexpr bool epi_is_attn(int epi) { return epi == EPI_ATTN_BIAS || epi == EPI_ATTN_LNFOLD; }
 
 __device__ __forceinline__ float gelu_erf(float x) {
   const float z = fabsf(x) * 0.70710678118654752f;
@@ -389,4 +392,146 @@
   }
 }
 
-}
+constexpr int kAttnSt = 36;
+constexpr int kAttnStage = 64 * kAttnSt * 4;
+template <bool FOLD, bool PRE = false>
+__device__ __forceinline__ void attn_wave_tile(floatx4 (&acc)[4][6], int wr0, int head, int wn, int M, int H,
+                                               const float* __restrict__ bias, const LnFold& lf,
+                                               const int* __restrict__ mask, float scale,
+                                               float* __restrict__ ctx, int lane, unsigned char* stg,
+                                               const unsigned char* partner) {
+  static_assert(kAttnStage >= 8 * 1024, "the partials of two sequences fit the staging");
+  const int c = lane & 15, g = lane >> 4;
+  const unsigned long long kbits = __ballot(mask[min(wr0 + lane, M - 1)] != 0);
+  float own_mu = 0.f, own_rho = 0.f;
+  if constexpr (FOLD) ln_row_own<4>(lf.stats_in, wr0, M, lf.eps, lane, own_mu, own_rho);
+  if constexpr (PRE) {
+#pragma unroll
+    for (int m = 0; m < 4; ++m)
+#pragma unroll
+      for (int n = 0; n < 2; ++n)
+#pragma unroll
+        for (int e = 0; e < 4; ++e) acc[m][n][e] = acc[m][n][e] * scale;
+  } else {
+    float bv[6], sv[6];
+#pragma unroll
+    for (int n = 0; n < 6; ++n) {
+      const int col = (n >> 1) * H + 64 * head + 32 * wn + 16 * (n & 1) + c;
+      bv[n] = bias[col];
+      if constexpr (FOLD) sv[n] = lf.s[col];
+    }
+#pragma unroll
+    for (int m = 0; m < 4; ++m)
+#pragma unroll
+      for (int e = 0; e < 4; ++e) {
+        float mu = 0.f, rho = 0.f;
+        if constexpr (FOLD) {
+          mu = ln_row_bcast(own_mu, lane, m, e);
+          rho = ln_row_bcast(own_rho, lane, m, e);
+        }
+#pragma unroll
+        for (int n = 0; n < 6; ++n) {
+          float v;
+          if constexpr (FOLD)
+            v = __fmaf_rn(rho, __fmaf_rn(-mu, sv[n], acc[m][n][e]), bv[n]);
+          else
+            v = acc[m][n][e] + bv[n];
+          acc[m][n][e] = n < 2 ? v * scale : v;
+        }
+      }
+  }
+  float* sf = reinterpret_cast<float*>(stg);
+  floatx4 sp[2][2][2];
+#pragma unroll
+  for (int s = 0; s < 2; ++s) {
+#pragma unroll
+    for (int t = 0; t < 2; ++t)
+#pragma unroll
+      for (int mb = 0; mb < 2; ++mb)
+#pragma unroll
+        for (int nd = 0; nd < 2; ++nd)
+#pragma unroll
+          for (int e = 0; e < 4; ++e)
+            sf[(32 * t + 16 * mb + 4 * g + e) * kAttnSt + 16 * nd + c] = acc[2 * s + mb][2 * t + nd][e];
+    floatx4 qf[2][2], kf[2][2];
+#pragma unroll
+    for (int blk = 0; blk < 2; ++blk)
+#pragma unroll
+      for (int hf = 0; hf < 2; ++hf) {
+        qf[blk][hf] = *reinterpret_cast<const floatx4*>(&sf[(16 * blk + c) * kAttnSt + 16 * hf + 4 * g]);
+        kf[blk][hf] = *reinterpret_cast<const floatx4*>(&sf[(32 + 16 * blk + c) * kAttnSt + 16 * hf + 4 * g]);
+      }
+#pragma unroll
+    for (int kb = 0; kb < 2; ++kb)
+#pragma unroll
+      for (int qb = 0; qb < 2; ++qb) {
+        floatx4 st = {0.f, 0.f, 0.f, 0.f};
+#pragma unroll
+        for (int i = 0; i < 8; ++i)
+          st = __builtin_amdgcn_mfma_f32_16x16x4f32(kf[kb][i >> 2][i & 3], qf[qb][i >> 2][i & 3], st, 0, 0, 0);
+        sp[s][kb][qb] = st;
+      }
+  }
+#pragma unroll
+  for (int i = 0; i < 8; ++i)
+    *reinterpret_cast<floatx4*>(stg + i * 1024 + lane * 16) = sp[i >> 2][(i >> 1) & 1][i & 1];
+  asm volatile("s_waitcnt lgkmcnt(0)\n\ts_barrier" ::: "memory");
+#pragma unroll
+  for (int i = 0; i < 8; ++i)
+    sp[i >> 2][(i >> 1) & 1][i & 1] += *reinterpret_cast<const floatx4*>(partner + i * 1024 + lane * 16);
+#pragma unroll
+  for (int s = 0; s < 2; ++s) {
+    const unsigned kb32 = (unsigned)(kbits >> (32 * s));
+    float inv[2];
+#pragma unroll
+    for (int qb = 0; qb < 2; ++qb) {
+      float mx = -INFINITY;
+#pragma unroll
+      for (int kb = 0; kb < 2; ++kb)
+#pragma unroll
+        for (int e = 0; e < 4; ++e) {
+          const bool live = (kb32 >> (16 * kb + 4 * g + e)) & 1u;
+          sp[s][kb][qb][e] = live ? sp[s][kb][qb][e] : -INFINITY;
+          mx = fmaxf(mx, sp[s][kb][qb][e]);
+        }
+      mx = fmaxf(mx, __shfl_xor(mx, 16));
+      mx = fmaxf(mx, __shfl_xor(mx, 32));
+      float l = 0.f;
+#pragma unroll
+      for (int kb = 0; kb < 2; ++kb)
+#pragma unroll
+        for (int e = 0; e < 4; ++e) {
+          const float v = sp[s][kb][qb][e];
+          const float p = v == -INFINITY ? 0.f : expf(v - mx);
+          sp[s][kb][qb][e] = p;
+          l += p;
+        }
+      l += __shfl_xor(l, 16);
+      l += __shfl_xor(l, 32);
+      inv[qb] = l > 0.f ? 1.0f / l : 0.f;
+    }
+#pragma unroll
+    for (int qb = 0; qb < 2; ++qb) {
+      floatx4 o[2] = {{0.f, 0.f, 0.f, 0.f}, {0.f, 0.f, 0.f, 0.f}};
+#pragma unroll
+      for (int kb = 0; kb < 2; ++kb)
+#pragma unroll
+        for (int e = 0; e < 4; ++e)
+#pragma unroll
+          for (int nd = 0; nd < 2; ++nd)
+            o[nd] = __builtin_amdgcn_mfma_f32_16x16x4f32(sp[s][kb][qb][e], acc[2 * s + kb][4 + nd][e], o[nd], 0, 0, 0);
+#pragma unroll
+      for (int e = 0; e < 4; ++e) {
+        const float iq = __shfl(inv[qb], 4 * g + e);
+        const int row = wr0 + 32 * s + 16 * qb + 4 * g + e;
+        if (row < M) {
+          float* dst = ctx + (int64_t)row * H + 64 * head + 32 * wn + c;
+          dst[0] = o[0][e] * iq;
+          dst[16] = o[1][e] * iq;
+        }
+      }
+    }
+  }
+}
+
+}
diff --git a/mediquery-rag_amd/csrc/gemm_x6p.hip b/mediquery-rag_amd/csrc/gemm_x6p.hip
--- a/mediquery-rag_amd/csrc/gemm_x6p.hip
+++ b/mediquery-rag_amd/csrc/gemm_x6p.hip
@@ -87,10 +87,14 @@
                                                              const float* __restrict__ bias,
                                                              const float* __restrict__ resid, int ldr,
                                                              float* __restrict__ out, int ldo, int M, int N,
-                                                             int K, int rx, LnFold lf) {
+                                                             int K, int rx, LnFold lf, AttnEpi at) {
   __shared__ __attribute__((aligned(1024))) unsigned char lds[T::NBUF * T::STAGE];
   const unsigned lds0 = (unsigned)(uintptr_t)(x6p_lds_t*)lds;
   constexpr bool HAND = EPI == EPI_RESID_LN_STATS && T::LDR && T::M16 && !T::DEEP && T::NBUF == 3 && !FORMER;
+  constexpr bool ATTN = epi_is_attn(EPI);
+  static_assert(!ATTN || (T::LDR && T::M16 && !T::DEEP && T::NBUF == 3 && T::WAVES_M == 2 && T::WAVES_N == 2 &&
+                          T::TM == 2 && T::TN == 3 && 4 * kAttnStage <= T::STAGE),
+                "attention epilogue: the 128 x 192 loader-wave tile");
   static_assert(!HAND || (T::NW == 4 && 2 * T::WM * T::WN * 4 <= T::STAGE && T::WN == kLnPartW && T::STAGE % 1024 == 0),
                 "hand-off: two wave tiles of t per ring slot");
   const int lane = threadIdx.x & 63;
@@ -151,7 +155,8 @@
     } else {
       if constexpr (T::DBG & 32) return;
       const int b = in - T::NA, nbl = b / 3, p = b - nbl * 3;
-      const int nbg = min((is_n0 >> 5) + nbl, nbw - 1);
+      int nbg = min((is_n0 >> 5) + nbl, nbw - 1);
+      if constexpr (ATTN) nbg = (nbl % 3) * (N / 96) + 2 * (is_n0 / T::BN) + nbl / 3;
       const unsigned char* wbase = W3 + ((size_t)(nbg * nk + kt) * 3 + p) * 1024;
       x6p_glds(wbase, (unsigned)lane * 16u, dst + T::KS * T::A_SUB + ks * T::B_SUB + b * 1024);
     }
@@ -351,9 +356,16 @@
         asm volatile("s_barrier" ::: "memory");
         return;
       }
+      int l_st = 0;
       for (int j = 0; j < S; ++j) {
         wait_stages(IC<T::AHEAD - 2>{});
         issue((j + T::AHEAD) % T::NBUF);
+        if constexpr (ATTN) {
+          if (++l_st == nst) {
+            l_st = 0;
+            asm volatile("s_barrier" ::: "memory");
+          }
+        }
       }
       asm volatile("s_waitcnt vmcnt(0)" ::: "memory");
       return;
@@ -407,19 +419,22 @@
     };
     zero4();
     wait_stages(IC<T::AHEAD - 1>{});
-#pragma unroll
-    for (int m = 0; m < MB; ++m) {
-      rd_raw(lds, m, 0);
-      rd_raw(lds, m, 1);
-      if (m < MB - 1) {
-#pragma unroll
-        for (int q = 0; q < NSUB; ++q) sub(m, q);
-      }
-    }
-#pragma unroll
-    for (int n = 0; n < NB16; ++n)
-#pragma unroll
-      for (int p = 0; p < 3; ++p) rd_b(lds, n, p);
+    auto load_ops = [&](const unsigned char* st) __attribute__((always_inline)) {
+#pragma unroll
+      for (int m = 0; m < MB; ++m) {
+        rd_raw(st, m, 0);
+        rd_raw(st, m, 1);
+        if (m < MB - 1) {
+#pragma unroll
+          for (int q = 0; q < NSUB; ++q) sub(m, q);
+        }
+      }
+#pragma unroll
+      for (int n = 0; n < NB16; ++n)
+#pragma unroll
+        for (int p = 0; p < 3; ++p) rd_b(st, n, p);
+    };
+    load_ops(lds);
     int rb = 1 % T::NBUF;
     int ib = T::AHEAD % T::NBUF;
     for (int j = 0; j < S; ++j) {
@@ -427,6 +442,9 @@
         wait_stages(IC<T::AHEAD - 2>{});
       } else {
         if constexpr (T::DEEP) __builtin_amdgcn_s_waitcnt(0xC07F);
+        if constexpr (ATTN) {
+          if (c_st == nst - 1) __builtin_amdgcn_s_waitcnt(0xC07F);
+        }
         asm volatile("s_barrier" ::: "memory");
       }
       const unsigned char* st = lds + rb * T::STAGE;
@@ -457,8 +475,16 @@
         c_st = 0;
         int m0, n0;
         coords(c_i, m0, n0);
-        store_wave_tile16<EPI, MB, NB16>(acc4, m0 + wm * T::WM, n0 + wn * T::WN, M, N, bias, resid, ldr, out, ldo,
-                                         lane, lf);
+        if constexpr (ATTN) {
+          unsigned char* fs = lds + (j % T::NBUF) * T::STAGE;
+          attn_wave_tile<EPI == EPI_ATTN_LNFOLD>(acc4, m0 + wm * T::WM, n0 / T::BN, wn, M, N / 3, bias, lf, at.mask,
+                                                 at.scale, out, lane, fs + cw * kAttnStage,
+                                                 fs + (cw ^ 1) * kAttnStage);
+          load_ops(st);
+        } else {
+          store_wave_tile16<EPI, MB, NB16>(acc4, m0 + wm * T::WM, n0 + wn * T::WN, M, N, bias, resid, ldr, out, ldo,
+                                           lane, lf);
+        }
         zero4();
         ++c_i;
       }
@@ -543,6 +569,25 @@
   asm volatile("s_waitcnt vmcnt(0)" ::: "memory");
 }
 
+__global__ __launch_bounds__(256) void attn32_kernel(const float* __restrict__ qkv, const int* __restrict__ mask,
+                                                     float* __restrict__ ctx, int M, int H, float scale) {
+  __shared__ __attribute__((aligned(16))) unsigned char stg[4 * kAttnStage];
+  const int lane = threadIdx.x & 63, c = lane & 15, g = lane >> 4;
+  const int cw = __builtin_amdgcn_readfirstlane(threadIdx.x >> 6), wm = cw >> 1, wn = cw & 1;
+  const int heads = H / 64, head = blockIdx.x % heads, wr0 = (blockIdx.x / heads) * 128 + 64 * wm;
+  floatx4 acc[4][6];
+#pragma unroll
+  for (int m = 0; m < 4; ++m)
+#pragma unroll
+    for (int e = 0; e < 4; ++e) {
+      const float* row = qkv + (int64_t)min(wr0 + 16 * m + 4 * g + e, M - 1) * (3 * H) + 64 * head + 32 * wn + c;
+#pragma unroll
+      for (int n = 0; n < 6; ++n) acc[m][n][e] = row[(n >> 1) * H + 16 * (n & 1)];
+    }
+  attn_wave_tile<false, true>(acc, wr0, head, wn, M, H, nullptr, LnFold{}, mask, scale, ctx, lane,
+                              stg + cw * kAttnStage, stg + (cw ^ 1) * kAttnStage);
+}
+
 __global__ __launch_bounds__(256) void split_w3_kernel(const float* __restrict__ W, int N, int K,
                                                        uintx4* __restrict__ w3) {
   const int k8n = K >> 3, np = (N + 31) & ~31;
@@ -589,14 +634,15 @@
     }
   }
   const int tiles = ((g.M + T::BM - 1) / T::BM) * ((g.N + T::BN - 1) / T::BN);
-  const int grid = (std::min(tiles, num_cus) + 7) / 8 * 8;
+  int grid = (std::min(tiles, num_cus) + 7) / 8 * 8;
+  if (g.max_wg > 0) grid = std::min(grid, g.max_wg);
   const int tiles_m = (g.M + T::BM - 1) / T::BM, tiles_n = (g.N + T::BN - 1) / T::BN;
   int rx = g.rx;
   if (rx < 0) rx = region_pick_rx(tiles_m, tiles_n, (double)T::BM * g.K * 4, (double)T::BN * g.K * 6, grid);
   if (rx > 0 && (8 % rx != 0 || rx > tiles_n || 8 / rx > tiles_m || grid < 8)) rx = 0;
   hipLaunchKernelGGL((gemm_x6p_kernel<T, EPI, FORMER>), dim3(grid), dim3(T::THREADS), 0, s, g.A, g.lda,
                      static_cast<const unsigned char*>(g.W3), g.bias, g.resid, g.ldr, g.out, g.ldo, g.M, g.N, g.K, rx,
-                     g.lf);
+                     g.lf, g.at);
 }
 
 template <int EPI>
@@ -676,6 +722,11 @@
                      s_out, c_out);
 }
 
+void launch_attn32(const float* qkv, const int* mask, float* ctx, int M, int H, float scale, hipStream_t s) {
+  hipLaunchKernelGGL(attn32_kernel, dim3((unsigned)(((M + 127) / 128) * (H / 64))), dim3(256), 0, s, qkv, mask, ctx, M,
+                     H, scale);
+}
+
 void launch_split_w3(const float* W, int N, int K, void* w3, hipStream_t s) {
   const int64_t n = (int64_t)((N + 31) & ~31) * (K >> 3);
   hipLaunchKernelGGL(split_w3_kernel, dim3((unsigned)((n + 255) / 256)), dim3(256), 0, s, W, N, K,
@@ -702,6 +753,8 @@
     case EPI_BIAS_LNFOLD: launch_tile_fold<EPI_BIAS_LNFOLD>(g, tile, num_cus, s); return;
     case EPI_GELU_ERF_LNFOLD: launch_tile_fold<EPI_GELU_ERF_LNFOLD>(g, tile, num_cus, s); return;
     case EPI_GELU_TANH_LNFOLD: launch_tile_fold<EPI_GELU_TANH_LNFOLD>(g, tile, num_cus, s); return;
+    case EPI_ATTN_BIAS: launch_t<X6p0, EPI_ATTN_BIAS>(g, num_cus, s); return;
+    case EPI_ATTN_LNFOLD: launch_t<X6p0, EPI_ATTN_LNFOLD>(g, num_cus, s); return;
     default: launch_tile<EPI_BIAS>(g, tile, num_cus, s); return;
   }
 }
@@ -768,7 +821,6 @@
   } else {
     MQ_CHECK_ARG(epi_is_lnfold(epi), "epi must be a LayerNorm-fold kind (got %d)", epi);
     MQ_CHECK_ARG(stats_in && s_fold, "consumer: NULL buffer");
-    MQ_CHECK_ARG(K == kLnPartW * kLnMaxParts, "consumer: K must be %d (got %d)", kLnPartW * kLnMaxParts, K);
   }
   int dev = 0, cus = 256;
   (void)hipGetDevice(&dev);
@@ -785,4 +837,33 @@
   return MQ_OK;
 }
 
-}
+int mq_debug_gemm_x6p_attn(const float* A, const void* W3, const float* bias, const int* mask, float* ctx, int M,
+                           int K, int heads, float scale, int epi, const float* stats_in, const float* s_fold,
+                           float eps, int max_workgroups, void* stream) {
+  using namespace mq;
+  clear_error();
+  MQ_CHECK_ARG(A && W3 && bias && mask && ctx, "NULL buffer");
+  MQ_CHECK_ARG(M > 0 && M % 32 == 0 && K > 0 && K % 32 == 0 && heads > 0 && heads <= 1024,
+               "bad shape M=%d K=%d heads=%d (M and K must be multiples of 32)", M, K, heads);
+  MQ_CHECK_ARG((int64_t)M * heads * 64 < (1ll << 31) && (int64_t)M * K < (1ll << 29), "M too large");
+  MQ_CHECK_ARG(epi == EPI_ATTN_BIAS || epi == EPI_ATTN_LNFOLD, "epi must be an attention kind (got %d)", epi);
+  MQ_CHECK_ARG(epi != EPI_ATTN_LNFOLD || (stats_in && s_fold), "fold: NULL buffer");
+  MQ_CHECK_ARG(max_workgroups >= 0 && max_workgroups % 8 == 0,
+               "max_workgroups must be 0 or a multiple of 8 (got %d)", max_workgroups);
+  int dev = 0, cus = 256;
+  (void)hipGetDevice(&dev);
+  (void)hipDeviceGetAttribute(&cus, hipDeviceAttributeMultiprocessorCount, dev);
+  const int H = 64 * heads;
+  X6pArgs a{A, K, W3, bias, nullptr, 0, ctx, H, M, 3 * H, K};
+  a.lf.stats_in = stats_in;
+  a.lf.s = s_fold;
+  a.lf.eps = eps;
+  a.at.mask = mask;
+  a.at.scale = scale;
+  a.max_wg = max_workgroups;
+  launch_gemm_x6p(a, epi, 0, cus, (hipStream_t)stream);
+  MQ_HIP(hipGetLastError());
+  return MQ_OK;
+}
+
+}
diff --git a/mediquery-rag_amd/csrc/gemm_x6p.hpp b/mediquery-rag_amd/csrc/gemm_x6p.hpp
--- a/mediquery-rag_amd/csrc/gemm_x6p.hpp
+++ b/mediquery-rag_amd/csrc/gemm_x6p.hpp
@@ -59,6 +59,11 @@
 void launch_ln_fold_weight(const float* W, const float* bias, const float* g, const float* b, int N, int K, float* Wg,
                            float* s_out, float* c_out, hipStream_t s);
 
+struct AttnEpi {
+  const int* mask = nullptr;
+  float scale = 0.f;
+};
+
 struct X6pArgs {
   const float* A;
   int lda;
@@ -71,7 +76,11 @@
   int M, N, K;
   int rx = -1;
   LnFold lf{};
+  AttnEpi at{};
+  int max_wg = 0;
 };
+
+void launch_attn32(const float* qkv, const int* mask, float* ctx, int M, int H, float scale, hipStream_t s);
 
 int x6p_pick_tile(int M, int N, int num_cus);
 void launch_gemm_x6p(const X6pArgs& g, int epi, int tile, int num_cus, hipStream_t s);
diff --git a/mediquery-rag_amd/mediquery_hip/_lib.py b/mediquery-rag_amd/mediquery_hip/_lib.py
--- a/mediquery-rag_amd/mediquery_hip/_lib.py
+++ b/mediquery-rag_amd/mediquery_hip/_lib.py
@@ -26,6 +26,7 @@
 MQ_ENC_OPT_ROWS_PLANES = 10
 MQ_ENC_OPT_LN_FOLD = 11
 MQ_ENC_OPT_CLS_KFREE = 12
+MQ_ENC_OPT_QKV_ATTN = 13
 
 
 class MQError(RuntimeError):
@@ -120,6 +121,7 @@
     "mq_debug_gemm_x6p": (_I, [_P, _P, _P, _P, _P, _I, _I, _I, _I, _I, _P]),
     "mq_debug_gemm_x6p_ln": (_I, [_P, _P, _P, _P, _P, _I, _I, _I, _I, _I, _P, _P, _P, _P, _P, ctypes.c_float, _P]),
     "mq_debug_ln_fold_weight": (_I, [_P, _P, _P, _P, _I, _I, _P, _P, _P, _P]),
+    "mq_debug_gemm_x6p_attn": (_I, [_P, _P, _P, _P, _P, _I, _I, _I, ctypes.c_float, _I, _P, _P, ctypes.c_float, _I, _P]),
     "mq_debug_attention": (_I, [_P, _P, _I, _I, _I, _I, ctypes.c_float, _I, _P, _P]),
     "mq_debug_cls_attention": (_I, [_P, _P, _P, _P, _P, ctypes.c_float, _P, _I, _I, _I, _I, ctypes.c_float, _P, _P, _P,
                                     _P, _P]),
diff --git a/mediquery-rag_amd/mediquery_hip/native.py b/mediquery-rag_amd/mediquery_hip/native.py
--- a/mediquery-rag_amd/mediquery_hip/native.py
+++ b/mediquery-rag_amd/mediquery_hip/native.py
@@ -260,7 +260,7 @@
                "splitk_tiles": _lib.MQ_ENC_OPT_SPLITK_TILES, "ln_on_load": _lib.MQ_ENC_OPT_LN_ON_LOAD,
                "resident_layers": _lib.MQ_ENC_OPT_RESIDENT_LAYERS, "x6_presplit": _lib.MQ_ENC_OPT_X6_PRESPLIT,
                "rows_planes": _lib.MQ_ENC_OPT_ROWS_PLANES, "ln_fold": _lib.MQ_ENC_OPT_LN_FOLD,
-               "cls_kfree": _lib.MQ_ENC_OPT_CLS_KFREE}
+               "cls_kfree": _lib.MQ_ENC_OPT_CLS_KFREE, "qkv_attn": _lib.MQ_ENC_OPT_QKV_ATTN}
 
     def set_option(self, name, value):
         _lib.call("mq_encoder_set_option", self._h, self.OPTIONS[name], int(value))
```
